# MiniXC/LightningFastSpeech2

Hardware: AMD Instinct MI355X
Metric: mel-frames/sec (whole node), 256-phoneme batch-32 (higher is better)
Workload: dtype bf16

## Files before the change

### lightningfastspeech2_amd/csrc/capi_ops.hip

```cpp
#include <math.h>

#include "fs2_common.h"
#include "fs2_kernels.h"

using namespace fs2;

namespace fs2 {

template <typename S, typename D>
__global__ __launch_bounds__(256) void convert_kernel(const S* __restrict__ s, D* __restrict__ d, size_t n) {
    for (size_t i = (size_t)blockIdx.x * 256 + threadIdx.x; i < n; i += (size_t)gridDim.x * 256)
        d[i] = Num<D>::from_f32(Num<S>::to_f32(s[i]));
}

int launch_convert(const ConvertArgs& a, int sdt, int ddt, hipStream_t st) {
    if (a.n == 0) return FS2_OK;
    size_t blocks = (a.n + 255) / 256;
    if (blocks > 4096) blocks = 4096;
    const dim3 g((unsigned)blocks), b(256);
    if (sdt == FS2_F32 && ddt == FS2_F32) hipLaunchKernelGGL((convert_kernel<float, float>), g, b, 0, st, (const float*)a.src, (float*)a.dst, a.n);
    else if (sdt == FS2_F32 && ddt == FS2_BF16) hipLaunchKernelGGL((convert_kernel<float, bf16>), g, b, 0, st, (const float*)a.src, (bf16*)a.dst, a.n);
    else if (sdt == FS2_BF16 && ddt == FS2_F32) hipLaunchKernelGGL((convert_kernel<bf16, float>), g, b, 0, st, (const bf16*)a.src, (float*)a.dst, a.n);
    else if (sdt == FS2_BF16 && ddt == FS2_BF16) hipLaunchKernelGGL((convert_kernel<bf16, bf16>), g, b, 0, st, (const bf16*)a.src, (bf16*)a.dst, a.n);
    else return FS2_ERR_ARG;
    return hipGetLastError() == hipSuccess ? FS2_OK : FS2_ERR_HIP;
}

}

namespace fs2 {
int apply_knob(Tuning& t, int variant) {
    int ok = 1;
    if (variant == 1500 || variant == 1501) t.attn_x3 = variant - 1500;
    else if (variant >= 1400 && variant <= 1402) t.gemm_wres = variant - 1400;
    else if (variant == 1340 || variant == 1341) t.enc_attn_out = variant - 1340;
    else if (variant == 1320 || variant == 1321) t.pred_fuse_embed = variant - 1320;
    else if (variant >= 1200 && variant <= 1204) t.attn_pipe = variant - 1200;
    else if (variant == 1100 || variant == 1101) t.colsum_fused = variant - 1100;
    else if (variant == 1000 || variant == 1001) t.bgemm_tn256 = variant - 1000;
    else if (variant >= 905 && variant <= 908) { if (variant >= 907) t.attn_bwd_nb_dq = 3 + ((variant - 905) & 1); else t.attn_bwd_nb = 3 + ((variant - 905) & 1); }
    else if (variant == 909) t.attn_bwd_nb = 1;
    else if (variant >= 900 && variant <= 903) { if (variant >= 902) t.attn_bwd_nb_dq = ((variant - 900) & 1) + 1; else t.attn_bwd_nb = ((variant - 900) & 1) + 1; }
    else if (variant == 904) t.attn_bwd_nb_dq = 0;
    else if (variant == 800 || variant == 801) t.bgemm_full = variant - 800;
    else if (variant == 700 || variant == 701) t.bgemm_xcd = variant - 700;
    else if (variant == 500 || variant == 501) t.split_f32 = variant - 500;
    else if (variant == 230 || variant == 231) t.head_sums = variant - 230;
    else if (variant == 220 || variant == 221) t.gemm_persist = variant - 220;
    else if (variant >= 200 && variant <= 202) t.slab_xcd_remap = variant - 200;
    else if (variant >= 0 && variant <= 7) t.gemm_variant = variant;
    else ok = 0;
    if (!ok) return FS2_ERR_ARG;
    ++t.gen;
    return FS2_OK;
}
Tuning& op_tuning() {
    static thread_local Tuning t;
    return t;
}
}

extern "C" {

int fs2_op_convert(int32_t sdt, int32_t ddt, const void* src, void* dst, size_t n, void* stream) {
    ConvertArgs a{src, dst, n};
    return launch_convert(a, sdt, ddt, (hipStream_t)stream);
}

int fs2_op_predictor(int32_t dtype, const void* x, const void* w, const float* bias, const float* ln_g,
                     const float* ln_b, const float* head_w, float head_b, const uint8_t* mask, float* pred,
                     void* packed_scratch, int32_t B, int32_t S, int32_t H, int32_t nlayers, int32_t taps,
                     void* stream) {
    if (!predictor_fused_supported(dtype, H, taps, nlayers, S)) return FS2_ERR_SHAPE;
    if (!x || !w || !bias || !ln_g || !ln_b || !head_w || !pred || !packed_scratch) return FS2_ERR_ARG;
    const size_t lb = predictor_packed_bytes_per_layer();
    for (int l = 0; l < nlayers; ++l) {
        const int r = launch_pack_predictor_weights((const char*)w + (size_t)l * H * taps * H * 2,
                                                    (char*)packed_scratch + lb * l, (hipStream_t)stream);
        if (r != FS2_OK) return r;
    }
    PredictorArgs a;
    a.x = x; a.wpk = packed_scratch; a.bias = bias; a.ln_g = ln_g; a.ln_b = ln_b; a.head_w = head_w; a.head_b = head_b;
    a.mask = mask; a.pred = pred; a.B = B; a.S = S; a.H = H; a.nlayers = nlayers; a.taps = taps; a.eps = 1e-5f;
    return launch_predictor_fused(a, (hipStream_t)stream);
}

int fs2_op_predictor_dw(int32_t dtype, const void* x, const float* dw_w, const float* dw_b, const void* w, const float* bias,
                        const float* ln_g, const float* ln_b, const float* head_w, float head_b, const uint8_t* mask, float* pred,
                        void* packed_scratch, int32_t B, int32_t S, int32_t H, int32_t nlayers, void* stream) {
    if (!predictor_fused_supported(dtype, H, 3, nlayers, S)) return FS2_ERR_SHAPE;
    if (!x || !dw_w || !dw_b || !w || !bias || !ln_g || !ln_b || !head_w || !pred || !packed_scratch) return FS2_ERR_ARG;
    const size_t lb = predictor_packed_bytes_per_layer(1);
    for (int l = 0; l < nlayers; ++l) {
        const int r = launch_pack_predictor_weights((const char*)w + (size_t)l * H * H * 2, (char*)packed_scratch + lb * l, (hipStream_t)stream, 1);
        if (r != FS2_OK) return r;
    }
    PredictorArgs a;
    a.x = x; a.wpk = packed_scratch; a.dw_w = dw_w; a.dw_b = dw_b; a.bias = bias; a.ln_g = ln_g; a.ln_b = ln_b; a.head_w = head_w; a.head_b = head_b;
    a.mask = mask; a.pred = pred; a.B = B; a.S = S; a.H = H; a.nlayers = nlayers; a.taps = 3; a.eps = 1e-5f;
    return launch_predictor_fused(a, (hipStream_t)stream);
}

int fs2_op_soft_dtw(const float* x, const float* y, int32_t B, int32_t N, int32_t M, int32_t D, float gamma, float* out,
                    void* stream) {
    if (!x || !y || !out) return FS2_ERR_ARG;
    SoftDtwArgs a{x, y, out, B, N, M, D, gamma};
    return launch_soft_dtw(a, (hipStream_t)stream);
}
size_t fs2_op_soft_dtw_grad_scratch_bytes(int32_t B, int32_t N, int32_t M) { return soft_dtw_grad_scratch_bytes(B, N, M); }
int fs2_op_soft_dtw_grad(const float* x, const float* y, int32_t B, int32_t N, int32_t M, int32_t D, float gamma, float* out,
                         float* grad_x, void* scratch, size_t scratch_bytes, void* stream) {
    if (!x || !y || !out) return FS2_ERR_ARG;
    SoftDtwArgs a{x, y, out, B, N, M, D, gamma};
    return launch_soft_dtw_grad(a, grad_x, scratch, scratch_bytes, (hipStream_t)stream);
}

size_t fs2_op_masked_loss_ws_bytes(void) { return fs2::masked_loss_ws_bytes(); }

int fs2_op_masked_loss(const float* pred, const void* truth, int32_t truth_kind, const uint8_t* pad_mask, int64_t rows,
                       int32_t inner, int32_t kind, void* ws, float* out2, void* stream) {
    if (!pred || !truth || !pad_mask || !ws || !out2) return FS2_ERR_ARG;
    if ((kind != 0 && kind != 1) || (truth_kind != 0 && truth_kind != 1)) return FS2_ERR_ARG;
    fs2::LossArgs a;
    a.pred = pred; a.truth = truth; a.mask = pad_mask; a.ws = ws; a.out = out2;
    a.rows = rows; a.inner = inner; a.kind = kind; a.truth_kind = truth_kind;
    return fs2::launch_masked_loss(a, (hipStream_t)stream);
}

int fs2_op_set_vocoder_fused_resblock(int32_t on) {
    fs2::op_tuning().voc_fused_resblock = on;
    return FS2_OK;
}

int fs2_op_set_vocoder_lds_limit(int32_t kib) {
    fs2::op_tuning().voc_lds_limit = kib;
    return FS2_OK;
}



int fs2_op_set_gemm_variant(int32_t variant) { return fs2::apply_knob(fs2::op_tuning(), variant); }

int fs2_op_gemm(int32_t dtype, int32_t out_dtype, const void* x, const void* w, const float* bias, void* c,
                int32_t M, int32_t N, int32_t Cin, int32_t taps, int32_t S, int32_t relu, void* stream) {
    GemmArgs a;
    a.X = x; a.W = w; a.bias = bias; a.C = c;
    a.M = M; a.N = N; a.K = taps * Cin; a.ldx = Cin; a.ldc = N;
    a.Cin = Cin; a.taps = taps; a.pad = (taps - 1) / 2; a.S = S; a.relu = relu;
    return launch_gemm(a, dtype, out_dtype, (hipStream_t)stream);
}

int fs2_op_gemm_relu_dropout(int32_t dtype, const void* x, const void* w, const float* bias, void* c, int32_t M, int32_t N, int32_t Cin,
                             int32_t taps, int32_t S, float p, uint64_t seed, uint64_t key, void* stream) {
    if (!(p > 0.f && p < 1.f)) return FS2_ERR_ARG;
    GemmArgs a;
    a.X = x; a.W = w; a.bias = bias; a.C = c;
    a.M = M; a.N = N; a.K = taps * Cin; a.ldx = Cin; a.ldc = N;
    a.Cin = Cin; a.taps = taps; a.pad = (taps - 1) / 2; a.S = S; a.relu = 1;
    a.drop_p = p; a.drop_seed = seed; a.drop_key = key;
    return launch_gemm(a, dtype, dtype, (hipStream_t)stream);
}

int fs2_op_gemm_add(int32_t dtype, const void* x, const void* w, const float* bias, const void* addend, void* c, int32_t M, int32_t N,
                    int32_t Cin, int32_t taps, int32_t S, void* stream) {
    if (!addend) return FS2_ERR_ARG;
    GemmArgs a;
    a.X = x; a.W = w; a.bias = bias; a.C = c;
    a.M = M; a.N = N; a.K = taps * Cin; a.ldx = Cin; a.ldc = N;
    a.Cin = Cin; a.taps = taps; a.pad = (taps - 1) / 2; a.S = S; a.relu = 0;
    a.epi_res = addend;
    if (N < 192 || M % S || !(taps & 1)) return FS2_ERR_SHAPE;
    return launch_gemm(a, dtype, dtype, (hipStream_t)stream);
}

int fs2_op_gemm_rowscale(const void* x, const void* w, const float* bias, const float* rowstats, const float* wg,
                         void* c, int32_t M, int32_t N, int32_t Cin, void* stream) {
    if (!x || !w || !bias || !rowstats || !wg || !c) return FS2_ERR_ARG;
    GemmArgs a;
    a.X = x; a.W = w; a.bias = bias; a.C = c;
    a.M = M; a.N = N; a.K = Cin; a.ldx = Cin; a.ldc = N;
    a.Cin = Cin; a.taps = 1; a.pad = 0; a.S = M; a.relu = 0;
    a.rs_stats = rowstats; a.rs_wg = wg;
    return launch_gemm(a, FS2_BF16, FS2_BF16, (hipStream_t)stream);
}
int fs2_op_rowstats_finish(const float* parts, int32_t nparts, int32_t ncols, float eps, float* out, int32_t M, void* stream) {
    return launch_rowstats_finish(parts, nparts, ncols, eps, out, M, (hipStream_t)stream);
}
int fs2_op_gemm_head(const void* x, const void* w, const float* bias, const float* head_gw, float* stats_out, float* head_out, int32_t M,
// ... 435 lines not shown
```

### lightningfastspeech2_amd/csrc/engine.hip

```cpp
#include <math.h>
#include <stdarg.h>
#include <stdio.h>
#include <string.h>

#include <functional>
#include <map>
#include <memory>
#include <string>
#include <vector>

#include "fs2_common.h"
#include "fs2_kernels.h"

using namespace fs2;

namespace {

struct HostTensor {
    std::vector<int64_t> shape;
    std::vector<float> data;
};

struct Arena {
    char* base = nullptr;
// ... 661 lines not shown
    a.B = B; a.S = S; a.C = w.C; a.k = w.k; a.pad = (w.k - 1) / 2;
    Bracket br(e, FS2_K_ROWOPS, st, 2.0 * B * S * (double)w.C * w.k, 2.0 * B * S * (double)w.C * (dt == FS2_BF16 ? 2 : 4));
    const int r = launch_dwconv(a, dt, st);
    if (r != FS2_OK) return fail(e, r, "dwconv launch failed");
    return FS2_OK;
}

int norm_only(fs2_engine* e, hipStream_t st, int dt, const void* v, const float* stats, const float* g, const float* b, void* y,
              int M, int H, const float* dot_w = nullptr, float dot_b = 0.f, const uint8_t* mask = nullptr, float* pred = nullptr) {
    LayerNormArgs l;
    l.pre_stats = stats; l.pre_parts = ln_parts(H);
    l.x = v; l.res = nullptr; l.gamma = g; l.beta = b; l.y = y;
    l.dot_w = dot_w; l.dot_b = dot_b; l.mask = mask; l.pred = pred;
    l.M = M; l.H = H; l.eps = 1e-5f;
    Bracket br(e, FS2_K_ROWOPS, st, 0, 2.0 * M * (double)H * (dt == FS2_BF16 ? 2 : 4));
    if (launch_layernorm(l, dt, st) != FS2_OK) return fail(e, FS2_ERR_HIP, "normalise-only LayerNorm launch failed");
    return FS2_OK;
}

struct LayerScratch {
    float *st1, *st2;
    float* rsf;
    float* hd;
    void *qkv, *att, *proj, *hid, *u, *vt;
    uint64_t* bits;
    int Spad, nw64;
};

int conformer(fs2_engine* e, hipStream_t st, const LayerW& w, void* x, void* tmp, int B, int S, int heads,
              const LayerScratch& sc, bool is_decoder, bool prenorm_in = false, const float* pg = nullptr, const float* pb = nullptr,
              bool leave_prenorm = false) {
    const int H = e->cfg.hidden, M = B * S, dt = w.in_proj.dt;
    const double dsz = dt == FS2_BF16 ? 2 : 4;
    Bracket* mha = is_decoder ? nullptr : new Bracket(e, FS2_K_ENC_MHA, st, 8.0 * M * (double)H * H + 4.0 * B * (double)S * S * H,
                                                      2.0 * M * H * dsz + 4.0 * H * H * dsz);
    struct MhaEnd { Bracket*& b; ~MhaEnd() { delete b; b = nullptr; } } mha_end{mha};
    const bool x3 = e->front_split && dt == FS2_F32 && e->tune.attn_x3;
    void* qkv_lo = x3 ? (void*)((char*)sc.qkv + (size_t)M * 3 * H * 2) : nullptr;
    if (prenorm_in) {
        if (!w.has_fold || !(w.depthwise && H > 256 && e->defer_ln)) return fail(e, FS2_ERR_STATE, "pre-norm block input without folded weights");
        const RowScale rs{sc.rsf, w.in_wg};
        CHK(gemm(e, st, w.in_proj_f, x, sc.qkv, M, M, false, dt, nullptr, -1, nullptr, nullptr, nullptr, &rs));
    } else {
        CHK(gemm(e, st, w.in_proj, x, sc.qkv, M, M, false, dt, nullptr, -1, nullptr, nullptr, qkv_lo));
    }
    AttnArgs a;
    a.tune = &e->tune;
    a.qkv_lo = qkv_lo;
    a.qkv = sc.qkv; a.vt = sc.vt; a.kbits = sc.bits; a.out = sc.att;
    a.B = B; a.S = S; a.H = H; a.heads = heads; a.Spad = sc.Spad; a.nw64 = sc.nw64;
    a.scale_log2e = (float)(1.4426950408889634 / sqrt((double)(H / heads)));
    if (w.wo_pk && S <= 768 && e->tune.enc_attn_out && !x3 && !prenorm_in && attn_out_ln_supported(dt, H, heads, S) &&
        !(w.depthwise && H > 256 && e->defer_ln)) {
        AttnOutArgs ao;
        ao.qkv = sc.qkv; ao.kbits = sc.bits; ao.wpk = w.wo_pk; ao.bias = w.out_proj.b; ao.res = x; ao.ln_g = w.g1; ao.ln_b = w.b1; ao.out = tmp;
        ao.B = B; ao.S = S; ao.H = H; ao.heads = heads; ao.nw64 = sc.nw64; ao.scale_log2e = a.scale_log2e; ao.eps = 1e-5f;
        {
            Bracket br(e, FS2_K_ATTENTION, st, 4.0 * B * (double)S * S * H + 2.0 * M * (double)H * H, 5.0 * M * H * dsz + (double)H * H * dsz);
            const int r = launch_attn_out_ln(ao, st);
            if (r != FS2_OK) return fail(e, r, "fused attention + out-projection launch failed");
        }
        delete mha; mha = nullptr;
        if (w.depthwise) {
            CHK(dwconv(e, st, w.dw, tmp, sc.u, B, S, dt));
            CHK(gemm(e, st, w.c1, sc.u, sc.hid, M, S, true, dt, nullptr, is_decoder ? FS2_K_DEC_FFN_CONV1 : -1));
        } else {
            CHK(gemm(e, st, w.c1, tmp, sc.hid, M, S, true, dt, nullptr, is_decoder ? FS2_K_DEC_FFN_CONV1 : -1));
        }
        LnFuse ln;
        ln.res = tmp; ln.g = w.g2; ln.b = w.b2; ln.tmp = sc.proj;
        CHK(gemm(e, st, w.c2, sc.hid, x, M, S, false, dt, &ln));
        return FS2_OK;
    }
    {
        Bracket br(e, FS2_K_ROWOPS, st, 0, 2.0 * M * H * dsz);
        const int r = x3 ? FS2_OK : launch_transpose_v(a, dt, st);
        if (r != FS2_OK) return fail(e, r, "transpose_v launch failed");
    }
    {
        Bracket br(e, FS2_K_ATTENTION, st, 4.0 * B * (double)S * S * H, 4.0 * M * H * dsz);
        Bracket br2(e, FS2_K_DEC_ATTENTION, st, 4.0 * B * (double)S * S * H, 4.0 * M * H * dsz, is_decoder);
        const int r = launch_attention(a, dt, st);
        if (r != FS2_OK) return fail(e, r, "attention launch failed");
    }
    if (w.depthwise && H > 256 && e->defer_ln) {
        Deferred d1;
        d1.res = x; d1.stats_out = sc.st1;
        if (prenorm_in) { d1.res_stats = sc.st2; d1.res_g = pg; d1.res_b = pb; }
        CHK(gemm(e, st, w.out_proj, sc.att, tmp, M, M, false, dt, nullptr, -1, nullptr, &d1));
        delete mha; mha = nullptr;
        LnOnLoad l1{sc.st1, w.g1, w.b1};
        CHK(dwconv(e, st, w.dw, tmp, sc.u, B, S, dt, &l1));
        CHK(gemm(e, st, w.c1, sc.u, sc.hid, M, S, true, dt, nullptr, is_decoder ? FS2_K_DEC_FFN_CONV1 : -1));
        Deferred d2;
        d2.res = tmp; d2.res_stats = sc.st1; d2.res_g = w.g1; d2.res_b = w.b1; d2.stats_out = sc.st2;
        CHK(gemm(e, st, w.c2, sc.hid, x, M, S, false, dt, nullptr, -1, nullptr, &d2));
        if (leave_prenorm) {
            if (launch_rowstats_finish(sc.st2, ln_parts(H), H, 1e-5f, sc.rsf, M, st) != FS2_OK) return fail(e, FS2_ERR_HIP, "row statistics launch failed");
            return FS2_OK;
        }
        return norm_only(e, st, dt, x, sc.st2, w.g2, w.b2, x, M, H);
    }
    {
        LnFuse ln;
        ln.res = x; ln.g = w.g1; ln.b = w.b1; ln.tmp = sc.proj;
        CHK(gemm(e, st, w.out_proj, sc.att, tmp, M, M, false, dt, &ln));
        delete mha; mha = nullptr;
    }
    if (w.depthwise) {
        CHK(dwconv(e, st, w.dw, tmp, sc.u, B, S, dt));
        CHK(gemm(e, st, w.c1, sc.u, sc.hid, M, S, true, dt, nullptr, is_decoder ? FS2_K_DEC_FFN_CONV1 : -1));
    } else {
        CHK(gemm(e, st, w.c1, tmp, sc.hid, M, S, true, dt, nullptr, is_decoder ? FS2_K_DEC_FFN_CONV1 : -1));
    }
    {
        LnFuse ln;
        ln.res = tmp; ln.g = w.g2; ln.b = w.b2; ln.tmp = sc.proj;
        CHK(gemm(e, st, w.c2, sc.hid, x, M, S, false, dt, &ln));
    }
    return FS2_OK;
}

int run_stack(fs2_engine* e, hipStream_t st, const std::vector<LayerW>& Ls, void* x, void* tmp, int B, int S, int heads,
              const LayerScratch& sc, bool is_decoder, bool leave_last = false, bool* left = nullptr) {
    const int H = e->cfg.hidden;
    bool pre = false;
    for (size_t i = 0; i < Ls.size(); ++i) {
        const LayerW& w = Ls[i];
        const bool deferred = w.depthwise && H > 256 && e->defer_ln;
        const bool leave = e->fold_ln && deferred && (i + 1 < Ls.size() ? Ls[i + 1].has_fold && Ls[i + 1].depthwise : leave_last);
        CHK(conformer(e, st, w, x, tmp, B, S, heads, sc, is_decoder, pre, pre ? Ls[i - 1].g2 : nullptr, pre ? Ls[i - 1].b2 : nullptr, leave));
        pre = leave;
    }
    if (left) *left = pre;
    return FS2_OK;
}

struct CwtOut {
    float* spec12 = nullptr;
    float* mean_std = nullptr;
    float* spec_out = nullptr;
};

struct EmbedTail {
    void* y;
    const float* bins;
    const float* emb;
    int nbins;
    float std, mean;
    const float* pe;
    const float* spk;
};

int predictor(fs2_engine* e, hipStream_t st, const PredictorW& P, const void* x, int B, int S, const uint8_t* mask,
              float* pred, const LayerScratch& sc, const CwtOut* cw = nullptr, const EmbedTail* tail = nullptr, bool* tail_done = nullptr) {
    const int M = B * S;
    if (tail_done) *tail_done = false;
    if (P.cwt && !cw) return fail(e, FS2_ERR_STATE, "CWT predictor without its output buffers");
    if (P.wpk && P.wpk_lo && e->fuse_predictor && P.dt == FS2_F32 && e->front_split &&
        predictor_fused_x3_supported(P.filt, P.layers[0].c.taps, (int)P.layers.size(), S)) {
        PredictorArgs a;
        a.x = x; a.wpk = P.wpk; a.wpk_lo = P.wpk_lo; a.bias = P.bias_all; a.ln_g = P.g_all; a.ln_b = P.b_all;
        a.head_w = P.head_w; a.head_b = P.head_b; a.mask = mask; a.pred = pred;
        a.B = B; a.S = S; a.H = P.filt; a.nlayers = (int)P.layers.size(); a.taps = P.layers[0].c.taps; a.eps = 1e-5f;
        const bool with_tail = tail && tail_done && !P.cwt && tail->y != x && tail->nbins >= 2 && tail->nbins - 1 <= 512;
        if (with_tail) {
            a.be_y = tail->y; a.be_bins = tail->bins; a.be_emb = tail->emb; a.be_nbins = tail->nbins;
            a.be_std = tail->std; a.be_mean = tail->mean; a.be_pe = tail->pe; a.be_spk = tail->spk;
        }
        const double fl = 2.0 * M * (double)P.filt * P.filt * a.taps * a.nlayers;
        Bracket br(e, FS2_K_CONV_GEMM, st, fl, (double)M * P.filt * 4 + (double)M * 4 + (with_tail ? 2.0 * M * P.filt * 4 : 0.0));
        Bracket brp(e, FS2_K_PREDICTOR, st, fl, (double)M * P.filt * 4 + (double)M * 4 + (with_tail ? 2.0 * M * P.filt * 4 : 0.0), x != e->xA && x != e->xB);
        const int r = launch_predictor_fused_x3(a, st);
        if (r != FS2_OK) return fail(e, r, "fused predictor (split arithmetic) launch failed (B=%d S=%d)", B, S);
        if (with_tail) *tail_done = true;
        return FS2_OK;
    }
    if (P.wpk && !P.wpk_lo && e->fuse_predictor && predictor_fused_supported(P.dt, P.filt, P.dw_all ? 3 : P.layers[0].c.taps, (int)P.layers.size(), S)) {
        PredictorArgs a;
        a.x = x; a.wpk = P.wpk; a.bias = P.bias_all; a.ln_g = P.g_all; a.ln_b = P.b_all;
        a.dw_w = P.dw_all; a.dw_b = P.dwb_all;
        a.head_w = P.head_w; a.head_b = P.head_b; a.mask = mask; a.pred = pred;
        a.B = B; a.S = S; a.H = P.filt; a.nlayers = (int)P.layers.size(); a.taps = P.dw_all ? 3 : P.layers[0].c.taps; a.eps = 1e-5f;
        const bool with_tail = tail && tail_done && !P.cwt && tail->y != x && tail->nbins >= 2 && tail->nbins - 1 <= 512;
        if (with_tail) {
            a.be_y = tail->y; a.be_bins = tail->bins; a.be_emb = tail->emb; a.be_nbins = tail->nbins;
            a.be_std = tail->std; a.be_mean = tail->mean; a.be_pe = tail->pe; a.be_spk = tail->spk;
        }
        const double fl = (P.dw_all ? 2.0 * M * (double)P.filt * (P.filt + 3) : 2.0 * M * (double)P.filt * P.filt * a.taps) * a.nlayers;
        const double by = (double)M * P.filt * 2 + (double)M * 4 + (with_tail ? 2.0 * M * P.filt * 2 : 0.0);
        Bracket br(e, FS2_K_CONV_GEMM, st, fl, by);
        Bracket brp(e, FS2_K_PREDICTOR, st, fl, by, x != e->xA && x != e->xB);
        const int r = launch_predictor_fused(a, st);
        if (r != FS2_OK) return fail(e, r, "fused predictor launch failed (B=%d S=%d)", B, S);
        if (with_tail) *tail_done = true;
        return FS2_OK;
    }
    if (P.layers[0].depthwise && P.filt > 256 && e->defer_ln) {
        const void* src = x;
        float* stats[2] = {sc.st1, sc.st2};
        const PredLayerW* prev = nullptr;
        bool head_done = false;
        for (size_t j = 0; j < P.layers.size(); ++j) {
            const PredLayerW& Lw = P.layers[j];
            void* out = (j & 1) ? sc.proj : sc.att;
            LnOnLoad lp{stats[(j + 1) & 1], prev ? prev->g : nullptr, prev ? prev->b : nullptr};
            CHK(dwconv(e, st, Lw.dw, src, sc.u, B, S, P.dt, prev ? &lp : nullptr));
            Deferred d;
            d.stats_out = stats[j & 1];
            if (j + 1 == P.layers.size() && !P.cwt && P.head_gw) { d.head_gw = P.head_gw; d.head_out = sc.hd; d.head_done = &head_done; }
            CHK(gemm(e, st, Lw.c, sc.u, out, M, S, true, P.dt, nullptr, -1, nullptr, &d));
            src = out;
            prev = &Lw;
        }
        float* stl = stats[(P.layers.size() - 1) & 1];
        if (head_done) {
            Bracket br(e, FS2_K_ROWOPS, st, 0, (double)M * ln_parts(P.filt) * 12);
            if (launch_head_finish(stl, sc.hd, ln_parts(P.filt), P.filt, 1e-5f, P.head_sum_gw, P.head_cst, mask, pred, M, st) != FS2_OK)
                return fail(e, FS2_ERR_HIP, "head finish launch failed");
            return FS2_OK;
        }
        if (!P.cwt) return norm_only(e, st, P.dt, src, stl, prev->g, prev->b, nullptr, M, P.filt, P.head_w, P.head_b, mask, pred);
        CHK(norm_only(e, st, P.dt, src, stl, prev->g, prev->b, (void*)src, M, P.filt));
        CHK(gemm(e, st, P.head_mat, src, cw->spec12, M, M, false, FS2_F32));
        CwtArgs ca{src, cw->spec12, 12, mask, P.ms_w, P.ms_b, cw->mean_std, pred, cw->spec_out, B, S, P.filt};
        if (launch_cwt_head(ca, P.dt, st) != FS2_OK) return fail(e, FS2_ERR_HIP, "cwt head launch failed");
        return FS2_OK;
    }
    const void* src = x;
    for (size_t j = 0; j < P.layers.size(); ++j) {
        const PredLayerW& Lw = P.layers[j];
        const bool last = j + 1 == P.layers.size();
        void* out = (j & 1) ? sc.proj : sc.att;
        void* other = (j & 1) ? sc.att : sc.proj;
        LnFuse ln;
        ln.g = Lw.g; ln.b = Lw.b;
        const bool keep = !last || P.cwt;
        if (last && !P.cwt) { ln.dot_w = P.head_w; ln.dot_b = P.head_b; ln.mask = mask; ln.pred = pred; }
        if (Lw.depthwise) {
            CHK(dwconv(e, st, Lw.dw, src, sc.u, B, S, P.dt));
            ln.tmp = other;
            CHK(gemm(e, st, Lw.c, sc.u, keep ? out : nullptr, M, S, true, P.dt, &ln));
        } else {
            ln.tmp = sc.u;
            CHK(gemm(e, st, Lw.c, src, keep ? out : nullptr, M, S, true, P.dt, &ln));
        }
        src = out;
    }
    if (P.cwt) {
        CHK(gemm(e, st, P.head_mat, src, cw->spec12, M, M, false, FS2_F32));
        CwtArgs ca{src, cw->spec12, 12, mask, P.ms_w, P.ms_b, cw->mean_std, pred, cw->spec_out, B, S, P.filt};
        if (launch_cwt_head(ca, P.dt, st) != FS2_OK) return fail(e, FS2_ERR_HIP, "cwt head launch failed");
    }
    return FS2_OK;
}

size_t layer_scratch_bytes(const fs2_engine* e, int B, int S) {
    const fs2_config& c = e->cfg;
    const size_t H = c.hidden, M = (size_t)B * S, esz = e->esz;
    size_t Fm = c.enc_filter > c.dec_filter ? c.enc_filter : c.dec_filter;
    size_t Pm = H;
    if ((size_t)c.var_filter > Pm) Pm = c.var_filter;
    if ((size_t)c.dur_filter > Pm) Pm = c.dur_filter;
    const size_t Spad = ((size_t)S + 63) / 64 * 64;
    return al(M * 3 * H * esz) + 3 * al(M * Pm * esz) + al(M * Fm * esz) + al((size_t)B * H * Spad * esz) +
           al((size_t)B * (Spad / 64) * 8) + 2 * al(M * (size_t)ln_parts((int)Pm) * 8) + al(M * 8) + al(M * 16) + 4096;
}
int take_layer_scratch(fs2_engine* e, Arena& ar, int B, int S, LayerScratch* sc) {
    const fs2_config& c = e->cfg;
    const size_t H = c.hidden, M = (size_t)B * S, esz = e->esz;
    size_t Fm = c.enc_filter > c.dec_filter ? c.enc_filter : c.dec_filter;
    size_t Pm = H;
    if ((size_t)c.var_filter > Pm) Pm = c.var_filter;
    if ((size_t)c.dur_filter > Pm) Pm = c.dur_filter;
    sc->Spad = (S + 63) / 64 * 64;
    sc->nw64 = sc->Spad / 64;
    sc->st1 = (float*)ar.take(M * (size_t)ln_parts((int)Pm) * 8);
    sc->st2 = (float*)ar.take(M * (size_t)ln_parts((int)Pm) * 8);
    sc->rsf = (float*)ar.take(M * 8);
    sc->hd = (float*)ar.take(M * 16);
    sc->qkv = ar.take(M * 3 * H * esz);
    sc->att = ar.take(M * Pm * esz);
    sc->proj = ar.take(M * Pm * esz);
    sc->hid = ar.take(M * Fm * esz);
    sc->u = ar.take(M * Pm * esz);
    sc->vt = ar.take((size_t)B * H * sc->Spad * esz);
    sc->bits = (uint64_t*)ar.take((size_t)B * sc->nw64 * 8);
    if (!sc->st1 || !sc->st2 || !sc->rsf || !sc->hd || !sc->qkv || !sc->att || !sc->proj || !sc->hid || !sc->u || !sc->vt || !sc->bits)
        return fail(e, FS2_ERR_NOMEM, "scratch arena too small");
    return FS2_OK;
}

size_t persist_bytes(const fs2_engine* e, int B, int L) {
    const size_t H = e->cfg.hidden, ML = (size_t)B * L, esz = e->esz;
    size_t pv = 0;
    for (int v = 0; v < e->cfg.n_variances; ++v)
        if (e->cfg.var_level[v]) pv += al(ML * 4) + (e->cfg.var_cwt[v] ? al(ML * 10 * 4) + al((size_t)B * 8) : 0);
    return al((size_t)B * H * 4) + 2 * al(ML * H * esz) + al(ML * 4) + 2 * al(ML * 4) + 2 * al((size_t)B * 4) + al(ML) + pv + 4096;
}
size_t encode_scratch_bytes(const fs2_engine* e, int B, int L) {
    size_t cw = 0;
    for (int v = 0; v < e->cfg.n_variances; ++v)
        if (e->cfg.var_level[v] && e->cfg.var_cwt[v]) cw = al((size_t)B * L * 12 * 4) + 512;
    return layer_scratch_bytes(e, B, L) + cw;
}
size_t decode_scratch_bytes(const fs2_engine* e, int B, int T) {
    const size_t H = e->cfg.hidden, MT = (size_t)B * T, esz = e->esz;
    size_t cw = 0;
    for (int v = 0; v < e->cfg.n_variances; ++v)
        if (e->cfg.var_cwt[v]) cw = al(MT * 12 * 4) + al((size_t)B * 8) + 512;
    return layer_scratch_bytes(e, B, T) + 2 * al(MT * H * esz) + al(MT) + (size_t)e->cfg.n_variances * al(MT * 4) + cw + 4096;
}
int ensure_arena(fs2_engine* e, Arena& ar, size_t need, const char* what) {
    if (need > ar.cap && !ar.external) HIPCHK(e, hipDeviceSynchronize());
    if (ar.reserve(need) != FS2_OK)
        return fail(e, FS2_ERR_NOMEM, ar.external ? "caller workspace too small: %s needs %zu bytes (fs2_workspace_bytes)"
                                                  : "%s arena: hipMalloc of %zu bytes failed", what, need);
    return FS2_OK;
}

int tap_store(fs2_engine* e, hipStream_t st, const std::string& name, const void* src, size_t n, int src_dt,
              Arena* arena = nullptr) {
    void* dst = (arena ? arena : &e->dbg)->take(n * 4);
    if (!dst) return fail(e, FS2_ERR_NOMEM, "debug arena too small");
    ConvertArgs a{src, dst, n};
    const int r = launch_convert(a, src_dt, FS2_F32, st);
    if (r != FS2_OK) return fail(e, r, "convert launch failed");
    e->taps[name] = {dst, n * 4};
    return FS2_OK;
}

}

extern "C" {

int fs2_abi_version(void) { return FS2_ABI_VERSION; }

const char* fs2_status_string(int s) {
    switch (s) {
        case FS2_OK: return "ok";
        case FS2_ERR_HIP: return "HIP runtime error";
        case FS2_ERR_SHAPE: return "unsupported shape/config";
        case FS2_ERR_ARG: return "bad argument";
        case FS2_ERR_WEIGHT: return "weight error";
        case FS2_ERR_STATE: return "call order violated";
        case FS2_ERR_NOMEM: return "out of device memory";
    }
    return "unknown status";
}

const char* fs2_last_error(const fs2_engine* e) { return e ? e->err : "null engine"; }

int fs2_create(const fs2_config* cfg, fs2_engine** out) {
    if (!cfg || !out) return FS2_ERR_ARG;
    fs2_engine* e = new fs2_engine();
    e->cfg = *cfg;
    e->err[0] = 0;
    *out = e;
    const int r = check_config(e);
    if (r != FS2_OK) return r;
    e->dt = cfg->dtype;
    e->fdt = cfg->dtype == FS2_BF16 ? FS2_BF16 : FS2_F32;
    e->bdt = (cfg->dtype == FS2_F32 || cfg->dtype == FS2_F32_X3) ? FS2_F32 : FS2_BF16;
    e->esz = cfg->dtype == FS2_BF16 ? 2 : 4;
    e->front_split = cfg->dtype == FS2_MIXED_X3 || cfg->dtype == FS2_F32_X3;
    build_spec(e);
    return FS2_OK;
}

int fs2_clone(const fs2_engine* src, fs2_engine** out) {
    if (!src || !out) return FS2_ERR_ARG;
    if (!src->finalized) return FS2_ERR_STATE;
    fs2_engine* e = new fs2_engine();
    e->cfg = src->cfg;
    e->dt = src->dt; e->fdt = src->fdt; e->bdt = src->bdt; e->esz = src->esz;
    e->err[0] = 0;
    e->finalized = true;
    e->fuse_predictor = src->fuse_predictor;
    e->use_graph = src->use_graph;
    e->zero_pad_mel = src->zero_pad_mel;
    e->defer_ln = src->defer_ln;
    e->fold_ln = src->fold_ln;
    e->tune = src->tune;
    e->front_split = src->front_split;
    e->spec = src->spec;
    e->dev_allocs = src->dev_allocs;
    e->phone_table = src->phone_table; e->pe = src->pe; e->spk_w = src->spk_w; e->spk_b = src->spk_b;
    e->enc = src->enc; e->dec = src->dec; e->dur = src->dur; e->vars = src->vars; e->mel = src->mel; e->priors_w = src->priors_w;
    e->mel_f = src->mel_f; e->mel_wg = src->mel_wg; e->mel_fold = src->mel_fold;
    *out = e;
    return FS2_OK;
}

int fs2_destroy(fs2_engine* e) {
    if (!e) return FS2_OK;
    (void)hipDeviceSynchronize();
    e->dev_allocs.reset();
    e->persist.release();
    e->scratch.release();
    e->dbg.release();
    e->dbg_enc.release();
    if (e->h_pinned) (void)hipHostFree(e->h_pinned);
    for (auto& g : e->dgraphs) if (g.exec) (void)hipGraphExecDestroy(g.exec);
    for (auto& g : e->egraphs) if (g.exec) (void)hipGraphExecDestroy(g.exec);
    if (e->gev_in) (void)hipEventDestroy(e->gev_in);
    if (e->gev_out) (void)hipEventDestroy(e->gev_out);
    if (e->gstream) (void)hipStreamDestroy(e->gstream);
    for (auto& s : e->prof)
        for (auto& ev : s.ev) { (void)hipEventDestroy(ev.first); (void)hipEventDestroy(ev.second); }
    delete e;
    return FS2_OK;
}

int fs2_load_weight(fs2_engine* e, const char* name, const float* data, const int64_t* shape, int32_t ndim) {
    if (!e || !name || !data || !shape || ndim < 0) return FS2_ERR_ARG;
    if (e->finalized) return fail(e, FS2_ERR_STATE, "weights already finalized");
    auto it = e->spec.find(name);
    if (it == e->spec.end()) return fail(e, FS2_ERR_WEIGHT, "unexpected weight '%s' for this config", name);
    const std::vector<int64_t>& want = it->second;
    bool ok = (size_t)ndim == want.size();
    size_t n = 1;
    for (int i = 0; ok && i < ndim; ++i) { ok = shape[i] == want[i]; n *= (size_t)shape[i]; }
    if (!ok) return fail(e, FS2_ERR_WEIGHT, "shape mismatch for '%s'", name);
    HostTensor t;
    t.shape.assign(shape, shape + ndim);
    t.data.assign(data, data + n);
    e->host[name] = std::move(t);
    return FS2_OK;
}

int fs2_finalize(fs2_engine* e) {
    if (!e) return FS2_ERR_ARG;
    if (e->finalized) return FS2_OK;
    for (auto& kv : e->spec)
        if (!e->host.count(kv.first)) return fail(e, FS2_ERR_WEIGHT, "missing weight '%s'", kv.first.c_str());
    const fs2_config& c = e->cfg;
    const int H = c.hidden;
    CHK(up_vec(e, "phone_embedding.weight", &e->phone_table));
    CHK(up_vec(e, "positional_encoding.pe", &e->pe));
    CHK(up_vec(e, "speaker_embedding.projection.weight", &e->spk_w));
    CHK(up_vec(e, "speaker_embedding.projection.bias", &e->spk_b));
    e->enc.resize(c.enc_layers);
    for (int i = 0; i < c.enc_layers; ++i)
        CHK(make_layer(e, "encoder.layers." + std::to_string(i), H, c.enc_filter, c.enc_depthwise, &e->enc[i], e->fdt));
    e->dec.resize(c.dec_layers);
    for (int i = 0; i < c.dec_layers; ++i)
        CHK(make_layer(e, "decoder.layers." + std::to_string(i), H, c.dec_filter, c.dec_depthwise, &e->dec[i], e->bdt));
    if (H > 256) {
        for (int i = 1; i < c.enc_layers && c.enc_depthwise && e->fdt == FS2_BF16; ++i)
            CHK(make_folded_in_proj(e, "encoder.layers." + std::to_string(i), "encoder.layers." + std::to_string(i - 1), H, &e->enc[i]));
        for (int i = 1; i < c.dec_layers && c.dec_depthwise && e->bdt == FS2_BF16; ++i)
            CHK(make_folded_in_proj(e, "decoder.layers." + std::to_string(i), "decoder.layers." + std::to_string(i - 1), H, &e->dec[i]));
    }
    CHK(make_predictor(e, "variance_adaptor.duration_predictor", c.dur_nlayers, c.dur_filter, c.dur_depthwise, &e->dur, e->fdt));
    e->vars.resize(c.n_variances);
    for (int v = 0; v < c.n_variances; ++v) {
        const std::string p = std::string("variance_adaptor.encoders.") + c.var_names[v];
        CHK(make_predictor(e, p + ".predictor", c.var_nlayers[v], c.var_filter, c.var_depthwise, &e->vars[v].pred, e->fdt, c.var_cwt[v] != 0));
        if (c.var_cwt[v]) {
            CHK(up_vec(e, p + ".mean_std_linear.weight", &e->vars[v].pred.ms_w));
            CHK(up_vec(e, p + ".mean_std_linear.bias", &e->vars[v].pred.ms_b));
        }
        CHK(up_vec(e, p + ".bins", &e->vars[v].bins));
        CHK(up_vec(e, p + ".embedding.weight", &e->vars[v].emb));
    }
    CHK(make_conv(e, "linear.weight", "linear.bias", &e->mel, e->bdt));
    if (H > 256 && c.dec_layers > 0 && c.dec_depthwise && e->bdt == FS2_BF16 && c.n_mels < 192) {
        const std::string pp = "decoder.layers." + std::to_string(c.dec_layers - 1);
        const HostTensor &w = W(e, "linear.weight"), &b = W(e, "linear.bias"), &g = W(e, pp + ".norm2.weight"), &be = W(e, pp + ".norm2.bias");
        const int N = (int)b.data.size();
        std::vector<float> wf((size_t)N * H), bf(N), wg(N);
        for (int n = 0; n < N; ++n) {
            double bacc = b.data[n], gacc = 0;
            for (int k = 0; k < H; ++k) {
                const float v = (float)((double)w.data[(size_t)n * H + k] * g.data[k]);
                wf[(size_t)n * H + k] = v;
                bacc += (double)w.data[(size_t)n * H + k] * be.data[k];
                gacc += (double)bf16_to_f32(f32_to_bf16(v));
            }
            bf[n] = (float)bacc;
            wg[n] = (float)gacc;
        }
        e->mel_f.N = N; e->mel_f.Cin = H; e->mel_f.taps = 1; e->mel_f.dt = FS2_BF16;
        CHK(upload_mat(e, wf.data(), wf.size(), &e->mel_f.w, FS2_BF16));
        CHK(upload_f32(e, bf.data(), bf.size(), &e->mel_f.b));
        CHK(upload_f32(e, wg.data(), wg.size(), &e->mel_wg));
        e->mel_fold = true;
    }
    e->priors_w.resize(c.n_priors);
    for (int p = 0; p < c.n_priors; ++p) {
        const std::string q = std::string("prior_embeddings.") + c.prior_names[p];
        CHK(up_vec(e, q + ".bins", &e->priors_w[p].bins));
        std::vector<float> t = W(e, q + ".embedding.weight").data;
        for (float& v : t) v = v > 0.f ? v : 0.f;
        CHK(upload_f32(e, t.data(), t.size(), &e->priors_w[p].emb));
    }
    e->host.clear();
    e->finalized = true;
    return FS2_OK;
}

int fs2_set_fused_predictor(fs2_engine* e, int32_t on) {
    if (!e) return FS2_ERR_ARG;
    e->fuse_predictor = on != 0;
    return FS2_OK;
}

int fs2_set_debug(fs2_engine* e, int32_t on) {
    if (!e) return FS2_ERR_ARG;
    e->debug = on != 0;
    return FS2_OK;
}

int fs2_set_deferred_layernorm(fs2_engine* e, int32_t on) {
    if (!e) return FS2_ERR_ARG;
    e->defer_ln = on != 0;
    return FS2_OK;
}

int fs2_set_tuning(fs2_engine* e, int32_t knob) {
    if (!e) return FS2_ERR_ARG;
    const bool op_only = (knob >= 900 && knob <= 909) || knob == 1000 || knob == 1001 || knob == 1100 || knob == 1101 ||
                         knob == 700 || knob == 701 || knob == 800 || knob == 801 || knob == 500 || knob == 501;
    if (op_only) return fail(e, FS2_ERR_ARG, "fs2_set_tuning(%d): an operator-level switch no engine launch reads (use fs2_op_set_gemm_variant on the calling thread)", (int)knob);
    const int r = apply_knob(e->tune, knob);
    if (r != FS2_OK) return fail(e, r, "fs2_set_tuning(%d): not a defined switch", (int)knob);
    return FS2_OK;
}

int fs2_set_folded_layernorm(fs2_engine* e, int32_t on) {
    if (!e) return FS2_ERR_ARG;
    e->fold_ln = on != 0;
    return FS2_OK;
}

int fs2_set_zero_pad_mel(fs2_engine* e, int32_t on) {
    if (!e) return FS2_ERR_ARG;
    e->zero_pad_mel = on != 0;
    return FS2_OK;
}

int fs2_workspace_bytes(const fs2_engine* e, int32_t B, int32_t L, int32_t T, size_t* persist, size_t* scratch) {
    if (!e || B <= 0 || L <= 0 || T < 0) return FS2_ERR_ARG;
    if (persist) *persist = persist_bytes(e, B, L);
    if (scratch) {
        const size_t enc = encode_scratch_bytes(e, B, L), dec = T > 0 ? decode_scratch_bytes(e, B, T) : 0;
        *scratch = enc > dec ? enc : dec;
    }
    return FS2_OK;
}

int fs2_set_workspace(fs2_engine* e, void* persist, size_t persist_bytes_, void* scratch, size_t scratch_bytes_) {
    if (!e || (persist == nullptr) != (scratch == nullptr)) return e ? fail(e, FS2_ERR_ARG, "give both buffers or neither") : FS2_ERR_ARG;
    if (((uintptr_t)persist | (uintptr_t)scratch) & 255) return fail(e, FS2_ERR_ARG, "workspace buffers must be 256-byte aligned");
    if (e->mid_forward && (char*)persist != e->persist.base)
        return fail(e, FS2_ERR_STATE, "the persist buffer holds the encoder state between fs2_encode and fs2_decode: only scratch may change there");
    if (!e->mid_forward) e->persist.adopt(persist, persist_bytes_);
    e->scratch.adopt(scratch, scratch_bytes_);
    return FS2_OK;
}

int fs2_set_frames(fs2_engine* e, int32_t T) {
    if (!e) return FS2_ERR_ARG;
    if (!e->encoded) return fail(e, FS2_ERR_STATE, "fs2_set_frames without a preceding successful fs2_encode");
    if (T < e->T) return fail(e, FS2_ERR_ARG, "fs2_set_frames can only pad: T=%d < this batch's %d", T, e->T);
    if (T > e->cfg.max_frames || T > e->cfg.pe_len) return fail(e, FS2_ERR_SHAPE, "T=%d exceeds max_frames/positional table", T);
    e->T = T;
    return FS2_OK;
}

static void drop_graphs(fs2_engine* e);
static int encode_body(fs2_engine* e, const int64_t* phones, const float* speaker, const int32_t* forced, LayerScratch& sc, hipStream_t st);

static int variance_stage(fs2_engine* e, hipStream_t st, int v, void*& x, void*& xalt, int B, int S, const uint8_t* mask, float* vpred,
                          const LayerScratch& sc, const CwtOut* cwo, bool add_pe_spk, Arena& dbg) {
    const fs2_config& c = e->cfg;
    const size_t M = (size_t)B * S, H = c.hidden, esz = e->esz;
    const bool tail_ok = e->tune.pred_fuse_embed && !e->debug && !e->forced_idx[v] && !e->forced_tgt[v] && !c.var_cwt[v] &&
                         (e->fdt == FS2_BF16 || (e->fdt == FS2_F32 && e->front_split && e->vars[v].pred.wpk_lo)) && H == 256;
    const EmbedTail tl{xalt, e->vars[v].bins, e->vars[v].emb, c.var_nbins, c.var_std[v], c.var_mean[v],
                       add_pe_spk ? e->pe : nullptr, add_pe_spk ? e->spk : nullptr};
    bool tail_done = false;
    CHK(predictor(e, st, e->vars[v].pred, x, B, S, mask, vpred, sc, cwo, tail_ok ? &tl : nullptr, &tail_done));
    if (tail_done) {
        std::swap(x, xalt);
        return FS2_OK;
    }
    int32_t* idx = nullptr;
    if (e->debug) {
        idx = (int32_t*)dbg.take(M * 4);
        if (!idx) return fail(e, FS2_ERR_NOMEM, "debug arena too small");
        e->taps[std::string("bucket_") + c.var_names[v]] = {idx, M * 4};
    }
    Bracket br(e, FS2_K_ROWOPS, st, 0, 2.0 * M * H * esz);
    BucketArgs ba{x, vpred, e->vars[v].bins, e->vars[v].emb, c.var_nbins, c.var_std[v], c.var_mean[v],
                  add_pe_spk ? e->pe : nullptr, add_pe_spk ? e->spk : nullptr, x, idx, B, S, (int)H,
                  e->forced_idx[v], 0, e->forced_tgt[v]};
    if (launch_bucket_embed(ba, e->fdt, st) != FS2_OK) return fail(e, FS2_ERR_HIP, "bucket_embed launch failed");
    return FS2_OK;
}
static int run_phase(fs2_engine* e, std::vector<fs2_engine::GraphEntry>& cache, const std::vector<uint64_t>& key, bool plain,
                     hipStream_t st, const std::function<int(hipStream_t)>& body);

int fs2_encode(fs2_engine* e, const int64_t* phones, const float* speaker, int32_t B, int32_t L,
               const int32_t* forced, void* stream, int32_t* T_out) {
    if (!e || !phones || !speaker || !T_out || B <= 0 || L <= 0) return e ? fail(e, FS2_ERR_ARG, "bad encode argument") : FS2_ERR_ARG;
    if (!e->finalized) return fail(e, FS2_ERR_STATE, "fs2_finalize not called");
    if (L > e->cfg.pe_len) return fail(e, FS2_ERR_SHAPE, "L=%d exceeds positional table %d", L, e->cfg.pe_len);
    hipStream_t st = (hipStream_t)stream;
    const fs2_config& c = e->cfg;
    const size_t H = c.hidden, ML = (size_t)B * L, esz = e->esz;
    e->encoded = false;
    e->mid_forward = false;
    e->B = B;
    e->L = L;
    e->taps.clear();
    CHK(ensure_arena(e, e->persist, persist_bytes(e, B, L), "persist"));
    CHK(ensure_arena(e, e->scratch, encode_scratch_bytes(e, B, L), "scratch"));
    e->spk = (float*)e->persist.take((size_t)B * H * 4);
    e->xA = e->persist.take(ML * H * esz);
    e->xB = e->persist.take(ML * H * esz);
    e->dur_pred = (float*)e->persist.take(ML * 4);
    e->d_dur = (int32_t*)e->persist.take(ML * 4);
    e->d_cum = (int32_t*)e->persist.take(ML * 4);
    e->d_totals = (int32_t*)e->persist.take((size_t)2 * B * 4);
    e->d_guard = e->d_totals ? e->d_totals + B : nullptr;
    e->src_mask = (uint8_t*)e->persist.take(ML);
    bool pv_ok = true, pv_forced = false;
    for (int v = 0; v < c.n_variances; ++v) {
        e->pv_pred[v] = e->pv_spec[v] = e->pv_ms[v] = nullptr;
        if (!c.var_level[v]) continue;
        e->pv_pred[v] = (float*)e->persist.take(ML * 4);
        if (c.var_cwt[v]) {
            e->pv_spec[v] = (float*)e->persist.take(ML * 10 * 4);
            e->pv_ms[v] = (float*)e->persist.take((size_t)B * 8);
        }
        pv_ok = pv_ok && e->pv_pred[v] && (!c.var_cwt[v] || (e->pv_spec[v] && e->pv_ms[v]));
        pv_forced = pv_forced || e->forced_idx[v] || e->forced_tgt[v];
    }
    if (!e->src_mask || !pv_ok) return fail(e, FS2_ERR_NOMEM, "persist arena too small");
    LayerScratch sc;
    CHK(take_layer_scratch(e, e->scratch, B, L, &sc));
    if (e->h_pinned_cap < 2 * B) {
        if (e->h_pinned) (void)hipHostFree(e->h_pinned);
        e->h_pinned = nullptr;
        HIPCHK(e, hipHostMalloc((void**)&e->h_pinned, (size_t)2 * B * 4, hipHostMallocDefault));
        e->h_pinned_cap = 2 * B;
        drop_graphs(e);
    }
    {
        std::vector<uint64_t> key = {(uint64_t)B, (uint64_t)L, (uint64_t)e->persist.base, (uint64_t)e->scratch.base, (uint64_t)phones,
                                     (uint64_t)speaker, (uint64_t)forced, (uint64_t)e->h_pinned, (uint64_t)e->fuse_predictor, (uint64_t)e->tune.gen,
                                     (uint64_t)e->defer_ln, (uint64_t)e->front_split, (uint64_t)e->fold_ln};
        const bool plain = c.n_priors != 0 || pv_forced;
        CHK(run_phase(e, e->egraphs, key, plain, st, [&](hipStream_t s2) { return encode_body(e, phones, speaker, forced, sc, s2); }));
    }
    HIPCHK(e, hipStreamSynchronize(st));
    e->totals.assign(e->h_pinned, e->h_pinned + B);
    e->guard.assign(e->h_pinned + B, e->h_pinned + 2 * B);
    int mx = 0;
    for (int b = 0; b < B; ++b) mx = e->totals[b] > mx ? e->totals[b] : mx;
    e->T = mx < c.max_frames ? mx : c.max_frames;
    if (e->T > c.pe_len) return fail(e, FS2_ERR_SHAPE, "T=%d exceeds positional table %d", e->T, c.pe_len);
    *T_out = e->T;
    e->encoded = true;
    e->mid_forward = true;
    return FS2_OK;
}

static int encode_body(fs2_engine* e, const int64_t* phones, const float* speaker, const int32_t* forced, LayerScratch& sc, hipStream_t st) {
    const fs2_config& c = e->cfg;
    const int B = e->B, L = e->L;
    const size_t H = c.hidden, ML = (size_t)B * L, esz = e->esz;
    {
        Bracket br(e, FS2_K_ROWOPS, st, 0, ML * H * esz);
        SpkProjArgs sp{speaker, e->spk_w, e->spk_b, e->spk, B, (int)H, c.dvec_dim};
        if (launch_spk_proj(sp, st) != FS2_OK) return fail(e, FS2_ERR_HIP, "spk_proj launch failed");
        EmbedArgs em{phones, e->phone_table, e->pe, e->spk, e->xA, e->src_mask, B, L, (int)H, c.n_phones};
        if (launch_embed(em, e->fdt, st) != FS2_OK) return fail(e, FS2_ERR_HIP, "embed launch failed");
        MaskBitsArgs mb{e->src_mask, sc.bits, B, L, sc.nw64};
        if (launch_mask_bits(mb, st) != FS2_OK) return fail(e, FS2_ERR_HIP, "mask_bits launch failed");
    }
    CHK(run_stack(e, st, e->enc, e->xA, e->xB, B, L, c.enc_heads, sc, false));
    if (e->debug) {
        const size_t need_d = al(ML * H * 4) + (size_t)c.n_variances * al(ML * 4) + 4096;
        if (need_d > e->dbg_enc.cap) HIPCHK(e, hipDeviceSynchronize());
        if (e->dbg_enc.reserve(need_d) != FS2_OK) return fail(e, FS2_ERR_NOMEM, "debug arena");
        CHK(tap_store(e, st, "encoder_out", e->xA, ML * H, e->fdt, &e->dbg_enc));
    }
    if (c.n_priors) {
        if (!e->priors_dev || e->priors_B != B) return fail(e, FS2_ERR_STATE, "fs2_set_priors(B=%d) required before fs2_encode", B);
        for (int p = 0; p < c.n_priors; ++p) {
            BucketArgs ba{e->xA, e->priors_dev + (size_t)p * B, e->priors_w[p].bins, e->priors_w[p].emb, c.var_nbins,
                          1.0f, 0.0f, nullptr, nullptr, e->xA, nullptr, B, L, (int)H, nullptr, 1};
            if (launch_bucket_embed(ba, e->fdt, st) != FS2_OK) return fail(e, FS2_ERR_HIP, "prior embedding launch failed");
        }
        e->priors_dev = nullptr;
    }
    CHK(predictor(e, st, e->dur, e->xA, B, L, e->src_mask, e->dur_pred, sc));
    void* x = e->xA;
    void* xalt = e->xB;
    float* spec12 = nullptr;
    for (int v = 0; v < c.n_variances; ++v) {
        if (!c.var_level[v]) continue;
        CwtOut cwo;
        if (c.var_cwt[v]) {
            if (!spec12) spec12 = (float*)e->scratch.take(ML * 12 * 4);
            if (!spec12) return fail(e, FS2_ERR_NOMEM, "scratch arena too small");
            cwo.spec12 = spec12;
            cwo.mean_std = e->pv_ms[v];
            cwo.spec_out = e->pv_spec[v];
        }
        CHK(variance_stage(e, st, v, x, xalt, B, L, e->src_mask, e->pv_pred[v], sc, c.var_cwt[v] ? &cwo : nullptr, false, e->dbg_enc));
        e->forced_idx[v] = nullptr, e->forced_tgt[v] = nullptr;
    }
    if (x != e->xA) HIPCHK(e, hipMemcpyAsync(e->xA, x, ML * H * esz, hipMemcpyDeviceToDevice, st));
    DurationArgs da{e->dur_pred, e->src_mask, forced, e->d_dur, e->d_cum, e->d_totals, e->d_guard, B, L};
    if (launch_durations(da, st) != FS2_OK) return fail(e, FS2_ERR_HIP, "durations launch failed");
    HIPCHK(e, hipMemcpyAsync(e->h_pinned, e->d_totals, (size_t)2 * B * 4, hipMemcpyDeviceToHost, st));
    return FS2_OK;
}

int fs2_set_priors(fs2_engine* e, const float* priors_device, int32_t B) {
    if (!e || !priors_device || B <= 0) return FS2_ERR_ARG;
    if (e->cfg.n_priors == 0) return fail(e, FS2_ERR_STATE, "this engine was configured without priors");
    e->priors_dev = priors_device;
    e->priors_B = B;
    return FS2_OK;
}

int fs2_last_totals(const fs2_engine* e, int32_t* totals, int32_t* guard, int32_t B) {
    if (!e || !e->encoded || B != e->B) return FS2_ERR_STATE;
    if (totals) memcpy(totals, e->totals.data(), (size_t)B * 4);
    if (guard) memcpy(guard, e->guard.data(), (size_t)B * 4);
    return FS2_OK;
}

static int decode_body(fs2_engine* e, const fs2_outputs* out, hipStream_t st) {
    const fs2_config& c = e->cfg;
    const int B = e->B, L = e->L, T = e->T;
    const size_t H = c.hidden, MT = (size_t)B * T, ML = (size_t)B * L, esz = e->esz;
    auto phone_outputs = [&]() -> int {
        if (out->duration_prediction) HIPCHK(e, hipMemcpyAsync(out->duration_prediction, e->dur_pred, ML * 4, hipMemcpyDeviceToDevice, st));
        if (out->duration_rounded) HIPCHK(e, hipMemcpyAsync(out->duration_rounded, e->d_dur, ML * 4, hipMemcpyDeviceToDevice, st));
        if (out->src_mask) HIPCHK(e, hipMemcpyAsync(out->src_mask, e->src_mask, ML, hipMemcpyDeviceToDevice, st));
        for (int v = 0; v < c.n_variances; ++v) {
            if (!c.var_level[v]) continue;
            if (out->variances[v]) HIPCHK(e, hipMemcpyAsync(out->variances[v], e->pv_pred[v], ML * 4, hipMemcpyDeviceToDevice, st));
            if (c.var_cwt[v] && out->var_spectrogram[v]) HIPCHK(e, hipMemcpyAsync(out->var_spectrogram[v], e->pv_spec[v], ML * 10 * 4, hipMemcpyDeviceToDevice, st));
            if (c.var_cwt[v] && out->var_mean_std[v]) HIPCHK(e, hipMemcpyAsync(out->var_mean_std[v], e->pv_ms[v], (size_t)B * 8, hipMemcpyDeviceToDevice, st));
        }
        return FS2_OK;
    };
    if (T == 0) { e->encoded = false; e->mid_forward = false; return phone_outputs(); }

    CHK(ensure_arena(e, e->scratch, decode_scratch_bytes(e, B, T), "scratch"));
    e->mid_forward = false;
    void* yA = e->scratch.take(MT * H * esz);
    void* yB = e->scratch.take(MT * H * esz);
    uint8_t* tmask = out->tgt_mask ? out->tgt_mask : (uint8_t*)e->scratch.take(MT);
    float* vpred[FS2_MAX_VARIANCES] = {nullptr, nullptr, nullptr, nullptr};
    int last_frame_v = -1;
    for (int v = 0; v < c.n_variances; ++v) {
        if (c.var_level[v]) continue;
        last_frame_v = v;
        vpred[v] = out->variances[v] ? out->variances[v] : (float*)e->scratch.take(MT * 4);
        if (!vpred[v]) return fail(e, FS2_ERR_NOMEM, "scratch arena too small");
    }
    float *cw_spec = nullptr, *cw_ms = nullptr;
    for (int v = 0; v < c.n_variances; ++v)
        if (c.var_cwt[v] && !c.var_level[v] && !cw_spec) {
            cw_spec = (float*)e->scratch.take(MT * 12 * 4);
            cw_ms = (float*)e->scratch.take((size_t)B * 8);
            if (!cw_spec || !cw_ms) return fail(e, FS2_ERR_NOMEM, "scratch arena too small");
        }
    LayerScratch sc;
    CHK(take_layer_scratch(e, e->scratch, B, T, &sc));
    if (!yA || !yB || !tmask) return fail(e, FS2_ERR_NOMEM, "scratch arena too small");
    if (e->debug) {
        const size_t need_d = 3 * al(MT * H * 4) + (size_t)c.n_variances * al(MT * 4) + 4096;
        if (need_d > e->dbg.cap) HIPCHK(e, hipDeviceSynchronize());
        if (e->dbg.reserve(need_d) != FS2_OK) return fail(e, FS2_ERR_NOMEM, "debug arena");
    }

    {
        Bracket br(e, FS2_K_ROWOPS, st, 0, 2.0 * MT * H * esz);
        RegulateArgs ra{e->xA, e->d_cum, e->d_totals, yA, tmask, B, L, T, (int)H};
        if (launch_regulate(ra, e->fdt, st) != FS2_OK) return fail(e, FS2_ERR_HIP, "regulate launch failed");
        MaskBitsArgs mb{tmask, sc.bits, B, T, sc.nw64};
        if (launch_mask_bits(mb, st) != FS2_OK) return fail(e, FS2_ERR_HIP, "mask_bits launch failed");
    }
    if (e->debug) CHK(tap_store(e, st, "regulated", yA, MT * H, e->fdt));
    const bool fuse_pe = !e->debug;
    for (int v = 0; v < c.n_variances; ++v) {
        if (c.var_level[v]) continue;
        CwtOut cwo;
        if (c.var_cwt[v]) {
            cwo.spec12 = cw_spec;
            cwo.mean_std = out->var_mean_std[v] ? out->var_mean_std[v] : cw_ms;
            cwo.spec_out = out->var_spectrogram[v];
        }
        CHK(variance_stage(e, st, v, yA, yB, B, T, tmask, vpred[v], sc, c.var_cwt[v] ? &cwo : nullptr, v == last_frame_v && fuse_pe, e->dbg));
    }
    if (e->debug) CHK(tap_store(e, st, "adaptor_out", yA, MT * H, e->fdt));
    if (!fuse_pe || last_frame_v < 0) {
        BucketArgs ba{yA, nullptr, nullptr, nullptr, 0, 0.f, 0.f, e->pe, e->spk, yA, nullptr, B, T, (int)H, nullptr};
        if (launch_bucket_embed(ba, e->fdt, st) != FS2_OK) return fail(e, FS2_ERR_HIP, "pe/spk add launch failed");
    }
    if (e->fdt != e->bdt) {
        ConvertArgs ca{yA, yB, MT * H};
        if (launch_convert(ca, e->fdt, e->bdt, st) != FS2_OK) return fail(e, FS2_ERR_HIP, "front -> back conversion failed");
        std::swap(yA, yB);
    }
    bool dec_pre = false;
    CHK(run_stack(e, st, e->dec, yA, yB, B, T, c.dec_heads, sc, true, e->mel_fold && out->mel && !e->debug, &dec_pre));
    if (e->debug) CHK(tap_store(e, st, "decoder_out", yA, MT * H, e->bdt));
    if (out->mel && dec_pre) {
        const RowScale rs{sc.rsf, e->mel_wg};
        CHK(gemm(e, st, e->mel_f, yA, out->mel, (int)MT, (int)MT, false, FS2_F32, nullptr, -1, e->zero_pad_mel ? tmask : nullptr, nullptr, nullptr, &rs));
    } else if (out->mel) {
        CHK(gemm(e, st, e->mel, yA, out->mel, (int)MT, (int)MT, false, FS2_F32, nullptr, -1, e->zero_pad_mel ? tmask : nullptr));
    }
    for (int v = 0; v < FS2_MAX_VARIANCES; ++v) e->forced_idx[v] = nullptr, e->forced_tgt[v] = nullptr;
    return phone_outputs();
}

static void drop_graphs(fs2_engine* e) {
    for (auto& g : e->dgraphs) if (g.exec) (void)hipGraphExecDestroy(g.exec);
    for (auto& g : e->egraphs) if (g.exec) (void)hipGraphExecDestroy(g.exec);
    e->dgraphs.clear();
    e->egraphs.clear();
}

static int run_phase(fs2_engine* e, std::vector<fs2_engine::GraphEntry>& cache, const std::vector<uint64_t>& key, bool plain,
                     hipStream_t st, const std::function<int(hipStream_t)>& body) {
    static const bool gdbg = getenv("FS2_GRAPH_DEBUG") != nullptr;
    plain = plain || !e->use_graph || e->debug;
    for (int k = 0; k < FS2_K_COUNT && !plain; ++k) plain = e->prof[k].enabled;
    if (plain) return body(st);
    fs2_engine::GraphEntry* g = nullptr;
    for (auto& c : cache) if (c.key == key) { g = &c; break; }
    if (!g) {
        if (cache.size() >= 8) {
            size_t old = 0;
            for (size_t i = 1; i < cache.size(); ++i) if (cache[i].stamp < cache[old].stamp) old = i;
            if (cache[old].exec) (void)hipGraphExecDestroy(cache[old].exec);
            cache.erase(cache.begin() + old);
        }
        cache.emplace_back();
        cache.back().key = key;
        cache.back().stamp = ++e->gclock;
        if (gdbg) fprintf(stderr, "fs2 graph: new signature (%zu cached)\n", cache.size());
        return body(st);
    }
    g->stamp = ++e->gclock;
    if (g->bad) { if (gdbg) fprintf(stderr, "fs2 graph: signature marked bad\n"); return body(st); }
    if (!e->gstream) {
        if (hipStreamCreateWithFlags(&e->gstream, hipStreamNonBlocking) != hipSuccess ||
            hipEventCreateWithFlags(&e->gev_in, hipEventDisableTiming) != hipSuccess ||
            hipEventCreateWithFlags(&e->gev_out, hipEventDisableTiming) != hipSuccess) {
            e->use_graph = false;
            return body(st);
        }
    }
    if (!g->exec) {
        if (hipStreamBeginCapture(e->gstream, hipStreamCaptureModeThreadLocal) != hipSuccess) { g->bad = true; return body(st); }
        const bool enc = e->encoded, mid = e->mid_forward;
        const int r = body(e->gstream);
        hipGraph_t graph = nullptr;
        const hipError_t ce = hipStreamEndCapture(e->gstream, &graph);
        hipError_t ie = hipSuccess;
        if (r != FS2_OK || ce != hipSuccess || !graph || (ie = hipGraphInstantiate(&g->exec, graph, nullptr, nullptr, 0)) != hipSuccess) {
            if (gdbg) fprintf(stderr, "fs2 graph: capture failed (body %d, end %d %s, instantiate %d)\n", r, (int)ce, hipGetErrorString(ce), (int)ie);
            if (graph) (void)hipGraphDestroy(graph);
            (void)hipGetLastError();
            g->exec = nullptr;
            g->bad = true;
            e->encoded = enc; e->mid_forward = mid;
            return body(st);
        }
        (void)hipGraphDestroy(graph);
    }
    HIPCHK(e, hipEventRecord(e->gev_in, st));
    HIPCHK(e, hipStreamWaitEvent(e->gstream, e->gev_in, 0));
    HIPCHK(e, hipGraphLaunch(g->exec, e->gstream));
    HIPCHK(e, hipEventRecord(e->gev_out, e->gstream));
    HIPCHK(e, hipStreamWaitEvent(st, e->gev_out, 0));
    e->graph_replays++;
    return FS2_OK;
}

int fs2_decode(fs2_engine* e, const fs2_outputs* out, void* stream) {
    if (!e || !out) return FS2_ERR_ARG;
    if (!e->encoded) return fail(e, FS2_ERR_STATE, "fs2_decode without a preceding successful fs2_encode");
    hipStream_t st = (hipStream_t)stream;
    bool plain = !e->use_graph || e->debug || e->T == 0;
    for (int v = 0; v < FS2_MAX_VARIANCES && !plain; ++v) plain = e->forced_idx[v] || e->forced_tgt[v];
    if (plain) return decode_body(e, out, st);
    const char* base0 = e->scratch.base;
    CHK(ensure_arena(e, e->scratch, decode_scratch_bytes(e, e->B, e->T), "scratch"));
    if (e->scratch.base != base0) drop_graphs(e);
    std::vector<uint64_t> key = {(uint64_t)e->B, (uint64_t)e->L, (uint64_t)e->T, (uint64_t)e->scratch.base, (uint64_t)e->persist.base,
                                 (uint64_t)e->xA, (uint64_t)e->d_cum, (uint64_t)e->spk, (uint64_t)e->zero_pad_mel, (uint64_t)e->fuse_predictor, (uint64_t)e->tune.gen,
                                 (uint64_t)e->defer_ln, (uint64_t)e->front_split, (uint64_t)e->fold_ln, (uint64_t)out->mel, (uint64_t)out->tgt_mask,
                                 (uint64_t)out->duration_prediction, (uint64_t)out->duration_rounded, (uint64_t)out->src_mask};
    for (int v = 0; v < FS2_MAX_VARIANCES; ++v) {
        key.push_back((uint64_t)out->variances[v]);
        key.push_back((uint64_t)out->var_mean_std[v]);
        key.push_back((uint64_t)out->var_spectrogram[v]);
    }
    const int r = run_phase(e, e->dgraphs, key, false, st, [&](hipStream_t s2) { return decode_body(e, out, s2); });
    if (r == FS2_OK) e->mid_forward = false;
    return r;
}

int fs2_set_graphs(fs2_engine* e, int32_t on) {
    if (!e) return FS2_ERR_ARG;
    e->use_graph = on != 0;
    if (!on) drop_graphs(e);
    return FS2_OK;
}

int64_t fs2_graph_replays(const fs2_engine* e) { return e ? e->graph_replays : -1; }

int fs2_force_buckets(fs2_engine* e, int32_t variance_index, const int32_t* idx) {
    if (!e || variance_index < 0 || variance_index >= e->cfg.n_variances) return FS2_ERR_ARG;
    e->forced_idx[variance_index] = idx;
    return FS2_OK;
}

int fs2_force_variance_targets(fs2_engine* e, int32_t variance_index, const float* tgt) {
    if (!e || variance_index < 0 || variance_index >= e->cfg.n_variances) return FS2_ERR_ARG;
    e->forced_tgt[variance_index] = tgt;
    return FS2_OK;
}

int fs2_debug_copy(fs2_engine* e, const char* what, void* dst, void* stream) {
    if (!e || !what || !dst) return FS2_ERR_ARG;
    auto it = e->taps.find(what);
    if (it == e->taps.end()) return fail(e, FS2_ERR_STATE, "no debug tap '%s' (fs2_set_debug before encode?)", what);
    HIPCHK(e, hipMemcpyAsync(dst, it->second.first, it->second.second, hipMemcpyDeviceToDevice, (hipStream_t)stream));
    return FS2_OK;
}

int fs2_profile_enable(fs2_engine* e, int32_t cls, int32_t enable) {
    if (!e || cls < 0 || cls >= FS2_K_COUNT) return FS2_ERR_ARG;
    ProfSlot& s = e->prof[cls];
    s.enabled = enable != 0;
    s.used = 0;
    s.flops = s.bytes = 0;
    return FS2_OK;
}

int fs2_profile_reserve(fs2_engine* e, int32_t cls, int32_t pairs) {
    if (!e || cls < 0 || cls >= FS2_K_COUNT || pairs < 0) return FS2_ERR_ARG;
// ... 31 lines not shown
```

### lightningfastspeech2_amd/csrc/fs2_kernels.h

```cpp
#pragma once
#include <hip/hip_runtime.h>
#include <stdint.h>

#include "../../include/fs2.h"

namespace fs2 {

struct Tuning {
    int gemm_variant = 0;
    int gemm_wres = 1;
    int head_sums = 1;
    int gemm_persist = 1;
    int slab_xcd_remap = 1;
    int split_f32 = 0;
    int attn_pipe = 3;
    int attn_x3 = 1;
    int enc_attn_out = 1;
    int pred_fuse_embed = 1;
    int attn_bwd_nb = 1, attn_bwd_nb_dq = 0;
    int colsum_fused = 0;
    int bgemm_full = 1, bgemm_xcd = 1, bgemm_tn256 = 1;
    int voc_lds_limit = 0;
    int voc_fused_resblock = 1;
    unsigned long long gen = 0;
};
Tuning& op_tuning();
int apply_knob(Tuning& t, int variant);
inline const Tuning& tuning_of(const Tuning* t) { return t ? *t : op_tuning(); }

struct GemmArgs {
    const void* X;
    const void* W;
    const float* bias;
    void* C;
    void* C_lo = nullptr;
    int M, N, K;
    int ldx, ldc;
    int Cin, taps, pad;
    int S;
    int relu;
    const void* res = nullptr;
    const float* ln_g = nullptr;
    const float* ln_b = nullptr;
    float ln_eps = 1e-5f;
    const float* dot_w = nullptr;
    float dot_b = 0.f;
    const uint8_t* mask = nullptr;
    float* pred = nullptr;
    void* ln_tmp = nullptr;
    void* z_out = nullptr;
    int xcd_remap = 0;
    const Tuning* tune = nullptr;
    const void* epi_res = nullptr;
    const float* epi_res_stats = nullptr;
    const float* epi_res_g = nullptr;
    const float* epi_res_b = nullptr;
    int epi_res_parts = 0;
    float* stats_out = nullptr;
    int w_presplit = 0;
    int split = 0;
    const uint8_t* zero_rows = nullptr;
    const void* gate = nullptr;
    float gate_scale = 1.f;
    float drop_p = 0.f;
    uint64_t drop_seed = 0, drop_key = 0;
    const float* rs_stats = nullptr;
    const float* rs_wg = nullptr;
    const float* head_gw = nullptr;
    float* head_out = nullptr;
    int ksplit = 0;
};
int launch_gemm(const GemmArgs& a, int in_dtype, int out_dtype, hipStream_t stream);
int launch_presplit_pack(const float* w, void* out, size_t n_values, hipStream_t stream);
bool gemm_presplit_eligible(int N, int K);
int launch_split_k_reduce(const float* part, void* out, size_t n, int ksplit, int accumulate, int out_dtype, hipStream_t stream);
int gemm_splitk_choice(int M, int N, int Cin, int taps, int S, int in_dtype);
bool gemm_wres_supported(const GemmArgs& a, int in_dtype, int out_dtype, bool force);
int launch_gemm_wres(const GemmArgs& a, hipStream_t stream);
bool gemm_persist_supported(const GemmArgs& a, int in_dtype, int out_dtype, int mi);
bool gemm_head_supported(const GemmArgs& a, int in_dtype, int out_dtype);
bool gemm_persist_pays(const GemmArgs& a, int mi);
int launch_gemm_persist(const GemmArgs& a, int mi, hipStream_t stream);

struct AttnArgs {
    const void* qkv;
    void* vt;
    const uint64_t* kbits;
    void* out;
    int B, S, H, heads, Spad, nw64;
    float scale_log2e;
    const void* qkv_lo = nullptr;
    float* lse2 = nullptr;
    float drop_p = 0.f;
    uint64_t drop_seed = 0, drop_key = 0;
    const Tuning* tune = nullptr;
};
struct AttnOutArgs {
    const void* qkv;
    const uint64_t* kbits;
    const void* wpk;
    const float* bias;
    const void* res;
    const float* ln_g;
    const float* ln_b;
    void* out;
    int B, S, H, heads, nw64;
    float scale_log2e, eps;
};
bool attn_out_ln_supported(int dtype, int H, int heads, int S);
int launch_attn_out_ln(const AttnOutArgs& a, hipStream_t stream);
struct AttnBwdArgs {
    const void* qkv;
    const void* dout;
    const float* lse2;
    const float* delta;
    const uint8_t* key_pad;
    void* dqkv;
    int B, S, H, heads;
    float scale_log2e, scale;
    float drop_p;
    uint64_t drop_seed, drop_key;
    const Tuning* tune = nullptr;
};
bool attention_bwd_supported(int dtype, int H, int heads);
int launch_attention_bwd(const AttnBwdArgs& a, int dtype, hipStream_t stream);
int launch_transpose_v(const AttnArgs& a, int dtype, hipStream_t stream);
int launch_split_hi_lo(const float* x, void* hi, void* lo, size_t n, hipStream_t stream);
int launch_attention(const AttnArgs& a, int dtype, hipStream_t stream);
bool attention_pipe_supported(const AttnArgs& a, int dtype);
int launch_attention_pipe(const AttnArgs& a, int variant, hipStream_t stream);

struct PredictorArgs {
    const void* x;
    const void* wpk;
    const float* dw_w = nullptr;
    const float* dw_b = nullptr;
    const void* wpk_lo = nullptr;
    const float* bias;
    const float* ln_g;
    const float* ln_b;
    const float* head_w;
    float head_b;
    const uint8_t* mask;
    float* pred;
    int B, S, H, nlayers, taps;
    float eps;
    void* be_y = nullptr;
    const float* be_bins = nullptr;
    const float* be_emb = nullptr;
    int be_nbins = 0;
    float be_std = 1.f, be_mean = 0.f;
    const float* be_pe = nullptr;
    const float* be_spk = nullptr;
};
bool predictor_fused_supported(int dtype, int H, int taps, int nlayers, int S);
size_t predictor_packed_bytes_per_layer(int taps = 3);
int launch_pack_predictor_weights(const void* w_layer , void* out_layer, hipStream_t stream, int taps = 3);
int launch_predictor_fused(const PredictorArgs& a, hipStream_t stream);
bool predictor_fused_x3_supported(int H, int taps, int nlayers, int S);
int launch_predictor_fused_x3(const PredictorArgs& a, hipStream_t stream);

struct VocConvArgs {
    const void* x;
    const void* w;
    const float* bias;
    const void* res;
    void* out;
    const int32_t* lengths;
    int len_scale;
    int B, S;
    int cin, cin_pad, n, taps, dil, pad;
    int wn;
    float in_slope;
    float scale;
    int accumulate;
    int in_fp32;
    int post;
    float out_slope = 1.f;
    const Tuning* tune = nullptr;
    int shift_from = 0;
};
struct VocResblockArgs {
    const void* x;
    void* out;
    const void* w;
    const float* bias;
    const int32_t* lengths;
    int len_scale;
    int B, S, C, taps, wn, npairs;
    int dil[3];
    float slope, scale;
    int accumulate;
    int x_act = 0;
    int out_act = 0;
    const Tuning* tune = nullptr;
};
struct LossArgs {
    const float* pred;
    const void* truth;
    const uint8_t* mask;
    void* ws;
    float* out;
    int64_t rows;
    int inner, kind, truth_kind;
};
struct SoftDtwArgs {
    const float* x;
    const float* y;
    float* out;
    int B, N, M, D;
    float gamma;
};
size_t soft_dtw_lds_bytes(int N, int M, int D);
int launch_soft_dtw(const SoftDtwArgs& a, hipStream_t stream);
size_t soft_dtw_grad_scratch_bytes(int B, int N, int M);
int launch_soft_dtw_grad(const SoftDtwArgs& a, float* grad_x, void* scratch, size_t scratch_bytes, hipStream_t stream);
size_t masked_loss_ws_bytes();
int launch_masked_loss(const LossArgs& a, hipStream_t stream);
int voc_resblock_mi16(const VocResblockArgs& a, int dtype);
int launch_vocoder_resblock(const VocResblockArgs& a, int dtype, hipStream_t stream);
int voc_steps_padded(int taps, int cin_pad, int dtype);
int launch_vocoder_conv(const VocConvArgs& a, int dtype, hipStream_t stream);

struct ConvertArgs {
    const void* src;
    void* dst;
    size_t n;
};
int launch_convert(const ConvertArgs& a, int src_dtype, int dst_dtype, hipStream_t stream);

struct LayerNormArgs {
    const void* x;
    const void* res;
    const float* gamma;
    const float* beta;
    void* y;
    const float* dot_w;
    float dot_b;
    const uint8_t* mask;
    float* pred;
    int M, H;
    float eps;
    const float* pre_stats = nullptr;
    int pre_parts = 0;
    const float* dot_b_dev = nullptr;
    float drop_p = 0.f;
    uint64_t drop_seed = 0, drop_key = 0;
};
int launch_layernorm(const LayerNormArgs& a, int dtype, hipStream_t stream);

int launch_rowstats_finish(const float* parts, int nparts, int ncols, float eps, float* out, int M, hipStream_t stream);
int launch_head_finish(const float* parts, const float* dots, int nparts, int ncols, float eps, float sum_gw, float cst, const uint8_t* mask, float* pred,
                       int M, hipStream_t stream);

struct DwConvArgs {
    const void* x;
    const float* w;
    const float* bias;
    void* y;
    int B, S, C, k, pad;
    const float* ln_stats = nullptr;
    const float* ln_g = nullptr;
    const float* ln_b = nullptr;
    int ln_parts = 0;
    float ln_eps = 1e-5f;
    int flip = 0;
};
int launch_dwconv(const DwConvArgs& a, int dtype, hipStream_t stream);

struct CwtArgs {
    const void* out_conv;
    const float* spec;
    int ld_spec;
    const uint8_t* mask;
    const float* ms_w;
    const float* ms_b;
    float* mean_std;
    float* pred;
    float* spec_out;
    int B, T, F;
};
int launch_cwt_head(const CwtArgs& a, int dtype, hipStream_t stream);

struct EmbedArgs {
    const int64_t* phones;
    const float* table;
    const float* pe;
    const float* spk;
    void* x;
    uint8_t* src_mask;
    int B, L, H, n_phones;
};
int launch_embed(const EmbedArgs& a, int dtype, hipStream_t stream);

struct SpkProjArgs {
    const float* dvec;
    const float* w;
    const float* b;
    float* spk;
    int B, H, Din;
};
int launch_spk_proj(const SpkProjArgs& a, hipStream_t stream);

struct MaskBitsArgs {
    const uint8_t* mask;
    uint64_t* bits;
    int B, S, nw64;
};
int launch_mask_bits(const MaskBitsArgs& a, hipStream_t stream);

struct DurationArgs {
    const float* dur_pred;
    const uint8_t* src_mask;
    const int32_t* forced;
    int32_t* dur;
    int32_t* cum;
    int32_t* totals;
    int32_t* guard;
    int B, L;
};
int launch_durations(const DurationArgs& a, hipStream_t stream);

struct RegulateArgs {
    const void* x;
    const int32_t* cum;
    const int32_t* totals;
    void* y;
    uint8_t* tgt_mask;
    int B, L, T, H;
};
int launch_regulate(const RegulateArgs& a, int dtype, hipStream_t stream);

struct BucketArgs {
    const void* x;
    const float* pred;
    const float* bins;
    const float* emb;
    int nbins;
    float std, mean;
    const float* pe;
    const float* spk;
    void* y;
    int32_t* idx_out;
    int B, T, H;
    const int32_t* forced_idx;
    int pred_per_utt = 0;
    const float* bucket_src = nullptr;
};
int launch_bucket_embed(const BucketArgs& a, int dtype, hipStream_t stream);

struct BGemmArgs {
    const void* A;
    const void* B;
    void* C;
    const float* bias = nullptr;
    int M = 0, N = 0, K = 0;
    long sAm = 0, sAk = 0;
    long sBk = 0, sBn = 0;
    long ldc = 0;
    int nb1 = 1, nb2 = 1;
    long sA1 = 0, sA2 = 0, sB1 = 0, sB2 = 0, sC1 = 0, sC2 = 0;
    float alpha = 1.f, beta = 0.f;
    int splitk = 1;
    float* ws = nullptr;
    int seg = 0;
    int taps = 1, Kin = 0;
    int a_shift0 = 0, a_shift_step = 0;
    long sBtap = 0;
    int b_shift0 = 0, b_shift_step = 0;
    const void* epi_p = nullptr;
    const float* epi_delta = nullptr;
    float drop_p = 0.f;
    uint64_t drop_seed = 0, drop_key = 0;
    int c_dtype = FS2_F32;
    int vecA = 0, vecB = 0;
    int xcd_remap = 0;
    const Tuning* tune = nullptr;
};
size_t bgemm_ws_bytes(const BGemmArgs& a);
bool bgemm_tn256_eligible(const BGemmArgs& a);
int launch_bgemm(const BGemmArgs& a, int dtype, hipStream_t stream);

struct LayerNormBwdArgs {
    const void* z;
    const void* res;
    const void* dy;
    const float* gamma;
    void* dz;
    float* part;
    int M, H, nparts;
    float eps;
    int relu_mask;
    float drop_p = 0.f;
    uint64_t drop_seed = 0, drop_key = 0;
    void* dzm = nullptr;
    float out_p = 0.f;
    uint64_t out_key = 0;
};
int layernorm_bwd_parts(int M);
int launch_layernorm_bwd(const LayerNormBwdArgs& a, int dtype, hipStream_t stream);

struct ColSumArgs {
    const void* x;
    float* out;
    float* ws;
    int M, N, ldx;
    int seg;
    int accumulate;
    float scale;
    float* out2 = nullptr;
    int n1 = 0;
    int accumulate2 = 0;
    const float* row_w = nullptr;
    const Tuning* tune = nullptr;
};
size_t col_sum_ws_bytes(int M, int N, int seg);
int launch_col_sum(const ColSumArgs& a, int dtype, hipStream_t stream);

struct SoftmaxArgs {
    const float* s;
    const void* p;
    void* out;
    const uint8_t* key_pad;
    int B, heads, S;
    float scale;
};
int launch_softmax_fwd(const SoftmaxArgs& a, int dtype, hipStream_t stream);
int launch_softmax_bwd(const SoftmaxArgs& a, int dtype, hipStream_t stream);

struct EwArgs {
    const void* a;
    const void* b;
    void* out;
    size_t n;
    float alpha, beta;
    int op;
};
int launch_ew(const EwArgs& a, int dtype, hipStream_t stream);

struct ScatterRowsArgs {
    const void* x;
    const int32_t* idx32;
    const int64_t* idx64;
    float* table;
    int R, H, V;
    int skip_row;
    float* ws = nullptr;
};
size_t scatter_rows_ws_bytes(int R, int H, int V);
int launch_scatter_rows(const ScatterRowsArgs& a, int dtype, hipStream_t stream);

struct RegulateBwdArgs {
    const void* dy;
    const int32_t* cum;
    void* dx;
    int B, L, T, H;
};
int launch_regulate_bwd(const RegulateBwdArgs& a, int dtype, hipStream_t stream);

struct LossBwdArgs {
    const float* pred;
    const void* truth;
    const uint8_t* mask;
    const float* stat;
    float* dpred;
    int64_t rows;
    int inner, kind, truth_kind;
    float alpha;
};
int launch_masked_loss_bwd(const LossBwdArgs& a, hipStream_t stream);

struct DwConvWgradArgs {
    const void* dy;
    const void* x;
    float* part;
    int B, S, C, k, pad;
};
int dwconv_wgrad_parts(int B, int S);
int launch_dwconv_wgrad(const DwConvWgradArgs& a, int dtype, hipStream_t stream);

struct FoldConv2Args {
    const float* G;
    const float* bg;
    const float* W21;
// ... 65 lines not shown
```

### lightningfastspeech2_amd/csrc/gemm_mfma.hip

```cpp
#include <string.h>

#include "fs2_common.h"
#include "fs2_kernels.h"

namespace fs2 {

static constexpr int BM = 128, BN = 128, ROWB = 128;
static constexpr int TILE_BYTES = BM * ROWB;

__device__ inline int swz(int row, int slot) { return row * ROWB + ((slot ^ (row & 7)) << 4); }

template <typename T, typename OutT, bool ZR = false>
__global__ __launch_bounds__(256) void gemm_conv_kernel(GemmArgs p) {
    extern __shared__ __attribute__((aligned(16))) unsigned char smem[];
    unsigned char* sX = smem;
    unsigned char* sW = smem + 2 * TILE_BYTES;
    constexpr int E16 = Num<T>::kPer16B;
    constexpr int KE = ROWB / (int)sizeof(T);

    const int tid = threadIdx.x, lane = tid & 63, wave = tid >> 6;
    const int tiles_n = (p.N + BN - 1) / BN;
    const int bm = blockIdx.x / tiles_n, bn = blockIdx.x % tiles_n;
    const int m0 = bm * BM, n0 = bn * BN;

// ... 1014 lines not shown
            __syncthreads();
            float2* red = (float2*)slab0;
#pragma unroll
            for (int mi = 0; mi < MI; ++mi) {
                const float s1 = group4_sum(a1[mi]), s2 = group4_sum(a2[mi]);
                if (fg == 0) red[wn * BMs + wm * (MI * 16) + mi * 16 + fr] = make_float2(s1, s2);
            }
            __syncthreads();
            for (int row = tid; row < BMs; row += 512) {
                const int t = t0 + row;
                if (t < S) {
                    const float2 q0 = red[row], q1 = red[BMs + row], q2 = red[2 * BMs + row], q3 = red[3 * BMs + row];
                    ((float2*)p.stats_out)[(rowbase + t) * (size_t)tiles_n + bn] =
                        make_float2((q0.x + q1.x) + (q2.x + q3.x), (q0.y + q1.y) + (q2.y + q3.y));
                }
            }
        }
        return;
    }
    const bool fulln = n0 + S_BN <= p.N;
    if (p.rs_stats) {
        if constexpr (sizeof(T) == 2 && sizeof(OutT) == 2 && !SPLIT) {
            if (fulln) store(BoolC<false>{}, BoolC<true>{}, BoolC<false>{}, BoolC<false>{}, BoolC<true>{});
            else store(BoolC<false>{}, BoolC<false>{}, BoolC<false>{}, BoolC<false>{}, BoolC<true>{});
        }
    } else if (p.gate) {
        if (fulln) store(BoolC<false>{}, BoolC<true>{}, BoolC<true>{}, BoolC<false>{}, BoolC<false>{});
        else store(BoolC<false>{}, BoolC<false>{}, BoolC<true>{}, BoolC<false>{}, BoolC<false>{});
    } else if (p.drop_p > 0.f) {
        if (fulln) store(BoolC<true>{}, BoolC<true>{}, BoolC<false>{}, BoolC<true>{}, BoolC<false>{});
        else store(BoolC<true>{}, BoolC<false>{}, BoolC<false>{}, BoolC<true>{}, BoolC<false>{});
    } else if (fulln) {
        if (p.relu) store(BoolC<true>{}, BoolC<true>{}, BoolC<false>{}, BoolC<false>{}, BoolC<false>{});
        else store(BoolC<false>{}, BoolC<true>{}, BoolC<false>{}, BoolC<false>{}, BoolC<false>{});
    } else {
        if (p.relu) store(BoolC<true>{}, BoolC<false>{}, BoolC<false>{}, BoolC<false>{}, BoolC<false>{});
        else store(BoolC<false>{}, BoolC<false>{}, BoolC<false>{}, BoolC<false>{}, BoolC<false>{});
    }
#else
    (void)p;
#endif
}

template <typename T, typename OutT, int MI, bool LN, bool SPLIT = false, bool DEFER = false>
static int launch_slab_t(const GemmArgs& a0, hipStream_t stream) {
    GemmArgs a = a0;
    a.xcd_remap = tuning_of(a0.tune).slab_xcd_remap;
    const int BMs = SlabCfg<MI>::BM;
    if (a.xcd_remap == 2) {
        const int tn = (a.N + S_BN - 1) / S_BN, rows = (a.M / a.S) * ((a.S + BMs - 1) / BMs);
        const bool ok = (tn == 4 || tn == 8 || tn == 16) && a.ksplit <= 1 && rows % (16 / tn) == 0 &&
                        (size_t)a.N * a.K * sizeof(T) > (size_t)3 << 20;
        if (!ok) a.xcd_remap = 1;
    }
    if constexpr (SPLIT) {
        if (a.taps > 1) {
            const int tiles = (a.M / a.S) * ((a.S + BMs - 1) / BMs) * ((a.N + S_BN - 1) / S_BN) * (a.ksplit > 1 ? a.ksplit : 1);
            hipLaunchKernelGGL((gemm_conv_slab_kernel<T, OutT, MI, LN, SPLIT, DEFER, true>), dim3(tiles), dim3(512), 0, stream, a);
            return hipGetLastError() == hipSuccess ? FS2_OK : FS2_ERR_HIP;
        }
    }
    if (a.taps == 1) a.S = a.M;
    const int tiles = (a.M / a.S) * ((a.S + BMs - 1) / BMs) * ((a.N + S_BN - 1) / S_BN) * (a.ksplit > 1 ? a.ksplit : 1);
    hipLaunchKernelGGL((gemm_conv_slab_kernel<T, OutT, MI, LN, SPLIT, DEFER>), dim3(tiles), dim3(512), 0, stream, a);
    return hipGetLastError() == hipSuccess ? FS2_OK : FS2_ERR_HIP;
}

static int presplit_on_the_fly(GemmArgs& a, hipStream_t stream, void** tmp) {
    hipStreamCaptureStatus cs = hipStreamCaptureStatusNone;
    if (hipStreamIsCapturing(stream, &cs) != hipSuccess || cs != hipStreamCaptureStatusNone) return FS2_ERR_STATE;
    const size_t bytes = (size_t)a.N * a.K * 4;
    if (hipMallocAsync(tmp, bytes, stream) != hipSuccess) return FS2_ERR_NOMEM;
    const int r = launch_presplit_pack((const float*)a.W, *tmp, (size_t)a.N * a.K, stream);
    a.W = *tmp;
    a.w_presplit = 1;
    return r;
}

template <int MI>
static int launch_slab_do(const GemmArgs& a, int in_dtype, int out_dtype, bool sp, hipStream_t stream) {
    if (a.ln_g) {
        if constexpr (MI <= 6) {
            if (a.N > S_BN) return FS2_ERR_SHAPE;
            if (in_dtype == FS2_F32 && out_dtype == FS2_F32)
                return sp ? launch_slab_t<float, float, MI, true, true>(a, stream) : launch_slab_t<float, float, MI, true>(a, stream);
            if (in_dtype == FS2_BF16 && out_dtype == FS2_BF16) return launch_slab_t<bf16, bf16, MI, true>(a, stream);
        }
        return FS2_ERR_SHAPE;
    }
    if (a.stats_out || a.epi_res) {
        if (a.epi_res && a.relu) return FS2_ERR_SHAPE;
        if constexpr (MI <= 6) {
            if (in_dtype == FS2_F32 && out_dtype == FS2_F32)
                return sp ? launch_slab_t<float, float, MI, false, true, true>(a, stream) : launch_slab_t<float, float, MI, false, false, true>(a, stream);
            if (in_dtype == FS2_BF16 && out_dtype == FS2_BF16) return launch_slab_t<bf16, bf16, MI, false, false, true>(a, stream);
        }
        return FS2_ERR_SHAPE;
    }
    if (in_dtype == FS2_F32 && out_dtype == FS2_F32)
        return sp ? launch_slab_t<float, float, MI, false, true>(a, stream) : launch_slab_t<float, float, MI, false>(a, stream);
    if (in_dtype == FS2_BF16 && out_dtype == FS2_BF16) return launch_slab_t<bf16, bf16, MI, false>(a, stream);
    if (in_dtype == FS2_BF16 && out_dtype == FS2_F32) return launch_slab_t<bf16, float, MI, false>(a, stream);
    return FS2_ERR_SHAPE;
}

template <int MI>
static int launch_slab(const GemmArgs& a_in, int in_dtype, int out_dtype, hipStream_t stream) {
    GemmArgs a = a_in;
    const bool sp = a.split || tuning_of(a.tune).split_f32;
    void* tmp = nullptr;
    if (in_dtype == FS2_F32 && out_dtype == FS2_F32 && sp && !a.w_presplit) {
        const int r = presplit_on_the_fly(a, stream, &tmp);
        if (r != FS2_OK) { if (tmp) (void)hipFreeAsync(tmp, stream); return r; }
    }
    const int r = launch_slab_do<MI>(a, in_dtype, out_dtype, sp, stream);
    if (tmp) (void)hipFreeAsync(tmp, stream);
    return r;
}

template <typename T, typename OutT, bool ZR = false>
static int launch_t(const GemmArgs& a, hipStream_t stream) {
    static bool attr_set = false;
    const size_t smem = 4 * TILE_BYTES;
    if (!attr_set) {
        hipError_t e = hipFuncSetAttribute((const void*)gemm_conv_kernel<T, OutT, ZR>,
                                           hipFuncAttributeMaxDynamicSharedMemorySize, (int)smem);
        if (e != hipSuccess) return FS2_ERR_HIP;
        attr_set = true;
    }
    const int tiles = ((a.M + BM - 1) / BM) * ((a.N + BN - 1) / BN);
    hipLaunchKernelGGL((gemm_conv_kernel<T, OutT, ZR>), dim3(tiles), dim3(256), smem, stream, a);
    return hipGetLastError() == hipSuccess ? FS2_OK : FS2_ERR_HIP;
}

static int launch_gemm_plain(const GemmArgs& a, int in_dtype, int out_dtype, hipStream_t stream, bool* fused);

int launch_gemm(const GemmArgs& a, int in_dtype, int out_dtype, hipStream_t stream) {
    const Tuning& tn = tuning_of(a.tune);
    const int g_gemm_variant = tn.gemm_variant, g_gemm_wres = tn.gemm_wres;
    if (a.head_out) {
        if (a.ln_g || !gemm_head_supported(a, in_dtype, out_dtype)) return FS2_ERR_SHAPE;
        return launch_gemm_persist(a, 6, stream);
    }
    if (!a.ln_g && a.drop_p > 0.f) {
        if (!a.relu || a.gate || a.stats_out || a.epi_res || a.ksplit > 1 || a.zero_rows || g_gemm_variant != 0 || a.N < 192 || a.M % a.S ||
            !(a.taps & 1) || in_dtype != out_dtype)
            return FS2_ERR_SHAPE;
        return launch_gemm_plain(a, in_dtype, out_dtype, stream, nullptr);
    }
    if (!a.ln_g) {
        if (g_gemm_wres && g_gemm_variant == 0 && a.ksplit <= 1 && gemm_wres_supported(a, in_dtype, out_dtype, g_gemm_wres == 2)) return launch_gemm_wres(a, stream);
        return launch_gemm_plain(a, in_dtype, out_dtype, stream, nullptr);
    }
    bool fused = false;
    if (a.z_out && a.N > S_BN) return FS2_ERR_SHAPE;
    if (a.drop_p > 0.f && (a.N > S_BN || !a.z_out)) return FS2_ERR_SHAPE;
    if (a.N <= S_BN && in_dtype == out_dtype) {
        const int r = launch_gemm_plain(a, in_dtype, out_dtype, stream, &fused);
        if (r != FS2_OK || fused) return r;
    }
    if (a.z_out) return FS2_ERR_SHAPE;
    if (!a.ln_tmp || in_dtype != out_dtype) return FS2_ERR_ARG;
    GemmArgs g = a;
    g.ln_g = nullptr;
    g.C = a.ln_tmp;
    const int r = launch_gemm_plain(g, in_dtype, out_dtype, stream, nullptr);
    if (r != FS2_OK) return r;
    LayerNormArgs l;
    l.x = a.ln_tmp; l.res = a.res; l.gamma = a.ln_g; l.beta = a.ln_b; l.y = a.C;
    l.dot_w = a.dot_w; l.dot_b = a.dot_b; l.mask = a.mask; l.pred = a.pred;
    l.M = a.M; l.H = a.N; l.eps = a.ln_eps;
    return launch_layernorm(l, out_dtype, stream);
}

static int launch_gemm_plain(const GemmArgs& a, int in_dtype, int out_dtype, hipStream_t stream, bool* fused) {
    const Tuning& tn_ = tuning_of(a.tune);
    const int g_gemm_variant = tn_.gemm_variant;
    const bool g_split_f32 = tn_.split_f32 != 0;
    if (a.M <= 0 || a.N <= 0) return FS2_OK;
    const int ke = in_dtype == FS2_BF16 ? 64 : 32;
    const int e16 = in_dtype == FS2_BF16 ? 8 : 4;
    if (a.K % ke || a.Cin % ke || a.ldx % e16 || a.K != a.taps * a.Cin) return FS2_ERR_SHAPE;
    if (a.ldc % 4) return FS2_ERR_SHAPE;
    if (a.rs_stats && a.N < 192) {
        if (fused || a.relu || a.gate || a.stats_out || a.epi_res || a.C_lo || a.ksplit > 1 || a.drop_p > 0.f || !a.rs_wg || a.taps != 1 || in_dtype != FS2_BF16)
            return FS2_ERR_SHAPE;
        if (out_dtype == FS2_F32) return a.zero_rows ? launch_t<bf16, float, true>(a, stream) : launch_t<bf16, float>(a, stream);
        if (out_dtype == FS2_BF16 && !a.zero_rows) return launch_t<bf16, bf16>(a, stream);
        return FS2_ERR_SHAPE;
    }
    if (a.zero_rows) {
        if (fused) return FS2_ERR_SHAPE;
        if (in_dtype == FS2_F32 && out_dtype == FS2_F32) return launch_t<float, float, true>(a, stream);
        if (in_dtype == FS2_BF16 && out_dtype == FS2_F32) return launch_t<bf16, float, true>(a, stream);
        return FS2_ERR_SHAPE;
    }
    if (a.rs_stats && (fused || a.relu || a.gate || a.stats_out || a.epi_res || a.zero_rows || a.C_lo || a.ksplit > 1 || a.drop_p > 0.f || g_gemm_variant == 1 ||
                       g_gemm_variant == 2 || !a.rs_wg || !(a.M % a.S == 0 && (a.taps & 1)) || a.N < 192 || in_dtype != FS2_BF16 ||
                       out_dtype != FS2_BF16))
        return FS2_ERR_SHAPE;
    if (a.gate && (fused || a.relu || a.stats_out || a.epi_res || g_gemm_variant != 0 || a.N < 192 || a.M % a.S || !(a.taps & 1) ||
                   in_dtype != out_dtype))
        return FS2_ERR_SHAPE;
    const int variant = g_gemm_variant;
    const bool slab_ok = a.M % a.S == 0 && (a.taps & 1);
    const int ksp = a.ksplit > 1 ? a.ksplit : 1;
    if (a.w_presplit && (!(a.split || g_split_f32) || variant != 0 || !slab_ok || a.N < 192 || in_dtype != FS2_F32 || a.ksplit > 1 || a.zero_rows))
        return FS2_ERR_SHAPE;
    if (a.C_lo && (fused || a.gate || a.stats_out || a.epi_res || a.zero_rows || a.ksplit > 1 || a.drop_p > 0.f || variant != 0 || !slab_ok ||
                   a.N < 192 || in_dtype != FS2_F32 || out_dtype != FS2_F32))
        return FS2_ERR_SHAPE;
    if (ksp > 1 && (fused || a.bias || a.relu || a.gate || a.stats_out || a.epi_res || a.zero_rows || out_dtype != FS2_F32 || !slab_ok ||
                    a.N < 192 || (a.Cin / ke) % ksp || (variant != 0 && (variant < 3 || variant > 7))))
        return FS2_ERR_SHAPE;
    if (variant >= 6 && variant <= 7 && slab_ok) {
        if (fused) *fused = true;
        if (variant == 6) return launch_slab<1>(a, in_dtype, out_dtype, stream);
        return launch_slab<2>(a, in_dtype, out_dtype, stream);
    }
    if (variant >= 3 && variant <= 5 && slab_ok && !(fused && variant == 5)) {
        if (fused) *fused = true;
        if (variant == 3) return launch_slab<4>(a, in_dtype, out_dtype, stream);
        if (variant == 4 || a.stats_out || a.epi_res) return launch_slab<6>(a, in_dtype, out_dtype, stream);
        return launch_slab<8>(a, in_dtype, out_dtype, stream);
    }
    if (fused && variant != 0) return FS2_OK;
    if (variant == 2) {
        if (a.stats_out || a.epi_res) return FS2_ERR_SHAPE;
        if (in_dtype == FS2_F32 && out_dtype == FS2_F32) return launch_glds_t<float, float>(a, stream);
        if (in_dtype == FS2_BF16 && out_dtype == FS2_BF16) return launch_glds_t<bf16, bf16>(a, stream);
        if (in_dtype == FS2_BF16 && out_dtype == FS2_F32) return launch_glds_t<bf16, float>(a, stream);
        return FS2_ERR_SHAPE;
    }
    if (variant == 0 && slab_ok && a.N >= 192) {
        const int S = a.taps == 1 ? a.M : a.S, nutt = a.M / S, tn = (a.N + S_BN - 1) / S_BN;
        int best = 0;
        long best_cost = 0, best_rows = 0;
        static const int kHeights[5] = {1, 2, 4, 6, 8};
        for (int hi = 0; hi < 5; ++hi) {
            const int mi = kHeights[hi];
            if (fused && mi > 6) continue;
            if ((a.stats_out || a.epi_res) && mi > 6) continue;
            const long bm = mi * 32, tm = (S + bm - 1) / bm;
            const long tiles = (long)nutt * tm * tn * ksp;
            long cost = ((tiles + 255) / 256) * (bm + 40);
            if (a.K / ksp >= 4096) cost = cost > tiles ? cost : tiles;
            if (!best || cost < best_cost) { best = mi; best_cost = cost; best_rows = (long)nutt * tm * bm; }
        }
        if (best_rows <= 2L * a.M || a.C_lo || a.w_presplit || a.rs_stats) {
            if (!fused && tn_.gemm_persist && gemm_persist_supported(a, in_dtype, out_dtype, best) && gemm_persist_pays(a, best))
                return launch_gemm_persist(a, best, stream);
            if (fused) *fused = true;
            if (best == 1) return launch_slab<1>(a, in_dtype, out_dtype, stream);
            if (best == 2) return launch_slab<2>(a, in_dtype, out_dtype, stream);
            if (best == 4) return launch_slab<4>(a, in_dtype, out_dtype, stream);
            if (best == 6) return launch_slab<6>(a, in_dtype, out_dtype, stream);
            return launch_slab<8>(a, in_dtype, out_dtype, stream);
        }
    }
    if (fused) return FS2_OK;
    if (a.stats_out || a.epi_res || a.gate || ksp > 1 || a.drop_p > 0.f || a.rs_stats) return FS2_ERR_SHAPE;
    if (in_dtype == FS2_F32 && out_dtype == FS2_F32) return launch_t<float, float>(a, stream);
    if (in_dtype == FS2_BF16 && out_dtype == FS2_BF16) return launch_t<bf16, bf16>(a, stream);
    if (in_dtype == FS2_BF16 && out_dtype == FS2_F32) return launch_t<bf16, float>(a, stream);
    return FS2_ERR_SHAPE;
}

bool gemm_presplit_eligible(int N, int K) { return N >= 192 && K % 32 == 0; }

__global__ __launch_bounds__(256) void presplit_pack_kernel(const float* w, unsigned char* out, size_t npairs) {
    const size_t i = (size_t)blockIdx.x * 256 + threadIdx.x;
    if (i >= npairs) return;
    const size_t chunk = i >> 2;
    const int sl = (int)(i & 3);
    const uint4 c0 = *(const uint4*)(w + chunk * 32 + 4 * sl), c1 = *(const uint4*)(w + chunk * 32 + 16 + 4 * sl);
    uint4 h, l;
    split_bf16x3(c0, c1, h, l);
    *(uint4*)(out + chunk * 128 + sl * 16) = h;
    *(uint4*)(out + chunk * 128 + (4 + sl) * 16) = l;
}
int launch_presplit_pack(const float* w, void* out, size_t n_values, hipStream_t stream) {
    if (n_values % 32) return FS2_ERR_SHAPE;
    if (!n_values) return FS2_OK;
    const size_t np = n_values / 8;
    hipLaunchKernelGGL(presplit_pack_kernel, dim3((unsigned)((np + 255) / 256)), dim3(256), 0, stream, w, (unsigned char*)out, np);
    return hipGetLastError() == hipSuccess ? FS2_OK : FS2_ERR_HIP;
}

template <typename OutT>
__global__ __launch_bounds__(256) void split_k_reduce_kernel(const float* __restrict__ part, OutT* __restrict__ out, size_t n, int ksplit,
                                                             int accumulate) {
    const size_t i = ((size_t)blockIdx.x * 256 + threadIdx.x) * 4;
    if (i >= n) return;
    float4 a = *(const float4*)(part + i);
    for (int s = 1; s < ksplit; ++s) {
        const float4 b = *(const float4*)(part + (size_t)s * n + i);
        a.x += b.x; a.y += b.y; a.z += b.z; a.w += b.w;
    }
    if constexpr (sizeof(OutT) == 4) {
        float4* o = (float4*)(out + i);
        if (accumulate) { const float4 c = *o; a.x += c.x; a.y += c.y; a.z += c.z; a.w += c.w; }
        *o = a;
    } else {
        uint2* o = (uint2*)(out + i);
        if (accumulate) {
            const uint2 c = *o;
// ... 37 lines not shown
```

### lightningfastspeech2_amd/csrc/gemm_wres.hip

```cpp
#include <hip/hip_runtime.h>

#include <type_traits>

#include "fs2_common.h"
#include "fs2_kernels.h"

namespace fs2 {
namespace {

constexpr int WR_K = 256, WR_ROWB = WR_K * 2, WR_MI = 3, WR_RT = 2 * WR_MI * 16;
constexpr int WR_TILEB = WR_RT * WR_ROWB;
__attribute__((unused)) constexpr int WR_NDMA = WR_TILEB / 1024 / 8;

__device__ __attribute__((unused)) inline int wr_wcol(int ni, int fgq) { return (ni >> 1) * 32 + fgq * 8 + (ni & 1) * 4; }

#ifdef FS2_WRES_PROBE
__device__ unsigned long long g_wres_stamps[2][64];
#define WRES_STAMP(i)                                                                                                      \
    do {                                                                                                                   \
        if (blockIdx.x == 0 && (threadIdx.x == 0 || threadIdx.x == 448) && (i) < 64)                                        \
            g_wres_stamps[threadIdx.x ? 1 : 0][i] = __builtin_amdgcn_s_memtime();                                           \
    } while (0)
#else
#define WRES_STAMP(i) do { } while (0)
#endif

__global__ __launch_bounds__(512) void gemm_wres_kernel(GemmArgs p, int ncol, int nrg, int tiles) {
#if defined(__HIP_DEVICE_COMPILE__)
    __shared__ __attribute__((aligned(16))) unsigned char xs0[WR_TILEB];
    __shared__ __attribute__((aligned(16))) unsigned char xs1[WR_TILEB];
    const int tid = threadIdx.x, lane = tid & 63;
    const int wave = __builtin_amdgcn_readfirstlane(tid >> 6);
    const int wm = wave >> 2, wn = wave & 3, fr = lane & 15, fg = lane >> 4;
    const int xcd = blockIdx.x & 7, q = blockIdx.x >> 3;
    const int ct = q % ncol, rg = (q / ncol) * 8 + xcd;
    if (rg >= nrg) return;
    const int tbeg = (int)((long)rg * tiles / nrg), tend = (int)((long)(rg + 1) * tiles / nrg);
    if (tbeg >= tend) return;
    const int n0 = ct * 256;
    WRES_STAMP(0);

    uint4 fw[8][4];
    {
        const __amdgpu_buffer_rsrc_t wrs =
            __builtin_amdgcn_make_buffer_rsrc((void*)p.W, 0, (unsigned)((size_t)p.N * WR_K * 2), 0x00020000);
        auto wswz = [](int row) { return ((row >> 1) & 1) | (((row >> 3) & 3) << 1); };
        auto stage = [&](int cc0) {
#pragma unroll
            for (int c = 0; c < 2; ++c)
#pragma unroll
                for (int i = 0; i < 4; ++i) {
                    const int P = (i * 8 + wave) * 64 + lane, row = P >> 3, ps = P & 7;
                    const unsigned voff = (unsigned)((n0 + row) * (WR_K * 2) + (cc0 + c) * 128 + ((ps ^ wswz(row)) << 4));
                    __builtin_amdgcn_raw_ptr_buffer_load_lds(wrs, (__attribute__((address_space(3))) void*)((c ? xs1 : xs0) + (i * 8 + wave) * 1024),
                                                             16, voff, 0, 0, 0);
                }
            dma_drain();
            __syncthreads();
#pragma unroll
            for (int c = 0; c < 2; ++c)
#pragma unroll
                for (int ni = 0; ni < 4; ++ni) {
                    const int wrow = wn * 64 + wr_wcol(ni, fr >> 2) + (fr & 3);
#pragma unroll
                    for (int h = 0; h < 2; ++h)
                        fw[(cc0 + c) * 2 + h][ni] = *(const uint4*)((c ? xs1 : xs0) + wrow * 128 + (((h * 4 + fg) ^ wswz(wrow)) << 4));
                }
            __syncthreads();
        };
        stage(0);
        stage(2);
    }
    __shared__ __attribute__((aligned(16))) float sbias[256];
    if (tid < 256) sbias[tid] = p.bias ? p.bias[n0 + tid] : 0.f;
    __syncthreads();

    const __amdgpu_buffer_rsrc_t xrs =
        __builtin_amdgcn_make_buffer_rsrc((void*)p.X, 0, (unsigned)(((size_t)(p.M - 1) * p.ldx + WR_K) * 2), 0x00020000);
    auto issue_piece = [&](auto BUF, int t, int k, bool live) {
        unsigned char* const dst = decltype(BUF)::value ? xs1 : xs0;
        const int c = k * 8 + wave, i = 2 * c + (lane >> 5), ps = lane & 31, m = t * WR_RT + i;
        const int ls = (ps & 16) | ((((ps & 7) ^ (i & 7)) << 1) | ((ps >> 3) & 1));
        const unsigned voff = (live && m < p.M) ? (unsigned)m * (unsigned)(p.ldx * 2) + (unsigned)(ls << 4) : 0xFFFFF000u;
        __builtin_amdgcn_raw_ptr_buffer_load_lds(xrs, (__attribute__((address_space(3))) void*)(dst + c * 1024), 16, voff, 0, 0, 0);
    };
    auto issue = [&](auto BUF, int t) {
#pragma unroll
        for (int k = 0; k < WR_NDMA; ++k) issue_piece(BUF, t, k, true);
    };
    const int arow = (wm * (WR_MI * 16) + fr) * WR_ROWB;
    const int acx = (((fg & 1) << 3) | ((fg >> 1) ^ (fr & 7))) << 4;
    auto compute = [&](auto BUF, f32x4_t (&acc)[4][WR_MI], auto side) {
        const unsigned char* const xs = decltype(BUF)::value ? xs1 : xs0;
        uint4 fx[2][WR_MI];
        auto ldx = [&](uint4 (&f)[WR_MI], int ks) {
#pragma unroll
            for (int mi = 0; mi < WR_MI; ++mi)
                f[mi] = *(const uint4*)(xs + arow + mi * 16 * WR_ROWB + (acx ^ ((((ks & 3) << 1) | ((ks >> 2) << 4)) << 4)));
        };
        ldx(fx[0], 0);
#pragma unroll
        for (int ks = 0; ks < 8; ++ks) {
            if (ks + 1 < 8) ldx(fx[(ks + 1) & 1], ks + 1);
#pragma unroll
            for (int ni = 0; ni < 4; ++ni) {
#pragma unroll
                for (int mi = 0; mi < WR_MI; ++mi) Mma16<bf16>::step(fw[ks][ni], fx[ks & 1][mi], acc[ni][mi]);
                if (ni == 0) side(ks);
            }
        }
    };
    auto store_piece = [&](int t, int mi, int j, const uint4& q) {
        const int m = t * WR_RT + wm * (WR_MI * 16) + mi * 16 + fr;
        if (m < p.M) *(uint4*)((bf16*)p.C + (size_t)m * p.ldc + n0 + wn * 64 + j * 32 + fg * 8) = q;
    };
    using B0 = std::integral_constant<int, 0>;
    using B1 = std::integral_constant<int, 1>;
    WRES_STAMP(1);
    issue(B0{}, tbeg);
    auto tile = [&](auto CUR, auto NXT, int t) {
        WRES_STAMP(4 + (t - tbeg) * 5);
        if (t == tbeg) __builtin_amdgcn_s_waitcnt(0x0F70);
        else __builtin_amdgcn_s_waitcnt(0x0F70 | 6);
        WRES_STAMP(5 + (t - tbeg) * 5);
        __syncthreads();
        WRES_STAMP(6 + (t - tbeg) * 5);
        const bool has_next = t + 1 < tend;
        auto side = [&](int ks) {
            if (ks < WR_NDMA) issue_piece(NXT, t + 1, ks, has_next);
        };
        WRES_STAMP(7 + (t - tbeg) * 5);
        f32x4_t acc[4][WR_MI];
#pragma unroll
        for (int a = 0; a < 4; ++a)
#pragma unroll
            for (int b = 0; b < WR_MI; ++b) acc[a][b] = (f32x4_t){0.f, 0.f, 0.f, 0.f};
        compute(CUR, acc, side);
        WRES_STAMP(8 + (t - tbeg) * 5);
#pragma unroll
        for (int mi = 0; mi < WR_MI; ++mi) {
#pragma unroll
            for (int j = 0; j < 2; ++j) {
                const float4 b0 = *(const float4*)(sbias + wn * 64 + j * 32 + fg * 8), b1 = *(const float4*)(sbias + wn * 64 + j * 32 + fg * 8 + 4);
                const float bv[8] = {b0.x, b0.y, b0.z, b0.w, b1.x, b1.y, b1.z, b1.w};
                float v[8];
#pragma unroll
                for (int r = 0; r < 8; ++r) {
                    v[r] = acc[2 * j + (r >> 2)][mi][r & 3] + bv[r];
                    if (p.relu) v[r] = fmaxf(v[r], 0.f);
                }
                store_piece(t, mi, j, make_uint4(pack_bf16x2(v[0], v[1]), pack_bf16x2(v[2], v[3]), pack_bf16x2(v[4], v[5]), pack_bf16x2(v[6], v[7])));
            }
        }
    };
    for (int t = tbeg; t < tend; t += 2) {
        tile(B0{}, B1{}, t);
        if (t + 1 < tend) tile(B1{}, B0{}, t + 1);
    }
#else
    (void)p; (void)ncol; (void)nrg; (void)tiles;
#endif
}

}


static int wres_row_groups(int ncol, int tiles) {
    int nrg = (256 / ncol) & ~7;
    if (nrg < 8) nrg = 8;
    if (nrg > ((tiles + 7) & ~7)) nrg = (tiles + 7) & ~7;
    return nrg;
}

bool gemm_wres_supported(const GemmArgs& a, int in_dtype, int out_dtype, bool force) {
    if (a.N >= 256 && a.N % 256 == 0 && !force) {
        const int tiles = (a.M + WR_RT - 1) / WR_RT;
        if (tiles < 3 * wres_row_groups(a.N / 256, tiles)) return false;
    }
    return in_dtype == FS2_BF16 && out_dtype == FS2_BF16 && a.taps == 1 && a.K == WR_K && a.Cin == WR_K && a.N >= 256 && a.N % 256 == 0 &&
           a.N <= 2048 && a.M > 0 && !a.res && !a.ln_g && !a.dot_w && !a.z_out && !a.epi_res && !a.stats_out && !a.gate && !a.zero_rows &&
           !a.split && !a.rs_stats && a.ldx % 8 == 0 && a.ldc % 8 == 0 && (size_t)a.M * a.ldx * 2 < 0xFFFFF000ull && (size_t)a.M * a.ldc * 2 < 0xFFFFF000ull;
}

int launch_gemm_wres(const GemmArgs& a, hipStream_t stream) {
    const int ncol = a.N / 256, tiles = (a.M + WR_RT - 1) / WR_RT, nrg = wres_row_groups(ncol, tiles);
    hipLaunchKernelGGL(gemm_wres_kernel, dim3((unsigned)(nrg * ncol)), dim3(512), 0, stream, a, ncol, nrg, tiles);
    return hipGetLastError() == hipSuccess ? FS2_OK : FS2_ERR_HIP;
}

}

#ifdef FS2_WRES_PROBE
extern "C" int fs2_dbg_wres_stamps(unsigned long long* out ) {
    if (hipDeviceSynchronize() != hipSuccess) return -1;
    return hipMemcpyFromSymbol(out, HIP_SYMBOL(fs2::g_wres_stamps), sizeof(unsigned long long) * 128) == hipSuccess ? 0 : -2;
}
#endif
```

### lightningfastspeech2_amd/csrc/predictor_fused.hip

```cpp
#include "fs2_common.h"
#include "fs2_kernels.h"
#include <type_traits>

namespace fs2 {

namespace {
constexpr int PF_H = 256, PF_TAPS = 3, PF_KB = PF_H / 32;
constexpr int PF_STEP_U4 = 8 * 2 * 64;
constexpr int PF_ROWB = PF_H * 2;
#ifndef FS2_PF_PREFETCH
#define FS2_PF_PREFETCH 1
#endif
constexpr bool PF_PREFETCH = FS2_PF_PREFETCH;
#ifndef FS2_PF_FENCE
#define FS2_PF_FENCE 1
#endif
#ifndef FS2_PF_RING
#define FS2_PF_RING 3
#endif
constexpr int PF_RING = FS2_PF_RING;
static_assert(PF_RING == 3 || PF_RING == 4, "ring depth 3 or 4");
#if FS2_PF_FENCE
#define PF_FENCE() __builtin_amdgcn_sched_barrier(0)
#else
#define PF_FENCE() do { } while (0)
#endif

}

__global__ void pack_predictor_weights_kernel(const bf16* __restrict__ W, uint4* __restrict__ out, int taps) {
    const int idx = blockIdx.x * blockDim.x + threadIdx.x;
    if (idx >= taps * PF_KB * PF_STEP_U4) return;
    const int lane = idx & 63, ni = (idx >> 6) & 1, wv = (idx >> 7) & 7, step = idx >> 10;
    const int tap = step / PF_KB, kb = step % PF_KB, fr = lane & 15, fg = lane >> 4;
    const int ch = wv * 32 + (fr >> 2) * 8 + ni * 4 + (fr & 3);
    out[idx] = *(const uint4*)(W + (size_t)ch * (taps * PF_H) + tap * PF_H + kb * 32 + fg * 8);
}

template <int MI16, int NWV, int MINW, bool X3 = false, bool DW = false>
__global__ __launch_bounds__(NWV * 64, MINW) void predictor_fused_kernel(PredictorArgs p) {
#if defined(__HIP_DEVICE_COMPILE__)
    static_assert(!(X3 && DW), "no split-arithmetic depth-wise form");
    constexpr int R = MI16 * 16, HFA = (MI16 + 1) / 2;
    constexpr int NFR = PF_H / (NWV * 16), NP = NFR / 2;
    constexpr int PLANE = (R + 2) * PF_ROWB;
    constexpr int TAPS = DW ? 1 : PF_TAPS, STEPS = TAPS * PF_KB;
    constexpr int RING = (X3 || DW) ? 4 : PF_RING;
    __shared__ __attribute__((aligned(16))) unsigned char slab[(X3 ? 2 : 1) * PLANE];
    __shared__ float red[2][NWV * R];

    const int tid = threadIdx.x, lane = tid & 63;
    const int wv = __builtin_amdgcn_readfirstlane(tid >> 6);
    const int fr = lane & 15, fg = lane >> 4;
    const int S = p.S, nl = p.nlayers, halo = nl - 1, V = R - 2 * halo;
    const int tiles = (S + V - 1) / V;
    const int ub = blockIdx.x / tiles, tm = blockIdx.x % tiles;
    const int t0 = tm * V - halo;

    if constexpr (X3) {
        const float* xu = (const float*)p.x + (size_t)ub * S * PF_H;
        constexpr int NIT = ((R + 2) * 32 + NWV * 64 - 1) / (NWV * 64);
        uint4 c0[NIT], c1[NIT];
#pragma unroll
        for (int u = 0; u < NIT; ++u) {
            int sidx = tid + u * NWV * 64;
            sidx = sidx < (R + 2) * 32 ? sidx : (R + 2) * 32 - 1;
            const int i = sidx >> 5, ps = sidx & 31, t = t0 - 1 + i;
            const int ls = (ps & 16) | ((((ps & 7) ^ (i & 7)) << 1) | ((ps >> 3) & 1));
            const int tc = t < 0 ? 0 : (t < S ? t : S - 1);
            c0[u] = *(const uint4*)(xu + (size_t)tc * PF_H + ls * 8);
            c1[u] = *(const uint4*)(xu + (size_t)tc * PF_H + ls * 8 + 4);
        }
#pragma unroll
        for (int u = 0; u < NIT; ++u) {
            const int sidx = tid + u * NWV * 64;
            if (sidx < (R + 2) * 32) {
                const int i = sidx >> 5, ps = sidx & 31, t = t0 - 1 + i;
                uint4 hi, lo;
                split_bf16x3(c0[u], c1[u], hi, lo);
                if (t < 0 || t >= S) hi = lo = make_uint4(0u, 0u, 0u, 0u);
                *(uint4*)(slab + i * PF_ROWB + (ps << 4)) = hi;
                *(uint4*)(slab + PLANE + i * PF_ROWB + (ps << 4)) = lo;
            }
        }
    } else
    {
        const bf16* xu = (const bf16*)p.x + (size_t)ub * S * PF_H;
        const __amdgpu_buffer_rsrc_t xrs =
            __builtin_amdgcn_make_buffer_rsrc((void*)xu, 0, (unsigned)((size_t)S * PF_ROWB), 0x00020000);
        constexpr int NCH = (R + 2) / 2;
#pragma unroll
        for (int k = 0; k < (NCH + NWV - 1) / NWV; ++k) {
            const int c = k * NWV + wv;
            if (c < NCH) {
                const int i = 2 * c + (lane >> 5), ps = lane & 31, t = t0 - 1 + i;
                const int ls = (ps & 16) | ((((ps & 7) ^ (i & 7)) << 1) | ((ps >> 3) & 1));
                const unsigned voff = (t >= 0 && t < S) ? (unsigned)(t * PF_ROWB + (ls << 4)) : 0xFFFFF000u;
                __builtin_amdgcn_raw_ptr_buffer_load_lds(xrs, (__attribute__((address_space(3))) void*)(slab + c * 1024),
                                                         16, voff, 0, 0, 0);
            }
        }
    }

    const uint4* __restrict__ wbase = (const uint4*)p.wpk + wv * NFR * 64 + lane;
    const uint4* __restrict__ wbase_lo = X3 ? (const uint4*)p.wpk_lo + wv * NFR * 64 + lane : nullptr;
    const int total = nl * STEPS;
    auto loadB = [&](uint4 (&b)[NFR], int g) {
        g = g < total ? g : total - 1;
#if defined(FS2_PF_PROBE) && (FS2_PF_PROBE & 1)
        g &= 1;
#endif
#pragma unroll
        for (int ni = 0; ni < NFR; ++ni) b[ni] = wbase[(size_t)g * PF_STEP_U4 + ni * 64];
    };
    auto loadBL = [&](uint4 (&b)[NFR], int g) {
        g = g < total ? g : total - 1;
#pragma unroll
        for (int ni = 0; ni < NFR; ++ni) b[ni] = wbase_lo[(size_t)g * PF_STEP_U4 + ni * 64];
    };
    uint4 bw[RING][NFR], bwl[X3 ? RING : 1][NFR];
    loadB(bw[0], 0);
    loadB(bw[1], 1);
    if constexpr (RING == 4) loadB(bw[2], 2);
    if constexpr (X3) {
        loadBL(bwl[0], 0);
        loadBL(bwl[1], 1);
        if constexpr (RING == 4) loadBL(bwl[2], 2);
    }

    dma_drain();
    __syncthreads();

    const int n0 = wv * (NFR * 16) + fg * 8;
    for (int l = 0; l < nl; ++l) {
#if defined(FS2_PF_PROBE) && (FS2_PF_PROBE & 4)
        if constexpr (false) {
#else
        if constexpr (DW) {
#endif
            static_assert(NWV * 64 == 256 && R % 8 == 0, "depth-wise pass: 32 slots x 8 row groups");
            constexpr int RPT = R / 8;
            int tid_d = tid;
            asm volatile("" : "+v"(tid_d));
            const int L = tid_d & 31, i0 = 1 + (tid_d >> 5) * RPT;
            f32x2_t wt[3][4], bs[4];
            {
                const float* wp = p.dw_w + (size_t)l * 3 * PF_H + L * 8;
#pragma unroll
                for (int tp = 0; tp < 3; ++tp) {
                    const float4 a = *(const float4*)(wp + tp * PF_H), b = *(const float4*)(wp + tp * PF_H + 4);
                    wt[tp][0] = (f32x2_t){a.x, a.y}; wt[tp][1] = (f32x2_t){a.z, a.w}; wt[tp][2] = (f32x2_t){b.x, b.y}; wt[tp][3] = (f32x2_t){b.z, b.w};
                }
                const float* bp = p.dw_b + (size_t)l * PF_H + L * 8;
                const float4 a = *(const float4*)bp, b = *(const float4*)(bp + 4);
                bs[0] = (f32x2_t){a.x, a.y}; bs[1] = (f32x2_t){a.z, a.w}; bs[2] = (f32x2_t){b.x, b.y}; bs[3] = (f32x2_t){b.z, b.w};
            }
            const SlabSwizzle sw(PF_ROWB / 16);
            auto rowp = [&](int i) { return slab + i * PF_ROWB + (sw.slot(L, i) << 4); };
            auto unpack = [](const uint4& v, f32x2_t (&f)[4]) {
                const unsigned u[4] = {v.x, v.y, v.z, v.w};
#pragma unroll
                for (int q = 0; q < 4; ++q) f[q] = (f32x2_t){__uint_as_float(u[q] << 16), __uint_as_float(u[q] & 0xffff0000u)};
            };
            uint4 raw[RPT + 2];
#pragma unroll
            for (int j = 0; j < RPT + 2; ++j) raw[j] = *(const uint4*)rowp(i0 - 1 + j);
            uint4 o[RPT];
            f32x2_t xa[4], xb[4], xc[4];
            unpack(raw[0], xa);
            unpack(raw[1], xb);
#pragma unroll
            for (int j = 0; j < RPT; ++j) {
                unpack(raw[j + 2], xc);
                unsigned w4[4];
#pragma unroll
                for (int q = 0; q < 4; ++q) {
                    f32x2_t a = wt[0][q] * xa[q];
                    a = __builtin_elementwise_fma(wt[1][q], xb[q], a);
                    a = __builtin_elementwise_fma(wt[2][q], xc[q], a);
                    a = a + bs[q];
                    w4[q] = pack_bf16x2(a.x, a.y);
                    xa[q] = xb[q];
                    xb[q] = xc[q];
                }
                o[j] = make_uint4(w4[0], w4[1], w4[2], w4[3]);
            }
            __syncthreads();
#pragma unroll
            for (int j = 0; j < RPT; ++j) *(uint4*)rowp(i0 + j) = o[j];
            __syncthreads();
        }
        f32x4_t acc[NFR][MI16];
        f32x4_t bq[NFR];
#pragma unroll
        for (int j = 0; j < NP; ++j) {
            const float* bias = p.bias + l * PF_H + n0 + 32 * j;
            const float4 b0 = *(const float4*)bias, b1 = *(const float4*)(bias + 4);
            bq[2 * j] = (f32x4_t){b0.x, b0.y, b0.z, b0.w};
            bq[2 * j + 1] = (f32x4_t){b1.x, b1.y, b1.z, b1.w};
        }
        auto mma = [&](auto FIRSTKB, const uint4& bfrag, const uint4& afrag, int ni, f32x4_t& a) {
            if constexpr (decltype(FIRSTKB)::value)
                a = __builtin_amdgcn_mfma_f32_16x16x32_bf16(*(const bf16x8_t*)&bfrag, *(const bf16x8_t*)&afrag, bq[ni], 0, 0, 0);
            else
                Mma16<bf16>::step(bfrag, afrag, a);
        };
        auto mma3 = [&](auto FIRSTKB, const uint4& bh, const uint4& bl, const uint4& ah, const uint4& al, int ni, f32x4_t& a) {
            mma(FIRSTKB, bl, ah, ni, a);
            Mma16<bf16>::step(bh, al, a);
            Mma16<bf16>::step(bh, ah, a);
        };
        auto tap = [&](int tp, auto FIRST) {
            constexpr bool first = decltype(FIRST)::value;
            const int i0 = fr + tp + (DW ? 1 : 0);
            const unsigned char* arow_p = slab + i0 * PF_ROWB;
            const int acx = (((fg & 1) << 3) | ((fg >> 1) ^ (i0 & 7))) << 4;
            constexpr int HFB = MI16 - HFA;
            auto loadA = [&](uint4 (&fx)[HFA], int kb, int hf) {
                const int m0 = hf * HFA, cnt = hf ? HFB : HFA;
#pragma unroll
                for (int mi = 0; mi < HFA; ++mi)
                    if (mi < cnt) fx[mi] = *(const uint4*)(arow_p + (m0 + mi) * 16 * PF_ROWB + (acx ^ ((((kb & 3) << 1) | ((kb >> 2) << 4)) << 4)));
            };
            auto loadAL = [&](uint4 (&fx)[HFA], int kb, int hf) {
                const int m0 = hf * HFA, cnt = hf ? HFB : HFA;
#pragma unroll
                for (int mi = 0; mi < HFA; ++mi)
                    if (mi < cnt) fx[mi] = *(const uint4*)(arow_p + PLANE + (m0 + mi) * 16 * PF_ROWB + (acx ^ ((((kb & 3) << 1) | ((kb >> 2) << 4)) << 4)));
            };
            auto kblock = [&](auto KB0, int kb, uint4 (&fxa)[HFA], uint4 (&fxb)[HFA], uint4 (&fla)[HFA], uint4 (&flb)[HFA]) {
                const int rs = (tp * PF_KB + kb) % RING, rn = (tp * PF_KB + kb + RING - 1) % RING;
                loadB(bw[rn], (l * TAPS + tp) * PF_KB + kb + RING - 1);
                if constexpr (X3) {
                    loadBL(bwl[rn], (l * TAPS + tp) * PF_KB + kb + RING - 1);
#pragma unroll
                    for (int mi = 0; mi < MI16; ++mi) {
                        const int c = kb * MI16 + mi, cur = c & 1, nxt = cur ^ 1;
                        const int nmi = mi + 1 < MI16 ? mi + 1 : 0, nkb = mi + 1 < MI16 ? kb : kb + 1;
                        if (nkb < PF_KB) {
                            const int off = nmi * 16 * PF_ROWB + (acx ^ ((((nkb & 3) << 1) | ((nkb >> 2) << 4)) << 4));
                            fxa[nxt] = *(const uint4*)(arow_p + off);
                            fla[nxt] = *(const uint4*)(arow_p + PLANE + off);
                        }
                        PF_FENCE();
#pragma unroll
                        for (int ni = 0; ni < NFR; ++ni) mma3(KB0, bw[rs][ni], bwl[rs][ni], fxa[cur], fla[cur], ni, acc[ni][mi]);
                        PF_FENCE();
                    }
                    (void)fxb; (void)flb;
                } else if constexpr (MINW == 1 || PF_PREFETCH) {
// ... 53 lines not shown

#if defined(FS2_PF_PROBE) && (FS2_PF_PROBE & 2)
        {
            f32x4_t s4 = {0.f, 0.f, 0.f, 0.f};
#pragma unroll
            for (int ni = 0; ni < NFR; ++ni)
#pragma unroll
                for (int m = 0; m < MI16; ++m) s4 += acc[ni][m];
            if (s4.x + s4.y + s4.z + s4.w == 12345.678f) red[0][tid] = s4.x;
            __syncthreads();
            continue;
        }
#endif
        auto relu = [](float x) { float y; asm("v_max_f32 %0, 0, %1" : "=v"(y) : "v"(x)); return y; };
        int lane_e = lane;
        asm volatile("" : "+v"(lane_e));
        const int fr = lane_e & 15, fg = lane_e >> 4;
        const int n0 = wv * (NFR * 16) + fg * 8;
        const float invn = 1.0f / (float)PF_H;
        float mean[MI16], rstd[MI16];
#pragma unroll
        for (int m = 0; m < MI16; ++m) {
            f32x2_t s2 = {0.f, 0.f};
#pragma unroll
            for (int ni = 0; ni < NFR; ++ni) {
                f32x4_t& a = acc[ni][m];
                a = (f32x4_t){relu(a[0]), relu(a[1]), relu(a[2]), relu(a[3])};
                s2 += a.xy;
                s2 += a.zw;
            }
            const float sm = group4_sum(s2.x + s2.y);
            if (fg == 0) red[0][wv * R + m * 16 + fr] = sm;
        }
        __syncthreads();
#pragma unroll
        for (int m = 0; m < MI16; ++m) {
            const int row = m * 16 + fr;
            float t8 = 0.f;
#pragma unroll
            for (int w = 0; w < NWV; ++w) t8 += red[0][w * R + row];
            mean[m] = t8 * invn;
            const f32x2_t mn2 = {mean[m], mean[m]};
            f32x2_t q2 = {0.f, 0.f};
#pragma unroll
            for (int ni = 0; ni < NFR; ++ni) {
                f32x4_t& a = acc[ni][m];
                const f32x2_t d0 = a.xy - mn2, d1 = a.zw - mn2;
                a = (f32x4_t){d0.x, d0.y, d1.x, d1.y};
                q2 = __builtin_elementwise_fma(d0, d0, q2);
                q2 = __builtin_elementwise_fma(d1, d1, q2);
            }
            const float q = group4_sum(q2.x + q2.y);
            if (fg == 0) red[1][wv * R + row] = q;
        }
        __syncthreads();
#pragma unroll
        for (int m = 0; m < MI16; ++m) {
            const int row = m * 16 + fr;
            float t8 = 0.f;
#pragma unroll
            for (int w = 0; w < NWV; ++w) t8 += red[1][w * R + row];
            rstd[m] = __builtin_amdgcn_rsqf(t8 * invn + p.eps);
        }
        const bool last = l + 1 == nl;
        float dsum[MI16];
#pragma unroll
        for (int m = 0; m < MI16; ++m) dsum[m] = 0.f;
#pragma unroll
        for (int j = 0; j < NP; ++j) {
            const int n = n0 + 32 * j;
            f32x2_t gg[4], ee[4], hw[4];
            {
                const float* gam = p.ln_g + l * PF_H + n;
                const float* bet = p.ln_b + l * PF_H + n;
                const float4 g0 = *(const float4*)gam, g1 = *(const float4*)(gam + 4);
                const float4 e0 = *(const float4*)bet, e1 = *(const float4*)(bet + 4);
                gg[0] = (f32x2_t){g0.x, g0.y}; gg[1] = (f32x2_t){g0.z, g0.w}; gg[2] = (f32x2_t){g1.x, g1.y}; gg[3] = (f32x2_t){g1.z, g1.w};
                ee[0] = (f32x2_t){e0.x, e0.y}; ee[1] = (f32x2_t){e0.z, e0.w}; ee[2] = (f32x2_t){e1.x, e1.y}; ee[3] = (f32x2_t){e1.z, e1.w};
                if (last) {
                    const float4 h0 = *(const float4*)(p.head_w + n), h1 = *(const float4*)(p.head_w + n + 4);
                    hw[0] = (f32x2_t){h0.x, h0.y}; hw[1] = (f32x2_t){h0.z, h0.w}; hw[2] = (f32x2_t){h1.x, h1.y}; hw[3] = (f32x2_t){h1.z, h1.w};
                }
            }
#pragma unroll
            for (int m = 0; m < MI16; ++m) {
                const int row = m * 16 + fr, t = t0 + row, i = row + 1;
                const f32x2_t rs2 = {rstd[m], rstd[m]};
                f32x2_t y[4];
#pragma unroll
                for (int r = 0; r < 4; ++r) {
                    const f32x4_t& a = acc[2 * j + (r >> 1)][m];
                    y[r] = __builtin_elementwise_fma((r & 1 ? a.zw : a.xy) * rs2, gg[r], ee[r]);
                }
                if (last) {
                    f32x2_t d2 = {dsum[m], 0.f};
#pragma unroll
                    for (int r = 0; r < 4; ++r) d2 = __builtin_elementwise_fma(y[r], hw[r], d2);
                    dsum[m] = d2.x + d2.y;
                } else {
                    const bool inside = t >= 0 && t < S;
                    const uint4 o = inside ? make_uint4(pack_bf16x2(y[0].x, y[0].y), pack_bf16x2(y[1].x, y[1].y),
                                                        pack_bf16x2(y[2].x, y[2].y), pack_bf16x2(y[3].x, y[3].y))
                                           : make_uint4(0u, 0u, 0u, 0u);
                    const int so = i * PF_ROWB + (SlabSwizzle(PF_ROWB / 16).slot(n >> 3, i) << 4);
                    *(uint4*)(slab + so) = o;
                    if constexpr (X3) {
                        const unsigned hw4[4] = {o.x, o.y, o.z, o.w};
                        unsigned lw[4];
#pragma unroll
                        for (int r = 0; r < 4; ++r)
                            lw[r] = pack_bf16x2(y[r].x - __uint_as_float(hw4[r] << 16), y[r].y - __uint_as_float(hw4[r] & 0xffff0000u));
                        *(uint4*)(slab + PLANE + so) = inside ? make_uint4(lw[0], lw[1], lw[2], lw[3]) : make_uint4(0u, 0u, 0u, 0u);
                    }
                }
            }
        }
        if (!last) {
            __syncthreads();
            continue;
        }
#pragma unroll
        for (int m = 0; m < MI16; ++m) {
            const float d = group4_sum(dsum[m]);
            if (fg == 0) red[0][wv * R + m * 16 + fr] = d;
        }
        __syncthreads();
        if (tid < R) {
            const int row = tid, t = t0 + row;
            if (row >= halo && row < R - halo && t < S) {
                float d = p.head_b;
#pragma unroll
                for (int w = 0; w < NWV; ++w) d += red[0][w * R + row];
                const size_t o = (size_t)ub * S + t;
                d = (p.mask && p.mask[o]) ? 0.f : d;
                p.pred[o] = d;
                red[1][row] = d;
            }
        }
    }
    int lane_t = lane;
    asm volatile("" : "+v"(lane_t));
    if (p.be_y) {
        __syncthreads();
        constexpr int EB = 8;
        const int nedge = p.be_nbins - 1, nb = (nedge + 63) >> 6;
        float bl[8];
#pragma unroll
        for (int k = 0; k < 8; ++k) {
            const int i = lane_t + 64 * k;
            bl[k] = i < nedge ? p.be_bins[i] : __builtin_inff();
        }
        using XT = typename std::conditional<X3, float, bf16>::type;
        using XV = typename std::conditional<X3, float4, uint2>::type;
        const XT* xg = (const XT*)p.x + (size_t)ub * S * PF_H + lane_t * 4;
        XT* yg = (XT*)p.be_y + (size_t)ub * S * PF_H + lane_t * 4;
        const float* spr = p.be_spk ? p.be_spk + (size_t)ub * PF_H + lane_t * 4 : nullptr;
        float4 sp4 = make_float4(0.f, 0.f, 0.f, 0.f);
        if (spr) sp4 = *(const float4*)spr;
        for (int base = halo + wv * EB; base < R - halo; base += NWV * EB) {
            XV xv[EB];
            float4 ev[EB], pv[EB];
            bool okr[EB];
#pragma unroll
            for (int j = 0; j < EB; ++j) {
                const int row = base + j, t = t0 + row;
                okr[j] = row < R - halo && t < S;
                const int rc = okr[j] ? row : halo, tc = okr[j] ? t : t0 + halo;
                const float v = mul_then_add(red[1][rc], p.be_std, p.be_mean);
                int lo = 0;
#pragma unroll
                for (int k = 0; k < 8; ++k)
                    if (k < nb) lo += __popcll(__ballot(bl[k] < v));
                if (v != v) lo = nedge;
                xv[j] = *(const XV*)(xg + (size_t)tc * PF_H);
                ev[j] = *(const float4*)(p.be_emb + (size_t)lo * PF_H + lane_t * 4);
                if (p.be_pe) pv[j] = *(const float4*)(p.be_pe + (size_t)tc * PF_H + lane_t * 4);
            }
#pragma unroll
            for (int j = 0; j < EB; ++j) {
                if (!okr[j]) continue;
                float v[4];
                if constexpr (X3) {
                    v[0] = xv[j].x; v[1] = xv[j].y; v[2] = xv[j].z; v[3] = xv[j].w;
                } else {
                    v[0] = __uint_as_float(xv[j].x << 16); v[1] = __uint_as_float(xv[j].x & 0xffff0000u);
                    v[2] = __uint_as_float(xv[j].y << 16); v[3] = __uint_as_float(xv[j].y & 0xffff0000u);
                }
                const float e4[4] = {ev[j].x, ev[j].y, ev[j].z, ev[j].w};
#pragma unroll
                for (int i = 0; i < 4; ++i) v[i] = __fadd_rn(v[i], e4[i]);
                if (p.be_pe) {
                    const float q4[4] = {pv[j].x, pv[j].y, pv[j].z, pv[j].w};
#pragma unroll
                    for (int i = 0; i < 4; ++i) v[i] = __fadd_rn(v[i], q4[i]);
                }
                if (spr) {
                    const float q4[4] = {sp4.x, sp4.y, sp4.z, sp4.w};
#pragma unroll
                    for (int i = 0; i < 4; ++i) v[i] = __fadd_rn(v[i], q4[i]);
                }
                if constexpr (X3) *(float4*)(yg + (size_t)(t0 + base + j) * PF_H) = make_float4(v[0], v[1], v[2], v[3]);
                else *(uint2*)(yg + (size_t)(t0 + base + j) * PF_H) = make_uint2(pack_bf16x2(v[0], v[1]), pack_bf16x2(v[2], v[3]));
            }
        }
    }
#else
    (void)p;
#endif
}

#ifdef FS2_PRED_PROBE
__device__ unsigned long long g_pred_stamps[64];
#define PRED_STAMP(i) do { if (blockIdx.x == 0 && threadIdx.x == 0) g_pred_stamps[i] = __builtin_amdgcn_s_memtime(); } while (0)
#else
#define PRED_STAMP(i) do { } while (0)
#endif
bool predictor_fused_supported(int dtype, int H, int taps, int nlayers, int S) {
    return dtype == FS2_BF16 && H == PF_H && taps == PF_TAPS && nlayers >= 1 && nlayers <= 16 && S >= 1 &&
           (size_t)S * PF_ROWB < 0xFFFFF000ull;
}

int launch_pack_predictor_weights(const void* w_layer, void* out_layer, hipStream_t stream, int taps) {
    if (taps != 1 && taps != PF_TAPS) return FS2_ERR_SHAPE;
    const int n = taps * PF_KB * PF_STEP_U4;
    hipLaunchKernelGGL(pack_predictor_weights_kernel, dim3((n + 255) / 256), dim3(256), 0, stream, (const bf16*)w_layer,
                       (uint4*)out_layer, taps);
    return hipGetLastError() == hipSuccess ? FS2_OK : FS2_ERR_HIP;
}

size_t predictor_packed_bytes_per_layer(int taps) { return (size_t)taps * PF_KB * PF_STEP_U4 * 16; }

bool predictor_fused_x3_supported(int H, int taps, int nlayers, int S) {
    return H == PF_H && taps == PF_TAPS && nlayers >= 1 && nlayers <= 16 && S >= 1 && 112 - 2 * (nlayers - 1) >= 32;
}
int launch_predictor_fused_x3(const PredictorArgs& a, hipStream_t stream) {
    if (!predictor_fused_x3_supported(a.H, a.taps, a.nlayers, a.S) || !a.wpk_lo) return FS2_ERR_SHAPE;
    if (a.be_y && (a.be_y == a.x || !a.be_bins || !a.be_emb || a.be_nbins < 2 || a.be_nbins - 1 > 512)) return FS2_ERR_ARG;
    if (a.B <= 0) return FS2_OK;
    const int halo2 = 2 * (a.nlayers - 1);
    auto tiles = [&](int R) { return (long)a.B * ((a.S + (R - halo2) - 1) / (R - halo2)); };
    hipLaunchKernelGGL((predictor_fused_kernel<7, 4, 1, true>), dim3((unsigned)tiles(112)), dim3(256), 0, stream, a);
    return hipGetLastError() == hipSuccess ? FS2_OK : FS2_ERR_HIP;
}

int launch_predictor_fused(const PredictorArgs& a, hipStream_t stream) {
    if (!predictor_fused_supported(FS2_BF16, a.H, a.taps, a.nlayers, a.S)) return FS2_ERR_SHAPE;
    if (a.B <= 0) return FS2_OK;
    const int halo2 = 2 * (a.nlayers - 1);
    if (112 - halo2 < 32) return FS2_ERR_SHAPE;
    auto tiles = [&](int R) { return (long)a.B * ((a.S + (R - halo2) - 1) / (R - halo2)); };
    if (a.be_y && (a.be_y == a.x || !a.be_bins || !a.be_emb || a.be_nbins < 2 || a.be_nbins - 1 > 512)) return FS2_ERR_ARG;
    if ((a.dw_w != nullptr) != (a.dw_b != nullptr)) return FS2_ERR_ARG;
    if (((uintptr_t)a.x | (uintptr_t)a.wpk | (uintptr_t)a.bias | (uintptr_t)a.ln_g | (uintptr_t)a.ln_b | (uintptr_t)a.head_w | (uintptr_t)a.dw_w |
         (uintptr_t)a.dw_b | (uintptr_t)a.be_y | (uintptr_t)a.be_emb | (uintptr_t)a.be_pe | (uintptr_t)a.be_spk) & 15)
        return FS2_ERR_ARG;
    const bool small = tiles(112) < 200 && 64 - halo2 >= 32;
    if (a.dw_w) {
        if (small) hipLaunchKernelGGL((predictor_fused_kernel<4, 4, 2, false, true>), dim3((unsigned)tiles(64)), dim3(256), 0, stream, a);
        else hipLaunchKernelGGL((predictor_fused_kernel<7, 4, 2, false, true>), dim3((unsigned)tiles(112)), dim3(256), 0, stream, a);
    } else if (small) {
        hipLaunchKernelGGL((predictor_fused_kernel<4, 4, 2>), dim3((unsigned)tiles(64)), dim3(256), 0, stream, a);
    } else {
        hipLaunchKernelGGL((predictor_fused_kernel<7, 4, 2>), dim3((unsigned)tiles(112)), dim3(256), 0, stream, a);
    }
    return hipGetLastError() == hipSuccess ? FS2_OK : FS2_ERR_HIP;
}

}
```

### lightningfastspeech2_amd/csrc/rowops.hip

```cpp
#include "fs2_common.h"
#include "fs2_kernels.h"

namespace fs2 {

template <typename T> __device__ inline void load4(const T* p, float* f);
template <> __device__ inline void load4<float>(const float* p, float* f) {
    const float4 v = *(const float4*)p;
    f[0] = v.x; f[1] = v.y; f[2] = v.z; f[3] = v.w;
}
template <> __device__ inline void load4<bf16>(const bf16* p, float* f) {
    const uint2 v = *(const uint2*)p;
    f[0] = __uint_as_float(v.x << 16); f[1] = __uint_as_float(v.x & 0xffff0000u);
    f[2] = __uint_as_float(v.y << 16); f[3] = __uint_as_float(v.y & 0xffff0000u);
}
template <typename T> __device__ inline void store4(T* p, const float* f);
template <> __device__ inline void store4<float>(float* p, const float* f) {
    *(float4*)p = make_float4(f[0], f[1], f[2], f[3]);
}
template <> __device__ inline void store4<bf16>(bf16* p, const float* f) {
    *(uint2*)p = make_uint2(pack_bf16x2(f[0], f[1]), pack_bf16x2(f[2], f[3]));
}

template <typename T, int NV>
__global__ __launch_bounds__(256) void layernorm_kernel(LayerNormArgs p) {
// ... 401 lines not shown
    if (a.B <= 0 || a.nw64 <= 0) return FS2_OK;
    hipLaunchKernelGGL(mask_bits_kernel, dim3(a.nw64, a.B), dim3(64), 0, stream, a);
    return hipGetLastError() == hipSuccess ? FS2_OK : FS2_ERR_HIP;
}

__device__ inline int dur_from_pred(float p) {
    const float v = rintf(__fsub_rn(expf(p), 1.0f));
    return v > 0.f ? (int)v : 0;
}

__global__ __launch_bounds__(256) void durations_kernel(DurationArgs p) {
    __shared__ int red[2][4];
    __shared__ int wsum[4];
    __shared__ int guard_s;
    const int b = blockIdx.x, tid = threadIdx.x, lane = tid & 63, wave = tid >> 6;
    const float* dp = p.dur_pred + (size_t)b * p.L;
    const uint8_t* mk = p.src_mask + (size_t)b * p.L;
    const int32_t* forced = p.forced ? p.forced + (size_t)b * p.L : nullptr;
    int guard = 0;
    if (!forced) {
        int sd = 0, nv = 0;
        for (int l = tid; l < p.L; l += 256) {
            if (!mk[l]) { sd += dur_from_pred(dp[l]); nv += 1; }
        }
#pragma unroll
        for (int o = 32; o > 0; o >>= 1) { sd += __shfl_xor(sd, o, 64); nv += __shfl_xor(nv, o, 64); }
        if (lane == 0) { red[0][wave] = sd; red[1][wave] = nv; }
        __syncthreads();
        if (tid == 0) {
            const int s = red[0][0] + red[0][1] + red[0][2] + red[0][3];
            const int n = red[1][0] + red[1][1] + red[1][2] + red[1][3];
            guard_s = s <= n / 2;
        }
        __syncthreads();
        guard = guard_s;
    }
    int running = 0;
    for (int base = 0; base < p.L; base += 256) {
        const int l = base + tid;
        int d = 0;
        if (l < p.L) {
            if (forced) d = forced[l];
            else d = (guard && !mk[l]) ? 1 : dur_from_pred(dp[l]);
            if (d < 0) d = 0;
        }
        int inc = d;
#pragma unroll
        for (int o = 1; o < 64; o <<= 1) {
            const int n = __shfl_up(inc, o, 64);
            if (lane >= o) inc += n;
        }
        __syncthreads();
        if (lane == 63) wsum[wave] = inc;
        __syncthreads();
        int off = running;
        for (int w = 0; w < wave; ++w) off += wsum[w];
        if (l < p.L) {
            p.dur[(size_t)b * p.L + l] = d;
            p.cum[(size_t)b * p.L + l] = off + inc;
        }
        running += wsum[0] + wsum[1] + wsum[2] + wsum[3];
    }
    if (tid == 0) {
        p.totals[b] = running;
        p.guard[b] = guard;
    }
}

int launch_durations(const DurationArgs& a, hipStream_t stream) {
    if (a.B <= 0) return FS2_OK;
    hipLaunchKernelGGL(durations_kernel, dim3(a.B), dim3(256), 0, stream, a);
    return hipGetLastError() == hipSuccess ? FS2_OK : FS2_ERR_HIP;
}

constexpr int RG_ROWS = 16, RG_MAXC = 16;
template <typename T>
__global__ __launch_bounds__(256) void regulate_kernel(RegulateArgs p) {
    const int lane = threadIdx.x & 63;
    const int tb = (blockIdx.x * 4 + (threadIdx.x >> 6)) * RG_ROWS, b = blockIdx.y;
    if (tb >= p.T) return;
    const int total = p.totals[b];
    const int32_t* cum = p.cum + (size_t)b * p.L;
    const int nvec = p.H * (int)sizeof(T) / 16;
    const bool fast = p.L <= 64 * RG_MAXC;
    int32_t cl[RG_MAXC];
    if (fast) {
#pragma unroll
        for (int k = 0; k < RG_MAXC; ++k) {
            const int i = lane + 64 * k;
            cl[k] = i < p.L ? cum[i] : 0x7fffffff;
        }
    }
    const int nc = (p.L + 63) / 64;
    const bool pair = nvec <= 32;
    const int half = lane >> 5, hl = lane & 31;
    for (int r = 0; r < RG_ROWS; r += pair ? 2 : 1) {
        if (tb + r >= p.T) break;
        int lo_of[2] = {0, 0};
        bool in_of[2] = {false, false};
#pragma unroll
        for (int q = 0; q < 2; ++q) {
            const int t = tb + r + q;
            if (q == 1 && !pair) break;
            if (t >= p.T) break;
            in_of[q] = t < total;
            if (lane == 0) p.tgt_mask[(size_t)b * p.T + t] = t >= total;
            if (t < total) {
                int lo = 0;
                if (fast) {
#pragma unroll
                    for (int k = 0; k < RG_MAXC; ++k)
                        if (k < nc) lo += __popcll(__ballot(cl[k] <= t));
                } else {
                    int hi = p.L;
                    while (lo < hi) {
                        const int mid = (lo + hi) >> 1;
                        if (cum[mid] > t) hi = mid; else lo = mid + 1;
                    }
                }
                lo_of[q] = lo;
            }
        }
        if (pair) {
            const int t = tb + r + half;
            if (t < p.T && hl < nvec) {
                uint4* dst = (uint4*)((T*)p.y + ((size_t)b * p.T + t) * p.H);
                const bool in = half ? in_of[1] : in_of[0];
                const int lo = half ? lo_of[1] : lo_of[0];
                dst[hl] = in ? ((const uint4*)((const T*)p.x + ((size_t)b * p.L + lo) * p.H))[hl] : make_uint4(0, 0, 0, 0);
            }
        } else {
            const int t = tb + r;
            uint4* dst = (uint4*)((T*)p.y + ((size_t)b * p.T + t) * p.H);
            if (in_of[0]) {
                const uint4* src = (const uint4*)((const T*)p.x + ((size_t)b * p.L + lo_of[0]) * p.H);
                for (int i = lane; i < nvec; i += 64) dst[i] = src[i];
            } else {
                for (int i = lane; i < nvec; i += 64) dst[i] = make_uint4(0, 0, 0, 0);
            }
        }
    }
}

int launch_regulate(const RegulateArgs& a, int dtype, hipStream_t stream) {
    if (a.B <= 0 || a.T <= 0) return FS2_OK;
    const int esz = dtype == FS2_BF16 ? 2 : 4;
    if ((a.H * esz) % 16) return FS2_ERR_SHAPE;
    const dim3 grid((a.T + 4 * RG_ROWS - 1) / (4 * RG_ROWS), a.B), block(256);
    if (dtype == FS2_BF16) hipLaunchKernelGGL(regulate_kernel<bf16>, grid, block, 0, stream, a);
    else hipLaunchKernelGGL(regulate_kernel<float>, grid, block, 0, stream, a);
    return hipGetLastError() == hipSuccess ? FS2_OK : FS2_ERR_HIP;
}

constexpr int BE_ROWS = 8, BE_MAXB = 8;
template <typename T, int NV>
__global__ __launch_bounds__(256) void bucket_embed_kernel(BucketArgs p) {
    const int lane = threadIdx.x & 63;
    const int row0 = (blockIdx.x * 4 + (threadIdx.x >> 6)) * BE_ROWS;
    const int M = p.B * p.T;
    if (row0 >= M) return;
    const int nedge = p.nbins - 1;
    const bool fast = nedge <= 64 * BE_MAXB;
    float bl[BE_MAXB];
    if (p.pred && fast) {
#pragma unroll
        for (int k = 0; k < BE_MAXB; ++k) {
            const int i = lane + 64 * k;
            bl[k] = i < nedge ? p.bins[i] : INFINITY;
        }
    }
    const int nb = (nedge + 63) / 64;
    for (int r = 0; r < BE_ROWS; ++r) {
        const int row = row0 + r;
        if (row >= M) break;
        const int b = row / p.T, t = row % p.T;
        const float* e = nullptr;
        if (p.pred) {
            const float src = p.bucket_src ? p.bucket_src[row] : p.pred[p.pred_per_utt ? b : row];
            const float v = mul_then_add(src, p.std, p.mean);
            int lo = 0;
            if (fast) {
#pragma unroll
                for (int k = 0; k < BE_MAXB; ++k)
                    if (k < nb) lo += __popcll(__ballot(bl[k] < v));
            } else {
                int hi = nedge;
                while (lo < hi) {
                    const int mid = (lo + hi) >> 1;
                    if (p.bins[mid] < v) lo = mid + 1; else hi = mid;
                }
            }
            if (v != v) lo = nedge;
            if (p.forced_idx) {
                lo = p.forced_idx[row];
                lo = lo < 0 ? 0 : (lo >= p.nbins ? p.nbins - 1 : lo);
            }
            if (lane == 0 && p.idx_out) p.idx_out[row] = lo;
            e = p.emb + (size_t)lo * p.H;
        }
        const T* x = (const T*)p.x + (size_t)row * p.H;
        T* y = (T*)p.y + (size_t)row * p.H;
        const float* pe = p.pe ? p.pe + (size_t)t * p.H : nullptr;
        const float* sp = p.spk ? p.spk + (size_t)b * p.H : nullptr;
        if constexpr (NV > 0) {
            float v[NV][4], ae[NV][4], ap[NV][4], as[NV][4];
#pragma unroll
            for (int i = 0; i < NV; ++i) {
                const int c = (i * 64 + lane) * 4;
                if (c < p.H) {
                    load4<T>(x + c, v[i]);
                    if (e) load4<float>(e + c, ae[i]);
                    if (pe) load4<float>(pe + c, ap[i]);
                    if (sp) load4<float>(sp + c, as[i]);
                }
            }
#pragma unroll
            for (int i = 0; i < NV; ++i) {
                const int c = (i * 64 + lane) * 4;
                if (c < p.H) {
#pragma unroll
                    for (int k = 0; k < 4; ++k) {
                        if (e) v[i][k] = __fadd_rn(v[i][k], ae[i][k]);
                        if (pe) v[i][k] = __fadd_rn(v[i][k], ap[i][k]);
                        if (sp) v[i][k] = __fadd_rn(v[i][k], as[i][k]);
                    }
                    store4<T>(y + c, v[i]);
                }
            }
        } else
        for (int c = lane * 4; c < p.H; c += 256) {
            float v[4], a[4];
            load4<T>(x + c, v);
            if (e) {
                load4<float>(e + c, a);
#pragma unroll
                for (int i = 0; i < 4; ++i) v[i] = __fadd_rn(v[i], a[i]);
            }
            if (pe) {
                load4<float>(pe + c, a);
#pragma unroll
                for (int i = 0; i < 4; ++i) v[i] = __fadd_rn(v[i], a[i]);
            }
            if (sp) {
                load4<float>(sp + c, a);
#pragma unroll
                for (int i = 0; i < 4; ++i) v[i] = __fadd_rn(v[i], a[i]);
            }
            store4<T>(y + c, v);
        }
    }
}

int launch_bucket_embed(const BucketArgs& a, int dtype, hipStream_t stream) {
    if (a.B * a.T <= 0) return FS2_OK;
    if (a.H % 4) return FS2_ERR_SHAPE;
    const dim3 grid((a.B * a.T + 4 * BE_ROWS - 1) / (4 * BE_ROWS)), block(256);
    switch (a.H <= 1024 ? (a.H + 255) / 256 : 0) {
#define FS2_BE(NVV)                                                                                             \
    case NVV:                                                                                                   \
        if (dtype == FS2_BF16) hipLaunchKernelGGL((bucket_embed_kernel<bf16, NVV>), grid, block, 0, stream, a); \
        else hipLaunchKernelGGL((bucket_embed_kernel<float, NVV>), grid, block, 0, stream, a);                  \
        break;
        FS2_BE(0) FS2_BE(1) FS2_BE(2) FS2_BE(3) FS2_BE(4)
#undef FS2_BE
    }
    return hipGetLastError() == hipSuccess ? FS2_OK : FS2_ERR_HIP;
}

__device__ inline float block_sum_256(float v, float* sh) {
    v = wave_sum(v);
    __syncthreads();
    if ((threadIdx.x & 63) == 0) sh[threadIdx.x >> 6] = v;
    __syncthreads();
    return (sh[0] + sh[1]) + (sh[2] + sh[3]);
}

template <typename T>
__global__ __launch_bounds__(256) void cwt_mean_std_kernel(CwtArgs p) {
    __shared__ float sh[4];
    const int b = blockIdx.x, tid = threadIdx.x;
    const T* x = (const T*)p.out_conv + (size_t)b * p.T * p.F;
    float d0 = 0.f, d1 = 0.f;
    for (int c = tid; c < p.F; c += 256) {
        float s = 0.f;
        for (int t = 0; t < p.T; ++t) s += Num<T>::to_f32(x[(size_t)t * p.F + c]);
        const float m = s / (float)p.T;
        d0 = fmaf(m, p.ms_w[c], d0);
        d1 = fmaf(m, p.ms_w[p.F + c], d1);
    }
    d0 = block_sum_256(d0, sh);
    d1 = block_sum_256(d1, sh);
    if (tid == 0) {
        p.mean_std[2 * b] = d0 + p.ms_b[0];
        p.mean_std[2 * b + 1] = d1 + p.ms_b[1];
    }
}

__global__ __launch_bounds__(256) void cwt_recompose_kernel(CwtArgs p) {
    __shared__ float sh[4];
    const int b = blockIdx.x, tid = threadIdx.x;
    float* pr = p.pred + (size_t)b * p.T;
    float acc = 0.f;
    for (int t = tid; t < p.T; t += 256) {
        const size_t row = (size_t)b * p.T + t;
        const bool pad = p.mask && p.mask[row];
        float s = 0.f;
// ... 27 lines not shown
```

Measured before the change: 26.65 million.

## Fuse residual+LN into wres GEMM, gather predictor rows, batch phone output copies

Adds a gemm_wres variant that folds the residual add and layer norm into the weight-resident GEMM epilogue, streaming the residual tile into LDS beside X. The first frame-level variance predictor now reads phoneme rows through a per-frame index instead of running a separate length-regulate kernel that materialises expanded hidden states; a small frame_index kernel builds the index and mask. Phone-level output memcpys are merged into one multi-segment copy kernel. This cuts launches and a full frame-level activation write/read, at the cost of more LDS use in the GEMM and indirect row loads in the predictor.

```diff
diff --git a/lightningfastspeech2_amd/csrc/capi_ops.hip b/lightningfastspeech2_amd/csrc/capi_ops.hip
--- a/lightningfastspeech2_amd/csrc/capi_ops.hip
+++ b/lightningfastspeech2_amd/csrc/capi_ops.hip
@@ -32,8 +32,11 @@
 int apply_knob(Tuning& t, int variant) {
     int ok = 1;
     if (variant == 1500 || variant == 1501) t.attn_x3 = variant - 1500;
+    else if (variant >= 1410 && variant <= 1412) t.gemm_wres_ln = variant - 1410;
     else if (variant >= 1400 && variant <= 1402) t.gemm_wres = variant - 1400;
     else if (variant == 1340 || variant == 1341) t.enc_attn_out = variant - 1340;
+    else if (variant == 1350 || variant == 1351) t.phone_out_fused = variant - 1350;
+    else if (variant == 1330 || variant == 1331) t.pred_gather = variant - 1330;
     else if (variant == 1320 || variant == 1321) t.pred_fuse_embed = variant - 1320;
     else if (variant >= 1200 && variant <= 1204) t.attn_pipe = variant - 1200;
     else if (variant == 1100 || variant == 1101) t.colsum_fused = variant - 1100;
diff --git a/lightningfastspeech2_amd/csrc/engine.hip b/lightningfastspeech2_amd/csrc/engine.hip
--- a/lightningfastspeech2_amd/csrc/engine.hip
+++ b/lightningfastspeech2_amd/csrc/engine.hip
@@ -837,10 +837,23 @@
     const float* spk;
 };
 
+struct RowGather {
+    const int32_t* idx;
+    int rows;
+};
+
+bool predictor_takes_tail(const fs2_engine* e, const PredictorW& P, int S, int nbins) {
+    return P.wpk && !P.wpk_lo && e->fuse_predictor && !P.cwt && nbins >= 2 && nbins - 1 <= 512 &&
+           predictor_fused_supported(P.dt, P.filt, P.dw_all ? 3 : P.layers[0].c.taps, (int)P.layers.size(), S);
+}
+
 int predictor(fs2_engine* e, hipStream_t st, const PredictorW& P, const void* x, int B, int S, const uint8_t* mask,
-              float* pred, const LayerScratch& sc, const CwtOut* cw = nullptr, const EmbedTail* tail = nullptr, bool* tail_done = nullptr) {
+              float* pred, const LayerScratch& sc, const CwtOut* cw = nullptr, const EmbedTail* tail = nullptr, bool* tail_done = nullptr,
+              const RowGather* gather = nullptr) {
     const int M = B * S;
     if (tail_done) *tail_done = false;
+    if (gather && !(tail && tail_done && predictor_takes_tail(e, P, S, tail->nbins) && tail->y != x))
+        return fail(e, FS2_ERR_STATE, "row gather without the single-launch predictor and its embedding tail");
     if (P.cwt && !cw) return fail(e, FS2_ERR_STATE, "CWT predictor without its output buffers");
     if (P.wpk && P.wpk_lo && e->fuse_predictor && P.dt == FS2_F32 && e->front_split &&
         predictor_fused_x3_supported(P.filt, P.layers[0].c.taps, (int)P.layers.size(), S)) {
@@ -872,10 +885,11 @@
             a.be_y = tail->y; a.be_bins = tail->bins; a.be_emb = tail->emb; a.be_nbins = tail->nbins;
             a.be_std = tail->std; a.be_mean = tail->mean; a.be_pe = tail->pe; a.be_spk = tail->spk;
         }
+        if (gather) { a.row_idx = gather->idx; a.src_rows = gather->rows; }
         const double fl = (P.dw_all ? 2.0 * M * (double)P.filt * (P.filt + 3) : 2.0 * M * (double)P.filt * P.filt * a.taps) * a.nlayers;
         const double by = (double)M * P.filt * 2 + (double)M * 4 + (with_tail ? 2.0 * M * P.filt * 2 : 0.0);
         Bracket br(e, FS2_K_CONV_GEMM, st, fl, by);
-        Bracket brp(e, FS2_K_PREDICTOR, st, fl, by, x != e->xA && x != e->xB);
+        Bracket brp(e, FS2_K_PREDICTOR, st, fl, by, gather || (x != e->xA && x != e->xB));
         const int r = launch_predictor_fused(a, st);
         if (r != FS2_OK) return fail(e, r, "fused predictor launch failed (B=%d S=%d)", B, S);
         if (with_tail) *tail_done = true;
@@ -994,7 +1008,8 @@
     size_t cw = 0;
     for (int v = 0; v < e->cfg.n_variances; ++v)
         if (e->cfg.var_cwt[v]) cw = al(MT * 12 * 4) + al((size_t)B * 8) + 512;
-    return layer_scratch_bytes(e, B, T) + 2 * al(MT * H * esz) + al(MT) + (size_t)e->cfg.n_variances * al(MT * 4) + cw + 4096;
+    return layer_scratch_bytes(e, B, T) + 2 * al(MT * H * esz) + al(MT) + al(MT * 4)  +
+           (size_t)e->cfg.n_variances * al(MT * 4) + cw + 4096;
 }
 int ensure_arena(fs2_engine* e, Arena& ar, size_t need, const char* what) {
     if (need > ar.cap && !ar.external) HIPCHK(e, hipDeviceSynchronize());
@@ -1257,12 +1272,22 @@
 static void drop_graphs(fs2_engine* e);
 static int encode_body(fs2_engine* e, const int64_t* phones, const float* speaker, const int32_t* forced, LayerScratch& sc, hipStream_t st);
 
+static bool variance_tail_ok(const fs2_engine* e, int v) {
+    return e->tune.pred_fuse_embed && !e->debug && !e->forced_idx[v] && !e->forced_tgt[v] && !e->cfg.var_cwt[v] &&
+           (e->fdt == FS2_BF16 || (e->fdt == FS2_F32 && e->front_split && e->vars[v].pred.wpk_lo)) && e->cfg.hidden == 256;
+}
 static int variance_stage(fs2_engine* e, hipStream_t st, int v, void*& x, void*& xalt, int B, int S, const uint8_t* mask, float* vpred,
-                          const LayerScratch& sc, const CwtOut* cwo, bool add_pe_spk, Arena& dbg) {
+                          const LayerScratch& sc, const CwtOut* cwo, bool add_pe_spk, Arena& dbg, const RowGather* gather = nullptr) {
     const fs2_config& c = e->cfg;
     const size_t M = (size_t)B * S, H = c.hidden, esz = e->esz;
-    const bool tail_ok = e->tune.pred_fuse_embed && !e->debug && !e->forced_idx[v] && !e->forced_tgt[v] && !c.var_cwt[v] &&
-                         (e->fdt == FS2_BF16 || (e->fdt == FS2_F32 && e->front_split && e->vars[v].pred.wpk_lo)) && H == 256;
+    const bool tail_ok = variance_tail_ok(e, v);
+    if (gather) {
+        const EmbedTail tg{x, e->vars[v].bins, e->vars[v].emb, c.var_nbins, c.var_std[v], c.var_mean[v],
+                           add_pe_spk ? e->pe : nullptr, add_pe_spk ? e->spk : nullptr};
+        bool done = false;
+        CHK(predictor(e, st, e->vars[v].pred, e->xA, B, S, mask, vpred, sc, nullptr, tail_ok ? &tg : nullptr, &done, gather));
+        return done ? FS2_OK : fail(e, FS2_ERR_STATE, "gathering predictor launch left no rows");
+    }
     const EmbedTail tl{xalt, e->vars[v].bins, e->vars[v].emb, c.var_nbins, c.var_std[v], c.var_mean[v],
                        add_pe_spk ? e->pe : nullptr, add_pe_spk ? e->spk : nullptr};
     bool tail_done = false;
@@ -1426,6 +1451,30 @@
     const int B = e->B, L = e->L, T = e->T;
     const size_t H = c.hidden, MT = (size_t)B * T, ML = (size_t)B * L, esz = e->esz;
     auto phone_outputs = [&]() -> int {
+        if (e->tune.phone_out_fused) {
+            CopySegArgs cs;
+            bool fits = true;
+            auto seg = [&](void* dst, const void* src, size_t bytes) {
+                if (!dst || !bytes) return;
+                if (cs.n == CS_MAXSEG || bytes > 0xFFFFFFFFull) { fits = false; return; }
+                cs.src[cs.n] = src; cs.dst[cs.n] = dst; cs.bytes[cs.n] = (unsigned)bytes;
+                cs.n++;
+            };
+            seg(out->duration_prediction, e->dur_pred, ML * 4);
+            seg(out->duration_rounded, e->d_dur, ML * 4);
+            seg(out->src_mask, e->src_mask, ML);
+            for (int v = 0; v < c.n_variances; ++v) {
+                if (!c.var_level[v]) continue;
+                seg(out->variances[v], e->pv_pred[v], ML * 4);
+                if (c.var_cwt[v]) seg(out->var_spectrogram[v], e->pv_spec[v], ML * 10 * 4);
+                if (c.var_cwt[v]) seg(out->var_mean_std[v], e->pv_ms[v], (size_t)B * 8);
+            }
+            if (fits) {
+                for (int s2 = cs.n; s2 < CS_MAXSEG; ++s2) { cs.src[s2] = nullptr; cs.dst[s2] = nullptr; cs.bytes[s2] = 0; }
+                if (launch_copy_segments(cs, st) != FS2_OK) return fail(e, FS2_ERR_HIP, "phone-level output copy launch failed");
+                return FS2_OK;
+            }
+        }
         if (out->duration_prediction) HIPCHK(e, hipMemcpyAsync(out->duration_prediction, e->dur_pred, ML * 4, hipMemcpyDeviceToDevice, st));
         if (out->duration_rounded) HIPCHK(e, hipMemcpyAsync(out->duration_rounded, e->d_dur, ML * 4, hipMemcpyDeviceToDevice, st));
         if (out->src_mask) HIPCHK(e, hipMemcpyAsync(out->src_mask, e->src_mask, ML, hipMemcpyDeviceToDevice, st));
@@ -1468,7 +1517,21 @@
         if (e->dbg.reserve(need_d) != FS2_OK) return fail(e, FS2_ERR_NOMEM, "debug arena");
     }
 
-    {
+    int gather_v = -1;
+    for (int v = 0; v < c.n_variances && gather_v < 0; ++v)
+        if (!c.var_level[v]) gather_v = v;
+    if (gather_v >= 0 && !(e->tune.pred_gather && e->fdt == FS2_BF16 && variance_tail_ok(e, gather_v) &&
+                           predictor_takes_tail(e, e->vars[gather_v].pred, T, c.var_nbins) && (size_t)L * H * esz < 0xFFFFF000ull))
+        gather_v = -1;
+    RowGather rg{nullptr, L};
+    if (gather_v >= 0) {
+        int32_t* fidx = (int32_t*)e->scratch.take(MT * 4);
+        if (!fidx) return fail(e, FS2_ERR_NOMEM, "scratch arena too small");
+        rg.idx = fidx;
+        Bracket br(e, FS2_K_ROWOPS, st, 0, MT * 5.0);
+        FrameIndexArgs fa{e->d_cum, e->d_totals, fidx, tmask, sc.bits, B, L, T, sc.nw64};
+        if (launch_frame_index(fa, st) != FS2_OK) return fail(e, FS2_ERR_HIP, "frame_index launch failed");
+    } else {
         Bracket br(e, FS2_K_ROWOPS, st, 0, 2.0 * MT * H * esz);
         RegulateArgs ra{e->xA, e->d_cum, e->d_totals, yA, tmask, B, L, T, (int)H};
         if (launch_regulate(ra, e->fdt, st) != FS2_OK) return fail(e, FS2_ERR_HIP, "regulate launch failed");
@@ -1485,7 +1548,8 @@
             cwo.mean_std = out->var_mean_std[v] ? out->var_mean_std[v] : cw_ms;
             cwo.spec_out = out->var_spectrogram[v];
         }
-        CHK(variance_stage(e, st, v, yA, yB, B, T, tmask, vpred[v], sc, c.var_cwt[v] ? &cwo : nullptr, v == last_frame_v && fuse_pe, e->dbg));
+        CHK(variance_stage(e, st, v, yA, yB, B, T, tmask, vpred[v], sc, c.var_cwt[v] ? &cwo : nullptr, v == last_frame_v && fuse_pe, e->dbg,
+                           v == gather_v ? &rg : nullptr));
     }
     if (e->debug) CHK(tap_store(e, st, "adaptor_out", yA, MT * H, e->fdt));
     if (!fuse_pe || last_frame_v < 0) {
diff --git a/lightningfastspeech2_amd/csrc/fs2_kernels.h b/lightningfastspeech2_amd/csrc/fs2_kernels.h
--- a/lightningfastspeech2_amd/csrc/fs2_kernels.h
+++ b/lightningfastspeech2_amd/csrc/fs2_kernels.h
@@ -9,6 +9,7 @@
 struct Tuning {
     int gemm_variant = 0;
     int gemm_wres = 1;
+    int gemm_wres_ln = 1;
     int head_sums = 1;
     int gemm_persist = 1;
     int slab_xcd_remap = 1;
@@ -17,6 +18,8 @@
     int attn_x3 = 1;
     int enc_attn_out = 1;
     int pred_fuse_embed = 1;
+    int pred_gather = 1;
+    int phone_out_fused = 1;
     int attn_bwd_nb = 1, attn_bwd_nb_dq = 0;
     int colsum_fused = 0;
     int bgemm_full = 1, bgemm_xcd = 1, bgemm_tn256 = 1;
@@ -77,6 +80,8 @@
 int gemm_splitk_choice(int M, int N, int Cin, int taps, int S, int in_dtype);
 bool gemm_wres_supported(const GemmArgs& a, int in_dtype, int out_dtype, bool force);
 int launch_gemm_wres(const GemmArgs& a, hipStream_t stream);
+bool gemm_wres_ln_supported(const GemmArgs& a, int in_dtype, int out_dtype, bool force);
+int launch_gemm_wres_ln(const GemmArgs& a, hipStream_t stream);
 bool gemm_persist_supported(const GemmArgs& a, int in_dtype, int out_dtype, int mi);
 bool gemm_head_supported(const GemmArgs& a, int in_dtype, int out_dtype);
 bool gemm_persist_pays(const GemmArgs& a, int mi);
@@ -152,6 +157,8 @@
     float be_std = 1.f, be_mean = 0.f;
     const float* be_pe = nullptr;
     const float* be_spk = nullptr;
+    const int32_t* row_idx = nullptr;
+    int src_rows = 0;
 };
 bool predictor_fused_supported(int dtype, int H, int taps, int nlayers, int S);
 size_t predictor_packed_bytes_per_layer(int taps = 3);
@@ -330,6 +337,25 @@
     int B, L, T, H;
 };
 int launch_regulate(const RegulateArgs& a, int dtype, hipStream_t stream);
+
+struct FrameIndexArgs {
+    const int32_t* cum;
+    const int32_t* totals;
+    int32_t* idx;
+    uint8_t* tgt_mask;
+    uint64_t* bits;
+    int B, L, T, nw64;
+};
+int launch_frame_index(const FrameIndexArgs& a, hipStream_t stream);
+
+constexpr int CS_MAXSEG = 16;
+struct CopySegArgs {
+    const void* src[CS_MAXSEG];
+    void* dst[CS_MAXSEG];
+    unsigned bytes[CS_MAXSEG];
+    int n = 0;
+};
+int launch_copy_segments(const CopySegArgs& a, hipStream_t stream);
 
 struct BucketArgs {
     const void* x;
diff --git a/lightningfastspeech2_amd/csrc/gemm_mfma.hip b/lightningfastspeech2_amd/csrc/gemm_mfma.hip
--- a/lightningfastspeech2_amd/csrc/gemm_mfma.hip
+++ b/lightningfastspeech2_amd/csrc/gemm_mfma.hip
@@ -1190,6 +1190,8 @@
         if (g_gemm_wres && g_gemm_variant == 0 && a.ksplit <= 1 && gemm_wres_supported(a, in_dtype, out_dtype, g_gemm_wres == 2)) return launch_gemm_wres(a, stream);
         return launch_gemm_plain(a, in_dtype, out_dtype, stream, nullptr);
     }
+    if (tn.gemm_wres_ln && g_gemm_variant == 0 && gemm_wres_ln_supported(a, in_dtype, out_dtype, tn.gemm_wres_ln == 2))
+        return launch_gemm_wres_ln(a, stream);
     bool fused = false;
     if (a.z_out && a.N > S_BN) return FS2_ERR_SHAPE;
     if (a.drop_p > 0.f && (a.N > S_BN || !a.z_out)) return FS2_ERR_SHAPE;
diff --git a/lightningfastspeech2_amd/csrc/gemm_wres.hip b/lightningfastspeech2_amd/csrc/gemm_wres.hip
--- a/lightningfastspeech2_amd/csrc/gemm_wres.hip
+++ b/lightningfastspeech2_amd/csrc/gemm_wres.hip
@@ -25,6 +25,7 @@
 #define WRES_STAMP(i) do { } while (0)
 #endif
 
+template <bool LN>
 __global__ __launch_bounds__(512) void gemm_wres_kernel(GemmArgs p, int ncol, int nrg, int tiles) {
 #if defined(__HIP_DEVICE_COMPILE__)
     __shared__ __attribute__((aligned(16))) unsigned char xs0[WR_TILEB];
@@ -71,15 +72,37 @@
         stage(0);
         stage(2);
     }
-    __shared__ __attribute__((aligned(16))) float sbias[256];
+    __shared__ __attribute__((aligned(16))) float sbias[LN ? 768 : 256];
     if (tid < 256) sbias[tid] = p.bias ? p.bias[n0 + tid] : 0.f;
+    if constexpr (LN) {
+        if (tid < 256) {
+            sbias[256 + tid] = p.ln_g[tid];
+            sbias[512 + tid] = p.ln_b[tid];
+        }
+    }
     __syncthreads();
+    __shared__ __attribute__((aligned(16))) unsigned char rsb[LN ? WR_TILEB : 16];
+    __shared__ float red1[LN ? 4 * WR_RT : 1];
+    __shared__ float red2[LN ? 4 * WR_RT : 1];
+    const __amdgpu_buffer_rsrc_t rrs = __builtin_amdgcn_make_buffer_rsrc(
+        (void*)(LN ? p.res : p.X), 0, (unsigned)(((size_t)(p.M - 1) * (LN ? p.ldc : p.ldx) + WR_K) * 2), 0x00020000);
+    auto issue_res = [&](int t, int k, bool live) {
+        if constexpr (LN) {
+            int ln = lane;
+            asm volatile("" : "+v"(ln));
+            const int m = t * WR_RT + wm * (WR_MI * 16) + k * 8 + (ln >> 3);
+            const unsigned voff = (live && m < p.M) ? (unsigned)m * (unsigned)(p.ldc * 2) + (unsigned)(wn * 128 + ((ln & 7) << 4)) : 0xFFFFF000u;
+            __builtin_amdgcn_raw_ptr_buffer_load_lds(rrs, (__attribute__((address_space(3))) void*)(rsb + (wave * 6 + k) * 1024), 16, voff, 0, 0, 0);
+        }
+    };
 
     const __amdgpu_buffer_rsrc_t xrs =
         __builtin_amdgcn_make_buffer_rsrc((void*)p.X, 0, (unsigned)(((size_t)(p.M - 1) * p.ldx + WR_K) * 2), 0x00020000);
     auto issue_piece = [&](auto BUF, int t, int k, bool live) {
         unsigned char* const dst = decltype(BUF)::value ? xs1 : xs0;
-        const int c = k * 8 + wave, i = 2 * c + (lane >> 5), ps = lane & 31, m = t * WR_RT + i;
+        int ln = lane;
+        if constexpr (LN) asm volatile("" : "+v"(ln));
+        const int c = k * 8 + wave, i = 2 * c + (ln >> 5), ps = ln & 31, m = t * WR_RT + i;
         const int ls = (ps & 16) | ((((ps & 7) ^ (i & 7)) << 1) | ((ps >> 3) & 1));
         const unsigned voff = (live && m < p.M) ? (unsigned)m * (unsigned)(p.ldx * 2) + (unsigned)(ls << 4) : 0xFFFFF000u;
         __builtin_amdgcn_raw_ptr_buffer_load_lds(xrs, (__attribute__((address_space(3))) void*)(dst + c * 1024), 16, voff, 0, 0, 0);
@@ -118,6 +141,8 @@
     using B1 = std::integral_constant<int, 1>;
     WRES_STAMP(1);
     issue(B0{}, tbeg);
+#pragma unroll
+    for (int k = 0; k < 6; ++k) issue_res(tbeg, k, true);
     auto tile = [&](auto CUR, auto NXT, int t) {
         WRES_STAMP(4 + (t - tbeg) * 5);
         if (t == tbeg) __builtin_amdgcn_s_waitcnt(0x0F70);
@@ -128,6 +153,7 @@
         const bool has_next = t + 1 < tend;
         auto side = [&](int ks) {
             if (ks < WR_NDMA) issue_piece(NXT, t + 1, ks, has_next);
+            if (ks < 6) issue_res(t + 1, ks, has_next);
         };
         WRES_STAMP(7 + (t - tbeg) * 5);
         f32x4_t acc[4][WR_MI];
@@ -135,8 +161,103 @@
         for (int a = 0; a < 4; ++a)
 #pragma unroll
             for (int b = 0; b < WR_MI; ++b) acc[a][b] = (f32x4_t){0.f, 0.f, 0.f, 0.f};
+        if constexpr (LN) {
+            int ln = lane;
+            asm volatile("" : "+v"(ln));
+            const int fr = ln & 15, fg = ln >> 4;
+#pragma unroll
+            for (int mi = 0; mi < WR_MI; ++mi)
+#pragma unroll
+                for (int j = 0; j < 2; ++j) {
+                    const uint4 rq = *(const uint4*)(rsb + (wave * 6 + mi * 2 + (fr >> 3)) * 1024 + (((fr & 7) * 8 + j * 4 + fg) << 4));
+                    const unsigned w4[4] = {rq.x, rq.y, rq.z, rq.w};
+#pragma unroll
+                    for (int e = 0; e < 4; ++e) {
+                        acc[2 * j + (e >> 1)][mi][(2 * e) & 3] = __uint_as_float(w4[e] << 16);
+                        acc[2 * j + (e >> 1)][mi][(2 * e + 1) & 3] = __uint_as_float(w4[e] & 0xffff0000u);
+                    }
+                }
+        }
         compute(CUR, acc, side);
         WRES_STAMP(8 + (t - tbeg) * 5);
+        if constexpr (LN) {
+            int ln = lane;
+            asm volatile("" : "+v"(ln));
+            const int fr = ln & 15, fg = ln >> 4;
+            const float lo = p.relu ? 0.f : -__builtin_inff();
+#pragma unroll
+            for (int ni = 0; ni < 4; ++ni) {
+                const int n = wn * 64 + wr_wcol(ni, fg);
+#pragma unroll
+                for (int r = 0; r < 4; ++r) {
+                    const float bvv = sbias[n + r];
+#pragma unroll
+                    for (int mi = 0; mi < WR_MI; ++mi) acc[ni][mi][r] = fmaxf(acc[ni][mi][r] + bvv, lo);
+                }
+            }
+            const float invn = 1.0f / (float)p.N;
+            float mean[WR_MI], rstd[WR_MI];
+#pragma unroll
+            for (int mi = 0; mi < WR_MI; ++mi) {
+                float sm = 0.f;
+#pragma unroll
+                for (int ni = 0; ni < 4; ++ni) sm += (acc[ni][mi][0] + acc[ni][mi][1]) + (acc[ni][mi][2] + acc[ni][mi][3]);
+                sm = group4_sum(sm);
+                if (fg == 0) red1[wn * WR_RT + wm * (WR_MI * 16) + mi * 16 + fr] = sm;
+            }
+            __syncthreads();
+#pragma unroll
+            for (int mi = 0; mi < WR_MI; ++mi) {
+                const int row = wm * (WR_MI * 16) + mi * 16 + fr;
+                mean[mi] = ((red1[row] + red1[WR_RT + row]) + (red1[2 * WR_RT + row] + red1[3 * WR_RT + row])) * invn;
+            }
+#pragma unroll
+            for (int mi = 0; mi < WR_MI; ++mi)
+#pragma unroll
+                for (int ni = 0; ni < 4; ++ni)
+#pragma unroll
+                    for (int r = 0; r < 4; ++r) acc[ni][mi][r] -= mean[mi];
+#pragma unroll
+            for (int mi = 0; mi < WR_MI; ++mi) {
+                float q = 0.f;
+#pragma unroll
+                for (int ni = 0; ni < 4; ++ni)
+#pragma unroll
+                    for (int r = 0; r < 4; ++r) q = __builtin_fmaf(acc[ni][mi][r], acc[ni][mi][r], q);
+                q = group4_sum(q);
+                if (fg == 0) red2[wn * WR_RT + wm * (WR_MI * 16) + mi * 16 + fr] = q;
+            }
+            __syncthreads();
+#pragma unroll
+            for (int mi = 0; mi < WR_MI; ++mi) {
+                const int row = wm * (WR_MI * 16) + mi * 16 + fr;
+                const float var = ((red2[row] + red2[WR_RT + row]) + (red2[2 * WR_RT + row] + red2[3 * WR_RT + row])) * invn;
+                rstd[mi] = 1.0f / sqrtf(var + p.ln_eps);
+            }
+            const float* lnp = sbias + 256;
+#pragma unroll
+            for (int j = 0; j < 2; ++j) {
+                const int n = wn * 64 + j * 32 + fg * 8;
+                float gg[8], bb[8];
+#pragma unroll
+                for (int h = 0; h < 2; ++h) {
+                    const float4 g4 = *(const float4*)(lnp + n + 4 * h), b4 = *(const float4*)(lnp + 256 + n + 4 * h);
+                    gg[4 * h] = g4.x; gg[4 * h + 1] = g4.y; gg[4 * h + 2] = g4.z; gg[4 * h + 3] = g4.w;
+                    bb[4 * h] = b4.x; bb[4 * h + 1] = b4.y; bb[4 * h + 2] = b4.z; bb[4 * h + 3] = b4.w;
+                }
+#pragma unroll
+                for (int mi = 0; mi < WR_MI; ++mi) {
+                    float y[8];
+#pragma unroll
+                    for (int r = 0; r < 8; ++r) y[r] = __builtin_fmaf(acc[2 * j + (r >> 2)][mi][r & 3] * rstd[mi], gg[r], bb[r]);
+                    const int m = t * WR_RT + wm * (WR_MI * 16) + mi * 16 + fr;
+                    if (m < p.M)
+                        *(uint4*)((bf16*)p.C + (size_t)m * p.ldc + wn * 64 + j * 32 + fg * 8) =
+                            make_uint4(pack_bf16x2(y[0], y[1]), pack_bf16x2(y[2], y[3]), pack_bf16x2(y[4], y[5]), pack_bf16x2(y[6], y[7]));
+                }
+            }
+            return;
+        }
 #pragma unroll
         for (int mi = 0; mi < WR_MI; ++mi) {
 #pragma unroll
@@ -182,9 +303,24 @@
            !a.split && !a.rs_stats && a.ldx % 8 == 0 && a.ldc % 8 == 0 && (size_t)a.M * a.ldx * 2 < 0xFFFFF000ull && (size_t)a.M * a.ldc * 2 < 0xFFFFF000ull;
 }
 
+bool gemm_wres_ln_supported(const GemmArgs& a, int in_dtype, int out_dtype, bool force) {
+    if (!force && a.S <= 768) return false;
+    return in_dtype == FS2_BF16 && out_dtype == FS2_BF16 && a.taps == 1 && a.K == WR_K && a.Cin == WR_K && a.N == 256 && a.M > 0 && a.C &&
+           a.res && a.ln_g && a.ln_b && !a.relu && a.drop_p == 0.f && !a.dot_w && !a.z_out && !a.epi_res && !a.stats_out && !a.gate &&
+           !a.zero_rows && !a.split && !a.rs_stats && !a.C_lo && a.ksplit <= 1 && a.ldx % 8 == 0 && a.ldc % 8 == 0 &&
+           (((uintptr_t)a.X | (uintptr_t)a.C | (uintptr_t)a.res) & 15) == 0 &&
+           (size_t)a.M * a.ldx * 2 < 0xFFFFF000ull && (size_t)a.M * a.ldc * 2 < 0xFFFFF000ull;
+}
+
+int launch_gemm_wres_ln(const GemmArgs& a, hipStream_t stream) {
+    const int tiles = (a.M + WR_RT - 1) / WR_RT, nrg = wres_row_groups(1, tiles);
+    hipLaunchKernelGGL(gemm_wres_kernel<true>, dim3((unsigned)nrg), dim3(512), 0, stream, a, 1, nrg, tiles);
+    return hipGetLastError() == hipSuccess ? FS2_OK : FS2_ERR_HIP;
+}
+
 int launch_gemm_wres(const GemmArgs& a, hipStream_t stream) {
     const int ncol = a.N / 256, tiles = (a.M + WR_RT - 1) / WR_RT, nrg = wres_row_groups(ncol, tiles);
-    hipLaunchKernelGGL(gemm_wres_kernel, dim3((unsigned)(nrg * ncol)), dim3(512), 0, stream, a, ncol, nrg, tiles);
+    hipLaunchKernelGGL(gemm_wres_kernel<false>, dim3((unsigned)(nrg * ncol)), dim3(512), 0, stream, a, ncol, nrg, tiles);
     return hipGetLastError() == hipSuccess ? FS2_OK : FS2_ERR_HIP;
 }
 
diff --git a/lightningfastspeech2_amd/csrc/predictor_fused.hip b/lightningfastspeech2_amd/csrc/predictor_fused.hip
--- a/lightningfastspeech2_amd/csrc/predictor_fused.hip
+++ b/lightningfastspeech2_amd/csrc/predictor_fused.hip
@@ -85,9 +85,11 @@
         }
     } else
     {
-        const bf16* xu = (const bf16*)p.x + (size_t)ub * S * PF_H;
+        const int32_t* ridx = p.row_idx ? p.row_idx + (size_t)ub * S : nullptr;
+        const int xrows = ridx ? p.src_rows : S;
+        const bf16* xu = (const bf16*)p.x + (size_t)ub * xrows * PF_H;
         const __amdgpu_buffer_rsrc_t xrs =
-            __builtin_amdgcn_make_buffer_rsrc((void*)xu, 0, (unsigned)((size_t)S * PF_ROWB), 0x00020000);
+            __builtin_amdgcn_make_buffer_rsrc((void*)xu, 0, (unsigned)((size_t)xrows * PF_ROWB), 0x00020000);
         constexpr int NCH = (R + 2) / 2;
 #pragma unroll
         for (int k = 0; k < (NCH + NWV - 1) / NWV; ++k) {
@@ -95,7 +97,9 @@
             if (c < NCH) {
                 const int i = 2 * c + (lane >> 5), ps = lane & 31, t = t0 - 1 + i;
                 const int ls = (ps & 16) | ((((ps & 7) ^ (i & 7)) << 1) | ((ps >> 3) & 1));
-                const unsigned voff = (t >= 0 && t < S) ? (unsigned)(t * PF_ROWB + (ls << 4)) : 0xFFFFF000u;
+                int srow = (t >= 0 && t < S) ? t : -1;
+                if (ridx && srow >= 0) srow = ridx[srow];
+                const unsigned voff = (srow >= 0 && srow < xrows) ? (unsigned)(srow * PF_ROWB + (ls << 4)) : 0xFFFFF000u;
                 __builtin_amdgcn_raw_ptr_buffer_load_lds(xrs, (__attribute__((address_space(3))) void*)(slab + c * 1024),
                                                          16, voff, 0, 0, 0);
             }
@@ -455,7 +459,8 @@
         }
         using XT = typename std::conditional<X3, float, bf16>::type;
         using XV = typename std::conditional<X3, float4, uint2>::type;
-        const XT* xg = (const XT*)p.x + (size_t)ub * S * PF_H + lane_t * 4;
+        const int32_t* ridx = (!X3 && p.row_idx) ? p.row_idx + (size_t)ub * S : nullptr;
+        const XT* xg = (const XT*)p.x + (size_t)ub * (ridx ? p.src_rows : S) * PF_H + lane_t * 4;
         XT* yg = (XT*)p.be_y + (size_t)ub * S * PF_H + lane_t * 4;
         const float* spr = p.be_spk ? p.be_spk + (size_t)ub * PF_H + lane_t * 4 : nullptr;
         float4 sp4 = make_float4(0.f, 0.f, 0.f, 0.f);
@@ -475,7 +480,14 @@
                 for (int k = 0; k < 8; ++k)
                     if (k < nb) lo += __popcll(__ballot(bl[k] < v));
                 if (v != v) lo = nedge;
-                xv[j] = *(const XV*)(xg + (size_t)tc * PF_H);
+                int srow = tc;
+                if constexpr (!X3) {
+                    if (ridx) srow = ridx[tc];
+                }
+                xv[j] = *(const XV*)(xg + (size_t)(srow < 0 ? 0 : srow) * PF_H);
+                if constexpr (!X3) {
+                    if (srow < 0) xv[j] = make_uint2(0u, 0u);
+                }
                 ev[j] = *(const float4*)(p.be_emb + (size_t)lo * PF_H + lane_t * 4);
                 if (p.be_pe) pv[j] = *(const float4*)(p.be_pe + (size_t)tc * PF_H + lane_t * 4);
             }
@@ -538,6 +550,7 @@
 }
 int launch_predictor_fused_x3(const PredictorArgs& a, hipStream_t stream) {
     if (!predictor_fused_x3_supported(a.H, a.taps, a.nlayers, a.S) || !a.wpk_lo) return FS2_ERR_SHAPE;
+    if (a.row_idx) return FS2_ERR_ARG;
     if (a.be_y && (a.be_y == a.x || !a.be_bins || !a.be_emb || a.be_nbins < 2 || a.be_nbins - 1 > 512)) return FS2_ERR_ARG;
     if (a.B <= 0) return FS2_OK;
     const int halo2 = 2 * (a.nlayers - 1);
@@ -554,6 +567,7 @@
     auto tiles = [&](int R) { return (long)a.B * ((a.S + (R - halo2) - 1) / (R - halo2)); };
     if (a.be_y && (a.be_y == a.x || !a.be_bins || !a.be_emb || a.be_nbins < 2 || a.be_nbins - 1 > 512)) return FS2_ERR_ARG;
     if ((a.dw_w != nullptr) != (a.dw_b != nullptr)) return FS2_ERR_ARG;
+    if (a.row_idx && (a.src_rows < 1 || (size_t)a.src_rows * PF_ROWB >= 0xFFFFF000ull)) return FS2_ERR_ARG;
     if (((uintptr_t)a.x | (uintptr_t)a.wpk | (uintptr_t)a.bias | (uintptr_t)a.ln_g | (uintptr_t)a.ln_b | (uintptr_t)a.head_w | (uintptr_t)a.dw_w |
          (uintptr_t)a.dw_b | (uintptr_t)a.be_y | (uintptr_t)a.be_emb | (uintptr_t)a.be_pe | (uintptr_t)a.be_spk) & 15)
         return FS2_ERR_ARG;
diff --git a/lightningfastspeech2_amd/csrc/rowops.hip b/lightningfastspeech2_amd/csrc/rowops.hip
--- a/lightningfastspeech2_amd/csrc/rowops.hip
+++ b/lightningfastspeech2_amd/csrc/rowops.hip
@@ -577,6 +577,78 @@
     return hipGetLastError() == hipSuccess ? FS2_OK : FS2_ERR_HIP;
 }
 
+__global__ __launch_bounds__(256) void frame_index_kernel(FrameIndexArgs p) {
+    const int lane = threadIdx.x & 63;
+    const int w = blockIdx.x * 4 + (threadIdx.x >> 6), b = blockIdx.y;
+    const int t0 = w * 64;
+    if (t0 >= p.T && w >= p.nw64) return;
+    const int total = p.totals[b];
+    const int32_t* cum = p.cum + (size_t)b * p.L;
+    const int t = t0 + lane;
+    const bool in = t < p.T && t < total;
+    int own = 0;
+    if (p.L <= 64 * RG_MAXC) {
+        int32_t cl[RG_MAXC];
+#pragma unroll
+        for (int k = 0; k < RG_MAXC; ++k) {
+            const int i = lane + 64 * k;
+            cl[k] = i < p.L ? cum[i] : 0x7fffffff;
+        }
+        const int nc = (p.L + 63) / 64;
+        const int nr = p.T - t0 < 64 ? p.T - t0 : 64;
+        for (int r = 0; r < nr; ++r) {
+            int lo = 0;
+#pragma unroll
+            for (int k = 0; k < RG_MAXC; ++k)
+                if (k < nc) lo += __popcll(__ballot(cl[k] <= t0 + r));
+            if (lane == r) own = lo;
+        }
+    } else if (in) {
+        int lo = 0, hi = p.L;
+        while (lo < hi) {
+            const int mid = (lo + hi) >> 1;
+            if (cum[mid] > t) hi = mid; else lo = mid + 1;
+        }
+        own = lo;
+    }
+    if (t < p.T) {
+        p.idx[(size_t)b * p.T + t] = in ? own : -1;
+        p.tgt_mask[(size_t)b * p.T + t] = t >= total;
+    }
+    const unsigned long long bal = __ballot(in);
+    if (lane == 0 && w < p.nw64) p.bits[(size_t)b * p.nw64 + w] = bal;
+}
+
+int launch_frame_index(const FrameIndexArgs& a, hipStream_t stream) {
+    if (a.B <= 0 || a.T <= 0) return FS2_OK;
+    const int nw = a.nw64 > (a.T + 63) / 64 ? a.nw64 : (a.T + 63) / 64;
+    hipLaunchKernelGGL(frame_index_kernel, dim3((nw + 3) / 4, a.B), dim3(256), 0, stream, a);
+    return hipGetLastError() == hipSuccess ? FS2_OK : FS2_ERR_HIP;
+}
+
+__global__ __launch_bounds__(256) void copy_segments_kernel(CopySegArgs p) {
+    const int s = blockIdx.y;
+    const unsigned char* src = (const unsigned char*)p.src[s];
+    unsigned char* dst = (unsigned char*)p.dst[s];
+    const size_t n = p.bytes[s];
+    const size_t nv = ((((uintptr_t)src | (uintptr_t)dst) & 15) == 0) ? n / 16 : 0;
+    const size_t i0 = (size_t)blockIdx.x * 256 + threadIdx.x, step = (size_t)gridDim.x * 256;
+    for (size_t i = i0; i < nv; i += step) ((uint4*)dst)[i] = ((const uint4*)src)[i];
+    for (size_t i = nv * 16 + i0; i < n; i += step) dst[i] = src[i];
+}
+
+int launch_copy_segments(const CopySegArgs& a, hipStream_t stream) {
+    if (a.n <= 0) return FS2_OK;
+    if (a.n > CS_MAXSEG) return FS2_ERR_ARG;
+    unsigned mx = 0;
+    for (int s = 0; s < a.n; ++s) mx = a.bytes[s] > mx ? a.bytes[s] : mx;
+    if (mx == 0) return FS2_OK;
+    unsigned bx = (mx / 16 + 255) / 256;
+    bx = bx < 1 ? 1 : (bx > 32 ? 32 : bx);
+    hipLaunchKernelGGL(copy_segments_kernel, dim3(bx, a.n), dim3(256), 0, stream, a);
+    return hipGetLastError() == hipSuccess ? FS2_OK : FS2_ERR_HIP;
+}
+
 constexpr int BE_ROWS = 8, BE_MAXB = 8;
 template <typename T, int NV>
 __global__ __launch_bounds__(256) void bucket_embed_kernel(BucketArgs p) {
```

Result: slower. 26.31 million (-1.3%).
